# SpectacularAI/3dgs-deblur

Hardware: AMD Instinct MI355X
Metric: fwd+bwd rasterize MPix/s at 1M Gaussians, 1080p, 5 sub-poses (higher is better)
Workload: dtype f32

## Files before the change

3dgs-deblur_amd/_lib.py:

```python
from __future__ import annotations

import ctypes
from pathlib import Path

from ._build import LIB_PATH, build_library

_P, _I, _F, _L = ctypes.c_void_p, ctypes.c_int, ctypes.c_float, ctypes.c_longlong

_SIGS = {
    "gs_subpose_viewmats_fwd": [_I, _P, _P, _P, _P, _P, _P],
    "gs_subpose_viewmats_bwd": [_I, _P, _P, _P, _P, _P, _P, _P, _P, _P],
    "gs_project_fwd": [_I, _P, _P, _F, _P, _P, _F, _F, _F, _F, _I, _I, _F, _P, _P, _P, _P, _P, _P, _P, _P, _P],
    "gs_project_bwd": [_I, _P, _P, _F, _P, _P, _F, _F, _F, _F, _I, _I, _F, _P, _P, _P, _P, _P, _P, _P, _P, _I, _P, _L, _P],
    "gs_sh_fwd": [_I, _I, _I, _P, _P, _P, _P],
    "gs_sh_bwd": [_I, _I, _I, _P, _P, _P, _P],
    "gs_project_fused_fwd": [_I, _I, _P, _P, _F, _P, _P, _P, _I, _I, _P, _F, _F, _F, _F, _I, _I, _F, _I, _I,
                             _P, _P, _P, _P, _P, _I, _P],
    "gs_slice_colors": [_I, _P, _P, _I, _P, _P, _P, _I, _I, _P, _P, _P],
    "gs_project_fused_bwd": [_I, _I, _P, _P, _F, _P, _P, _P, _I, _I, _P, _F, _F, _F, _F, _I, _I, _F, _I,
                             _P, _P, _P, _P, _P, _P, _P, _P, _P, _P, _I, _P, _I, _P, _P, _L, _P],
    "gs_project_pixvel_fwd": [_I, _I, _P, _P, _F, _P, _P, _P, _I, _I, _P, _P, _P, _F, _F, _F, _F, _I, _I, _F, _I, _I,
                              _P, _P, _P, _P, _F, _P, _P, _I, _P],
    "gs_rasterize_fwd_rs_slice": [_P, _P, _P, _P, _I, _I, _I, _P, _P, _P, _P, _P, _I, _I, _P, _I, _P, _P, _P, _I, _F, _P,
                                  _P],
    "gs_rasterize_bwd_rs_slice": [_P, _P, _P, _P, _P, _I, _I, _I, _P, _P, _P, _P, _P, _P, _P, _P, _P, _I, _I, _P, _F, _F,
                                  _P, _I, _F, _P, _P],
    "gs_project_pixvel_bwd": [_I, _I, _P, _P, _F, _P, _P, _P, _I, _I, _P, _P, _P, _F, _F, _F, _F, _I, _I, _F, _I,
                              _P, _P, _P, _P, _P, _P, _P, _P, _P, _P, _P, _I, _P, _I, _P, _P, _L, _P],
    "gs_pack_records": [_I, _P, _P, _P, _P, _P, _P, _I, _I, _P, _P, _P, _P],
    "gs_unpack_record_grads": [_I, _P, _P, _P, _P, _P, _P],
    "gs_exclusive_scan_u32": [_L, _P, _P, _P, _P, _L, _P],
    "gs_radix_sort_pairs_u32": [_L, _P, _P, _P, _P, _I, _I, _I, _P, _L, ctypes.POINTER(_I), _P],
    "gs_radix_sort_pairs_u64": [_L, _P, _P, _P, _P, _I, _I, _I, _P, _L, ctypes.POINTER(_I), _P],
    "gs_radix_sort_pairs_gather_u32": [_L, _P, _P, _P, _P, _I, _I, _I, _P, _L, ctypes.POINTER(_I), _P, _P, _P, _P],
    "gs_radix_sort_pairs_carry_u32": [_L, _P, _P, _P, _P, _I, _I, _I, _P, _L, ctypes.POINTER(_I), _P, _P, _P,
                                      ctypes.POINTER(_I), _P, _P],
    "gs_segmented_sort_pairs_u32": [_L, _L, _P, _P, _P, _P, _I, _I, _I, _P, _L, ctypes.POINTER(_I), _P],
    "gs_segmented_sort_compact_u32": [_L, _L, _P, _P, _P, _P, _I, _I, _I, ctypes.c_uint, _P, _P, _P, _P, _L,
                                      ctypes.POINTER(_I), _P],
    "gs_segmented_sort_select_u32": [_L, _L, _P, _P, _P, _P, _P, _I, _I, _I, ctypes.c_uint, _P, _P, _P, _P, _P, _P, _L,
                                     ctypes.POINTER(_I), _L, _P],
    "gs_depth_select": [_L, _L, _P, _P, _L, _P, _P, _P, _L, _P],
    "gs_exclusive_scan_segments_u32": [_L, _L, _P, _P, _P, _P, _P, _L, _P],
    "gs_make_depth_keys64": [_L, _I, _P, _P, _P],
    "gs_gather_counts": [_L, _P, _P, _P, _P],
    "gs_emit_intersects": [_L, _I, _I, _I, _P, _P, _P, _L, _P, _P, ctypes.c_uint, _P],
    "gs_tile_bin_edges_u32": [_L, _P, _I, _P, _P, _P],
    "gs_tile_bin_edges_u64": [_L, _P, _I, _P, _P],
    "gs_tile_bin_edges_ids_u32": [_L, _P, _I, _P, _P, _P, _P, _P],
    "gs_map_gaussian_to_intersects": [_I, _P, _P, _P, _P, _I, _I, _P, _P, _P],
    "gs_rasterize_fwd": [_P, _P, _P, _P, _P, _I, _I, _I, _I, _P, _P, _P, _I, _I, _P],
    "gs_rasterize_bwd": [_P, _P, _P, _P, _P, _I, _I, _I, _I, _P, _P, _P, _P, _P, _I, _I, _P],
    "gs_slice_plan": [_I, _I, _I, _P, _P, _L, _P, _P, _P, _P, _P, _P],
    "gs_slice_plan_select": [_I, _I, _I, _P, _P, _P, _P, _P, _P, _P, _P, _P],
    "gs_tile_open_sat": [_I, _I, _I, _P, _P, _P, _P, _P],
    "gs_slice_counts": [_I, _I, _I, _P, _P, _P, _P, _P, _I, _I, _P, _P, _P],
    "gs_emit_open_intersects": [_I, _I, _I, _I, _P, _P, _P, _P, _P, _P, _P, ctypes.c_uint, _I, _I, _P, _P, _P, _P],
    "gs_slice_counts_exact": [_I, _I, _I, _P, _P, _P, _P, _P, _P, _I, _I, _P, _P, _I, _P, _P, _P, _P, _P, _P],
    "gs_slice_counts_exact_swept": [_I, _I, _I, _P, _P, _P, _P, _P, _P, _I, _I, _P, _P, _I, _P, _P, _P, _P, _P, _F, _F, _F,
                                    _P],
    "gs_rasterize_fwd_slice": [_P, _P, _P, _P, _P, _I, _I, _I, _I, _P, _P, _P, _P, _P, _I, _I, _P, _P, _I, _P, _P, _P,
                               _I, _P],
    "gs_rasterize_bwd_slice": [_P, _P, _P, _P, _P, _I, _I, _I, _I, _P, _P, _P, _P, _P, _P, _P, _P, _P, _P, _P, _I, _P,
                               _I, _P, _F, _F, _P],
    "gs_rasterize_fwd_slice_stats": [_P, _P, _P, _P, _P, _I, _I, _I, _I, _P, _P, _P, _P, _P, _I, _I, _P, _P, _P, _P],
    "gs_reduce_grad_tuples": [_I, _P, _P, _P, _P, _P, _P, _P, _L, _P, _I, _P],
    "gs_combine_fwd": [_I, _L, _P, _F, _F, _P, _P],
    "gs_combine_bwd": [_I, _L, _P, _F, _F, _P, _P, _P, _P],
    "gs_combine_bwd_scale": [_I, _L, _F, _P, _P, _P, _P],
    "gs_combine_fwd_batched": [_I, _I, _L, _P, _F, _F, _P, _P],
    "gs_combine_bwd_batched": [_I, _I, _L, _P, _F, _F, _P, _P, _P, _P],
    "gs_combine_bwd_scale_batched": [_I, _I, _L, _F, _P, _P, _P, _P],
    "gs_dp_row_mask": [_I, _I, _P, _P, _P, _P],
    "gs_dp_pack_rows": [_L, _P, _I, _P, _P, _P, _P],
    "gs_dp_scatter_add_rows": [_L, _P, _I, _P, _P, _F, _P],
    "gs_dp_pack_masked_rows": [_I, _P, _P, _I, _P, _I, _P, _P, _P, _P],
    "gs_dp_scatter_add_payload": [_I, _P, _I, _P, _P, _F, _P],
    "gs_slice_project_records": [_I, _I, _I, _P, _P, _P, _P, _I, _I, _P, _P],
    "gs_project_records": [_I, _I, _P, _I, _I, _P, _P],
    "gs_frame_forward": [_P, _P, _P, _P, _P, _P, _P, _P, _P, _P, _I, _I, _P, _P, _P, _P, _P, _P, _P, _P, _L, _P, _L, _P, _P],
    "gs_frame_backward": [_P, _P, _P, _P, _P, _P, _P, _P, _F, _F, _I, _P, _P, _P, _P, _P, _L, _P],
    "gs_frame_backward_depth": [_P, _P, _P, _P, _P, _P, _P, _P, _F, _F, _I, _P, _P, _P, _P, _P, _L, _P, _P],
    "gs_xy_absgrad_sum": [_I, _I, _I, _P, _P, _P, _P],
    "gs_frame_profile_enable": [ctypes.c_uint],
    "gs_frame_profile_read": [_I, _P, _P],
    "gs_image_loss_fwd_bwd": [_I, _I, _P, _P, _F, _P, _P, _P, _L, _P],
    "gs_adam_step": [_I, _P, _P, _P, _P, _P, _P, ctypes.c_double, ctypes.c_double, ctypes.c_double, _I, _P],
    "gs_adam_step_rows": [_I, _I, _P, _P, _P, _P, _P, _P, _P, ctypes.c_double, ctypes.c_double, ctypes.c_double, _I,
                          _P, _L, _P],
    "gs_visible_rows": [_I, _I, _P, _P, _P],
    "gs_mcmc_inject_noise": [_I, _P, _P, _P, _P, _F, _L, _L, _P, _P, _P],
    "gs_mcmc_relocation": [_I, _P, _P, _P, _P, _P, _P],
    "gs_bilagrid_slice_fwd": [_I, _I, _I, _I, _I, _I, _I, _P, _P, _P, _P, _P],
    "gs_bilagrid_slice_bwd": [_I, _I, _I, _I, _I, _I, _I, _P, _P, _P, _P, _P, _P, _P, _L, _P],
    "gs_bilagrid_tv_fwd_bwd": [_I, _I, _I, _I, _P, _F, _P, _P, _P, _L, _P],
}
_SIGS_LL = {
    "gs_scan_workspace_bytes": [_L],
    "gs_radix_sort_workspace_bytes": [_L, _I, _I],
    "gs_segmented_sort_workspace_bytes": [_L, _L, _I, _I],
    "gs_segmented_sort_compact_workspace_bytes": [_L, _L, _I, _I, _I],
    "gs_depth_select_workspace_bytes": [_I],
    "gs_project_pose_scratch_bytes": [_I, _I, _I],
    "gs_image_loss_workspace_bytes": [_I, _I],
    "gs_adam_step_rows_workspace_bytes": [_I],
    "gs_frame_backward_bytes": [_P],
    "gs_bilagrid_slice_bwd_workspace_bytes": [_I, _I, _I, _I, _I, _I, _I],
    "gs_bilagrid_tv_workspace_bytes": [_I, _I, _I, _I],
}

_lib = None


class HipLibraryError(RuntimeError):
    pass


def load(build_if_missing: bool = True) -> ctypes.CDLL:
    global _lib
    if _lib is not None:
        return _lib
    import os
    import shutil
    override = os.environ.get("GSD_LIB_PATH")
    path = Path(override) if override else LIB_PATH
    if not override and build_if_missing and shutil.which(os.environ.get("HIPCC", "/opt/rocm/bin/hipcc")):
        from ._build import is_current, HASH_PATH, CSRC
        stale = not is_current()
        if stale and path.exists() and not HASH_PATH.exists():
            t = path.stat().st_mtime
            stale = any(f.stat().st_mtime > t for f in list(CSRC.glob("*.hip")) + list(CSRC.glob("*.h")))
        if stale:
            import fcntl
            try:
                lock = open(str(path) + ".lock", "w")
            except OSError as e:
                if not path.exists():
                    raise HipLibraryError(f"{path} is missing and {path.parent} is not writable: {e}") from e
                import warnings
                warnings.warn(f"{path} may be older than its sources and {path.parent} is not writable; loading it as is")
            else:
                with lock:
                    fcntl.flock(lock, fcntl.LOCK_EX)
                    try:
                        build_library()
                    finally:
                        fcntl.flock(lock, fcntl.LOCK_UN)
    if not path.exists():
        raise HipLibraryError(f"{path} is missing; run __graft_entry__.build()")
    try:
        lib = ctypes.CDLL(str(path))
    except OSError as e:
        raise HipLibraryError(f"cannot load HIP library {path}: {e}") from e
    for name, args in _SIGS.items():
        fn = getattr(lib, name)
        fn.argtypes = args
        fn.restype = _I
    for name, args in _SIGS_LL.items():
        fn = getattr(lib, name)
        fn.argtypes = args
        fn.restype = _L
    lib.gs_version.restype = ctypes.c_char_p
    lib.gs_version.argtypes = []
    _lib = lib
    return lib


def exported_names():
    return sorted(list(_SIGS) + list(_SIGS_LL) + ["gs_version"])


def check(status: int, what: str) -> None:
    if status != 0:
        kind = {1: "invalid argument", 3: "workspace too small"}.get(status, None)
        if kind is None and status >= 1000:
            kind = f"hipError_t {status - 1000}"
        raise HipLibraryError(f"{what} failed: {kind or status}")
```

3dgs-deblur_amd/csrc/binning.hip:

```cpp
#include <algorithm>
#include <atomic>
#include "gs_common.h"

namespace gs {

constexpr int kScanItems = 8;
constexpr int kScanBlock = 256 * kScanItems;

__device__ __forceinline__ unsigned block_excl_scan(unsigned v, unsigned& total, unsigned* lds ) {
  const int lane = lane_id(), wave = threadIdx.x >> 6;
  unsigned inc = v;
#pragma unroll
  for (int o = 1; o < 64; o <<= 1) {
    unsigned t = __shfl_up(inc, o);
    if (lane >= o) inc += t;
  }
  if (lane == 63) lds[wave] = inc;
  __syncthreads();
  unsigned w0 = lds[0], w1 = lds[1], w2 = lds[2], w3 = lds[3];
  unsigned woff = wave == 0 ? 0u : (wave == 1 ? w0 : (wave == 2 ? w0 + w1 : w0 + w1 + w2));
  total = w0 + w1 + w2 + w3;
  __syncthreads();
  return woff + inc - v;
}
// ... 175 lines not shown
  if (n <= kScanSmallMax && !dl.keys && !sm.cnt) {
    hipLaunchKernelGGL(scan_small_kernel, dim3(1), dim3(256), 0, st, n, in, out, total_out);
    return gs_launch_status();
  }
  unsigned* bsum = reinterpret_cast<unsigned*>(ws);
  hipLaunchKernelGGL(scan_reduce_kernel, dim3((unsigned)nb), dim3(256), 0, st, n, in, bsum, dl, sm);
  if (nb <= kScanFusedMaxBlocks || dl.keys || sm.cnt) {
    hipLaunchKernelGGL(scan_apply_fused_kernel, dim3((unsigned)nb), dim3(256), 0, st, n, in, bsum, out, total_out, dl,
                       sm);
  } else {
    hipLaunchKernelGGL(scan_bsums_kernel, dim3(1), dim3(256), 0, st, (unsigned)nb, bsum, total_out);
    hipLaunchKernelGGL(scan_apply_kernel, dim3((unsigned)nb), dim3(256), 0, st, n, in, bsum, out);
  }
  return gs_launch_status();
}

#ifndef GS_SORT_ROUNDS_U32
#define GS_SORT_ROUNDS_U32 16
#endif
template <typename KeyT> struct SortCfg;
template <> struct SortCfg<unsigned> { static constexpr int kRounds = GS_SORT_ROUNDS_U32; };
template <> struct SortCfg<unsigned long long> { static constexpr int kRounds = 16; };

template <typename KeyT> constexpr int sort_block_keys() { return 256 * SortCfg<KeyT>::kRounds; }

struct SegInfo { size_t seg_len; unsigned nblk_seg; };

struct SegDev {
  const unsigned* cnt_in;
  unsigned* cnt_out;
  const unsigned* total;
  unsigned long long skip;
  const unsigned* key_lo;
  const unsigned* key_hi;
};

template <typename KeyT>
struct KeepTest {
  KeyT skip, lo, hi;
  bool on, has_hi;
  __device__ __forceinline__ KeepTest(const SegDev& sd, unsigned seg)
      : skip((KeyT)sd.skip), lo(sd.key_lo ? (KeyT)sd.key_lo[seg] : (KeyT)0), hi(sd.key_hi ? (KeyT)sd.key_hi[seg] : (KeyT)0),
        on(sd.cnt_out != nullptr), has_hi(sd.key_hi != nullptr) {}
  __device__ __forceinline__ bool drop(KeyT k) const { return on && (k == skip || k < lo || (has_hi && k >= hi)); }
};

template <typename KeyT, int BITS>
__global__ __launch_bounds__(256) void radix_hist_kernel(size_t n, const KeyT* __restrict__ keys, int shift,
                                                         unsigned mask, SegInfo sg,
                                                         unsigned* __restrict__ ghist,
                                                         const unsigned* __restrict__ n_dev, SegDev sd) {
  constexpr int NB = 1 << BITS;
  constexpr int R = SortCfg<KeyT>::kRounds;
  if (n_dev) {
    n = min(n, (size_t)*n_dev);
    sg.nblk_seg = (unsigned)((n + 256 * R - 1) / (256 * R));
    if (blockIdx.x >= sg.nblk_seg) return;
  }
  __shared__ unsigned hist[NB];
  const unsigned seg = blockIdx.x / sg.nblk_seg, b = blockIdx.x % sg.nblk_seg;
  const size_t base = (size_t)seg * sg.seg_len + (size_t)b * (256 * R);
  size_t limit = min(n, (size_t)(seg + 1) * sg.seg_len);
  if (sd.cnt_in) limit = min(limit, (size_t)seg * sg.seg_len + sd.cnt_in[seg]);
  if (base >= limit) {
    for (int d = threadIdx.x; d < NB; d += 256) ghist[((size_t)seg * NB + d) * sg.nblk_seg + b] = 0u;
    return;
  }
  for (int d = threadIdx.x; d < NB; d += 256) hist[d] = 0;
  __syncthreads();
  KeyT k[R];
#pragma unroll
  for (int r = 0; r < R; ++r) {
    size_t i = base + (size_t)r * 256 + threadIdx.x;
    k[r] = i < limit ? keys[i] : (KeyT)0;
  }
  const int lane = lane_id();
  const KeepTest<KeyT> keep(sd, seg);
  bool skewed;
  {
    const size_t i0 = base + threadIdx.x;
    const bool ok0 = i0 < limit && !keep.drop(k[0]);
    const unsigned d = (unsigned)(k[0] >> shift) & mask;
    const unsigned long long m = __ballot(ok0);
    const unsigned d0 = (unsigned)readlane_i((int)d, m ? __ffsll((long long)m) - 1 : 0);
    skewed = __popcll(__ballot(ok0 && d == d0)) >= 16;
  }
  if (skewed) {
#pragma unroll
    for (int r = 0; r < R; ++r) {
      size_t i = base + (size_t)r * 256 + threadIdx.x;
      const bool ok = i < limit && !keep.drop(k[r]);
      const unsigned d = (unsigned)(k[r] >> shift) & mask;
      unsigned long long todo = __ballot(ok);
#pragma unroll 1
      for (int it = 0; it < 4 && todo; ++it) {
        const int src = __ffsll((long long)todo) - 1;
        const unsigned d0 = (unsigned)readlane_i((int)d, src);
        const unsigned long long same = __ballot(ok && d == d0) & todo;
        if (lane == src) atomicAdd(&hist[d0], (unsigned)__popcll(same));
        todo &= ~same;
      }
      if ((todo >> lane) & 1ull) atomicAdd(&hist[d], 1u);
    }
  } else {
#pragma unroll
    for (int r = 0; r < R; ++r) {
      size_t i = base + (size_t)r * 256 + threadIdx.x;
      if (i < limit && !keep.drop(k[r])) atomicAdd(&hist[(unsigned)(k[r] >> shift) & mask], 1u);
    }
  }
  __syncthreads();
  for (int d = threadIdx.x; d < NB; d += 256) ghist[((size_t)seg * NB + d) * sg.nblk_seg + b] = hist[d];
}

template <typename KeyT, int BITS, int PACK = 0>
__global__ __launch_bounds__(256) void radix_scatter_kernel(size_t n, const KeyT* __restrict__ keys_in,
                                                            const unsigned* __restrict__ vals_in,
                                                            KeyT* __restrict__ keys_out,
                                                            unsigned* __restrict__ vals_out, int shift, unsigned mask,
                                                            SegInfo sg,
                                                            const unsigned* __restrict__ ghist_scanned,
                                                            const unsigned* __restrict__ gather_src,
                                                            unsigned* __restrict__ gather_out,
                                                            const unsigned* __restrict__ n_dev, SegDev sd,
                                                            const unsigned* __restrict__ p2_in,
                                                            unsigned* __restrict__ p2_out,
                                                            int pack_bits) {
  constexpr int NB = 1 << BITS;
  constexpr int R = SortCfg<KeyT>::kRounds;
  constexpr int BK = 256 * R;
  if (n_dev) {
    n = min(n, (size_t)*n_dev);
    sg.nblk_seg = (unsigned)((n + BK - 1) / BK);
    if (blockIdx.x >= sg.nblk_seg) return;
  }
  {
    const unsigned seg0 = blockIdx.x / sg.nblk_seg, blk0 = blockIdx.x % sg.nblk_seg;
    if (sd.cnt_in && (size_t)blk0 * BK >= (size_t)sd.cnt_in[seg0]) return;
  }
  constexpr int DPT = NB / 256;
  __shared__ KeyT s_keys[BK];
  __shared__ unsigned s_vals[BK];
  __shared__ unsigned cnt[4][NB];
  __shared__ unsigned s_dbase[NB];
  __shared__ unsigned s_gbase[NB];
  __shared__ unsigned s_scan[8];
  const int lane = lane_id(), wave = threadIdx.x >> 6;
  for (int d = threadIdx.x; d < 4 * NB; d += 256) (&cnt[0][0])[d] = 0;
  __syncthreads();
  const unsigned seg = blockIdx.x / sg.nblk_seg, blk = blockIdx.x % sg.nblk_seg;
  const size_t bbase = (size_t)seg * sg.seg_len + (size_t)blk * BK;
  size_t limit = min(n, (size_t)(seg + 1) * sg.seg_len);
  if (sd.cnt_in) limit = min(limit, (size_t)seg * sg.seg_len + sd.cnt_in[seg]);
  const bool compacting = sd.cnt_out != nullptr;
  const KeepTest<KeyT> keep(sd, seg);
  const size_t wbase = bbase + (size_t)wave * (R * 64);
  const unsigned long long lt_mask = (1ull << lane) - 1ull;
  KeyT key[R];
  unsigned short pos[R];
#pragma unroll
  for (int r = 0; r < R; ++r) {
    size_t i = wbase + (size_t)r * 64 + lane;
    key[r] = i < limit ? keys_in[i] : (KeyT)0;
  }
#pragma unroll
  for (int r = 0; r < R; ++r) {
    size_t i = wbase + (size_t)r * 64 + lane;
    bool valid = i < limit && !keep.drop(key[r]);
    unsigned digit = (unsigned)(key[r] >> shift) & mask;
    unsigned long long peers = __ballot(valid);
#pragma unroll
    for (int b = 0; b < BITS; ++b) {
      bool bit = (digit >> b) & 1u;
      unsigned long long m = __ballot(bit);
      peers &= bit ? m : ~m;
    }
    unsigned prefix = __popcll(peers & lt_mask);
    unsigned total = __popcll(peers);
    unsigned base = 0;
    if (valid) base = cnt[wave][digit];
    __builtin_amdgcn_wave_barrier();
    if (valid && prefix == 0) cnt[wave][digit] = base + total;
    __builtin_amdgcn_wave_barrier();
    pos[r] = (unsigned short)(base + prefix);
  }
  __syncthreads();
  {
    unsigned c[DPT], sum = 0;
#pragma unroll
    for (int j = 0; j < DPT; ++j) {
      int d = threadIdx.x * DPT + j;
      c[j] = cnt[0][d] + cnt[1][d] + cnt[2][d] + cnt[3][d];
      sum += c[j];
    }
    unsigned tot;
    unsigned ex = block_excl_scan(sum, tot, s_scan);
    if (threadIdx.x == 0) s_scan[4] = tot;
    const unsigned seg_org = (unsigned)((size_t)seg * sg.seg_len);
    unsigned gb[DPT];
    const size_t seg_first = (size_t)seg * NB * sg.nblk_seg;
    const unsigned seg_base = ghist_scanned[seg_first];
    if (compacting && blk == 0 && threadIdx.x == 0) {
      const unsigned nseg = gridDim.x / sg.nblk_seg;
      const unsigned next = seg + 1 < nseg ? ghist_scanned[seg_first + (size_t)NB * sg.nblk_seg] : *sd.total;
      sd.cnt_out[seg] = next - seg_base;
    }
#pragma unroll
    for (int j = 0; j < DPT; ++j)
      gb[j] = ghist_scanned[seg_first + (size_t)(threadIdx.x * DPT + j) * sg.nblk_seg + blk] - seg_base + seg_org;
#pragma unroll
    for (int j = 0; j < DPT; ++j) {
      int d = threadIdx.x * DPT + j;
      s_dbase[d] = ex;
      s_gbase[d] = gb[j];
      unsigned run = ex;
#pragma unroll
      for (int w = 0; w < 4; ++w) {
        unsigned cw = cnt[w][d];
        cnt[w][d] = run;
        run += cw;
      }
      ex += c[j];
    }
  }
  __syncthreads();
  constexpr int RB = R >= 4 ? 4 : R;
  unsigned pv[RB];
#pragma unroll
  for (int r0 = 0; r0 < R; r0 += RB) {
    if (PACK == 1 || vals_in) {
      const unsigned* __restrict__ src = PACK == 1 ? gather_src : vals_in;
      const size_t last = limit ? limit - 1 : 0;
#pragma unroll
      for (int q = 0; q < RB; ++q) pv[q] = src[min(wbase + (size_t)(r0 + q) * 64 + lane, last)];
    }
#pragma unroll
    for (int q = 0; q < RB; ++q) {
      const int r = r0 + q;
      size_t i = wbase + (size_t)r * 64 + lane;
      if (i < limit && !keep.drop(key[r])) {
        unsigned digit = (unsigned)(key[r] >> shift) & mask;
        unsigned slot = cnt[wave][digit] + pos[r];
        s_keys[slot] = key[r];
        if (PACK == 1) s_vals[slot] = (unsigned)i | (min(pv[q], (1u << (32 - pack_bits)) - 1u) << pack_bits);
        else s_vals[slot] = vals_in ? pv[q] : (unsigned)i;
      }
    }
  }
  __syncthreads();
  const unsigned nvalid = s_scan[4];
#pragma unroll 4
  for (int r = 0; r < R; ++r) {
    unsigned slot = (unsigned)r * 256 + threadIdx.x;
    if (slot < nvalid) {
      KeyT k = s_keys[slot];
      unsigned digit = (unsigned)(k >> shift) & mask;
      size_t dst = (size_t)s_gbase[digit] + (slot - s_dbase[digit]);
      keys_out[dst] = k;
      const unsigned v = s_vals[slot];
      if (PACK == 2) {
        const unsigned idx = v & ((1u << pack_bits) - 1u), c = v >> pack_bits;
        vals_out[dst] = idx;
        gather_out[dst] = c == (1u << (32 - pack_bits)) - 1u ? gather_src[idx] : c;
      } else {
        vals_out[dst] = v;
        if (gather_out) gather_out[dst] = gather_src[v];
      }
    }
  }
  if (p2_out) {
    __syncthreads();
#pragma unroll
    for (int r0 = 0; r0 < R; r0 += RB) {
      const size_t last = limit ? limit - 1 : 0;
#pragma unroll
      for (int q = 0; q < RB; ++q) pv[q] = p2_in[min(wbase + (size_t)(r0 + q) * 64 + lane, last)];
#pragma unroll
      for (int q = 0; q < RB; ++q) {
        const int r = r0 + q;
        size_t i = wbase + (size_t)r * 64 + lane;
        if (i < limit && !keep.drop(key[r])) {
          unsigned digit = (unsigned)(key[r] >> shift) & mask;
          s_vals[cnt[wave][digit] + pos[r]] = pv[q];
        }
      }
    }
    __syncthreads();
#pragma unroll 4
    for (int r = 0; r < R; ++r) {
      unsigned slot = (unsigned)r * 256 + threadIdx.x;
      if (slot < nvalid) {
        unsigned digit = (unsigned)(s_keys[slot] >> shift) & mask;
        p2_out[(size_t)s_gbase[digit] + (slot - s_dbase[digit])] = s_vals[slot];
      }
    }
  }
}

constexpr int kTailR = 24;
constexpr int kTailLocalCap = kTailR * 1024;
constexpr int kTailMaxBits = 9;
constexpr size_t kTailLds = ((size_t)kTailLocalCap + 16 * (1 << kTailMaxBits) + 64) * sizeof(unsigned);

__global__ __launch_bounds__(1024) void seg_tail_sort_kernel(size_t seg_len, const unsigned* __restrict__ keys_in,
                                                             const unsigned* __restrict__ vals_in,
                                                             unsigned* __restrict__ keys_out,
                                                             unsigned* __restrict__ vals_out,
                                                             const unsigned* __restrict__ cnt_in, int begin_bit, int end_bit,
                                                             const unsigned* __restrict__ gather_src,
                                                             unsigned* __restrict__ gather_out, int pack_bits) {
  extern __shared__ unsigned tail_lds[];
  unsigned* const stage = tail_lds;
  unsigned* const cnt = stage + kTailLocalCap;
  unsigned* const red = cnt + 16 * (1 << kTailMaxBits);
  const unsigned seg = blockIdx.x;
  const unsigned n = cnt_in[seg];
  if (n == 0 || n > (unsigned)kTailLocalCap) return;
  const size_t org = (size_t)seg * seg_len;
  const int lane = lane_id(), wave = threadIdx.x >> 6;
  const unsigned Re = (n + 1023u) >> 10;
  const unsigned wbase = (unsigned)wave * Re * 64u;
  const unsigned long long lt_mask = (1ull << lane) - 1ull;
  unsigned key[kTailR];
  unsigned pos2[kTailR / 2];
  unsigned kmin = 0xffffffffu, kmax = 0u;
  const unsigned emask = end_bit >= 32 ? 0xffffffffu : (1u << end_bit) - 1u;
#pragma unroll
  for (int r = 0; r < kTailR; ++r) {
    const unsigned e = wbase + (unsigned)r * 64u + lane;
    const bool ok = (unsigned)r < Re && e < n;
    key[r] = ok ? keys_in[org + e] : 0u;
    if (ok) {
      stage[e] = vals_in[org + e];
      kmin = min(kmin, key[r] & emask);
      kmax = max(kmax, key[r] & emask);
    }
  }
#pragma unroll
  for (int o = 32; o > 0; o >>= 1) {
    kmin = min(kmin, (unsigned)__shfl_xor((int)kmin, o));
    kmax = max(kmax, (unsigned)__shfl_xor((int)kmax, o));
  }
  if (lane == 0) { red[wave] = kmin; red[16 + wave] = kmax; }
  __syncthreads();
#pragma unroll
  for (int w = 0; w < 16; ++w) { kmin = min(kmin, red[w]); kmax = max(kmax, red[16 + w]); }
  const unsigned base = kmin & ~((1u << begin_bit) - 1u);
  const unsigned span = (kmax - base) >> begin_bit;
  const int rem = span ? 32 - __clz((int)span) : 0;
  const int passes = (rem + kTailMaxBits - 1) / kTailMaxBits;
  const int wbits = passes ? (rem + passes - 1) / passes : 0;
  const unsigned nb = 1u << wbits, mask = nb - 1u;
  int shift = begin_bit;
  for (int p = 0; p < passes; ++p, shift += wbits) {
    for (unsigned d = threadIdx.x; d < 16u * nb; d += 1024u) cnt[d] = 0u;
    __syncthreads();
    unsigned* const wcnt = cnt + (unsigned)wave * nb;
#pragma unroll
    for (int r = 0; r < kTailR; ++r) {
      if ((unsigned)r < Re) {
        const unsigned e = wbase + (unsigned)r * 64u + lane;
        const bool valid = e < n;
        const unsigned digit = (((key[r] & emask) - base) >> shift) & mask;
        unsigned long long peers = __ballot(valid);
#pragma unroll
        for (int b = 0; b < kTailMaxBits; ++b) {
          if (b < wbits) {
            const bool bit = (digit >> b) & 1u;
            const unsigned long long m = __ballot(bit);
            peers &= bit ? m : ~m;
          }
        }
        const unsigned prefix = __popcll(peers & lt_mask), total = __popcll(peers);
        unsigned c0 = 0;
        if (valid) c0 = wcnt[digit];
        __builtin_amdgcn_wave_barrier();
        if (valid && prefix == 0) wcnt[digit] = c0 + total;
        __builtin_amdgcn_wave_barrier();
        pos2[r >> 1] = (r & 1) ? (pos2[r >> 1] | ((c0 + prefix) << 16)) : (c0 + prefix);
      }
    }
    __syncthreads();
    {
      const unsigned d = threadIdx.x;
      unsigned c = 0;
      if (d < nb) {
#pragma unroll
        for (int w = 0; w < 16; ++w) c += cnt[(unsigned)w * nb + d];
      }
      unsigned inc = c;
#pragma unroll
      for (int o = 1; o < 64; o <<= 1) {
        const unsigned t = __shfl_up(inc, o);
        if (lane >= o) inc += t;
      }
      if (lane == 63) red[32 + wave] = inc;
      __syncthreads();
      unsigned run = inc - c;
      for (int w = 0; w < wave; ++w) run += red[32 + w];
      if (d < nb) {
#pragma unroll
        for (int w = 0; w < 16; ++w) {
          const unsigned cw = cnt[(unsigned)w * nb + d];
          cnt[(unsigned)w * nb + d] = run;
          run += cw;
        }
      }
    }
    __syncthreads();
    unsigned val[kTailR];
#pragma unroll
    for (int r = 0; r < kTailR; ++r) {
      const unsigned e = wbase + (unsigned)r * 64u + lane;
      if ((unsigned)r < Re && e < n) {
        val[r] = stage[e];
        const unsigned rank = (r & 1) ? pos2[r >> 1] >> 16 : pos2[r >> 1] & 0xffffu;
        const unsigned slot = wcnt[(((key[r] & emask) - base) >> shift) & mask] + rank;
        pos2[r >> 1] = (r & 1) ? ((pos2[r >> 1] & 0xffffu) | (slot << 16)) : ((pos2[r >> 1] & 0xffff0000u) | slot);
      }
    }
    __syncthreads();
#pragma unroll
    for (int r = 0; r < kTailR; ++r) {
      const unsigned e = wbase + (unsigned)r * 64u + lane;
      if ((unsigned)r < Re && e < n) stage[(r & 1) ? pos2[r >> 1] >> 16 : pos2[r >> 1] & 0xffffu] = key[r];
    }
    __syncthreads();
#pragma unroll
    for (int r = 0; r < kTailR; ++r) {
      const unsigned e = wbase + (unsigned)r * 64u + lane;
      if ((unsigned)r < Re && e < n) key[r] = stage[e];
    }
    __syncthreads();
#pragma unroll
    for (int r = 0; r < kTailR; ++r) {
      const unsigned e = wbase + (unsigned)r * 64u + lane;
      if ((unsigned)r < Re && e < n) stage[(r & 1) ? pos2[r >> 1] >> 16 : pos2[r >> 1] & 0xffffu] = val[r];
    }
    __syncthreads();
  }
#pragma unroll
  for (int r = 0; r < kTailR; ++r) {
    const unsigned e = wbase + (unsigned)r * 64u + lane;
    if ((unsigned)r < Re && e < n) {
      keys_out[org + e] = key[r];
      const unsigned v = stage[e];
      if (pack_bits) {
        const unsigned idx = v & ((1u << pack_bits) - 1u), c = v >> pack_bits;
        vals_out[org + e] = idx;
        gather_out[org + e] = c == (1u << (32 - pack_bits)) - 1u ? gather_src[idx] : c;
      } else {
        vals_out[org + e] = v;
        if (gather_out) gather_out[org + e] = gather_src[v];
      }
    }
  }
}

template <typename KeyT>
static inline unsigned sort_nblk(size_t n) {
  return (unsigned)((n + sort_block_keys<KeyT>() - 1) / sort_block_keys<KeyT>());
}
template <typename KeyT>
static inline unsigned sort_nblk_seg(size_t n, size_t seg_len, unsigned* nblk_seg) {
  if (seg_len == 0 || seg_len >= n) { *nblk_seg = sort_nblk<KeyT>(n); return *nblk_seg; }
  *nblk_seg = sort_nblk<KeyT>(seg_len);
  return (unsigned)((n + seg_len - 1) / seg_len) * *nblk_seg;
}

static inline void radix_plan(int bits, int* passes, int* per, int* tmpl_bits, int max_digit = 11) {
  if (max_digit < 8) max_digit = 8;
  if (max_digit > 11) max_digit = 11;
  int ps = (bits + max_digit - 1) / max_digit;
  if (ps < 1) ps = 1;
  int w = (bits + ps - 1) / ps;
  *passes = ps; *per = w; *tmpl_bits = w < 8 ? 8 : w;
}

template <typename KeyT>
static inline size_t radix_hist_bytes(size_t n, size_t seg_len, int bits, int max_digit = 11) {
  int ps, per, tb;
  radix_plan(bits, &ps, &per, &tb, max_digit);
  unsigned nbs;
  size_t b = ((size_t)1 << tb) * sort_nblk_seg<KeyT>(n, seg_len, &nbs) * sizeof(unsigned);
  return (b + 255) & ~(size_t)255;
}

template <typename KeyT>
static inline size_t radix_ws_bytes(size_t n, size_t seg_len, int bits, int max_digit = 11) {
  int ps, per, tb;
  radix_plan(bits, &ps, &per, &tb, max_digit);
  unsigned nbs;
  return radix_hist_bytes<KeyT>(n, seg_len, bits, max_digit) +
         scan_ws_bytes(((size_t)1 << tb) * sort_nblk_seg<KeyT>(n, seg_len, &nbs)) + 256;
}

template <typename KeyT, int BITS>
static void radix_pass(size_t n, size_t seg_len, const KeyT* kin, const unsigned* vin, KeyT* kout, unsigned* vout,
                       int shift, unsigned mask, void* ws, size_t hist_bytes, hipStream_t st,
                       const unsigned* gather_src = nullptr, unsigned* gather_out = nullptr,
                       const unsigned* n_dev = nullptr, SegDev sd = SegDev{nullptr, nullptr, nullptr, 0ull, nullptr, nullptr},
                       const unsigned* p2_in = nullptr, unsigned* p2_out = nullptr, int pack = 0, int pack_bits = 0,
                       unsigned tail_blocks = 0) {
  SegInfo sg;
  unsigned nblk = sort_nblk_seg<KeyT>(n, seg_len, &sg.nblk_seg);
  sg.seg_len = (seg_len == 0 || seg_len >= n) ? n : seg_len;
  if (tail_blocks && tail_blocks < sg.nblk_seg) {
    nblk = nblk / sg.nblk_seg * tail_blocks;
    sg.nblk_seg = tail_blocks;
  }
  unsigned* ghist = reinterpret_cast<unsigned*>(ws);
  {
    size_t hn = ((size_t)1 << BITS) * nblk;
    void* scan_ws = reinterpret_cast<char*>(ws) + hist_bytes;
    hipLaunchKernelGGL((radix_hist_kernel<KeyT, BITS>), dim3(nblk), dim3(256), 0, st, n, kin, shift, mask, sg, ghist,
                       n_dev, sd);
    run_scan(hn, ghist, ghist, sd.cnt_out ? const_cast<unsigned*>(sd.total) : nullptr, scan_ws, st,
             DevLen{n_dev, (unsigned)sort_block_keys<KeyT>(), (unsigned)(1u << BITS)});
  }
  if constexpr (BITS == 8 && sizeof(KeyT) == 4) {
    if (pack == 1) {
      hipLaunchKernelGGL((radix_scatter_kernel<KeyT, BITS, 1>), dim3(nblk), dim3(256), 0, st, n, kin, vin, kout, vout,
                         shift, mask, sg, ghist, gather_src, gather_out, n_dev, sd, p2_in, p2_out, pack_bits);
      return;
    }
    if (pack == 2) {
      hipLaunchKernelGGL((radix_scatter_kernel<KeyT, BITS, 2>), dim3(nblk), dim3(256), 0, st, n, kin, vin, kout, vout,
                         shift, mask, sg, ghist, gather_src, gather_out, n_dev, sd, p2_in, p2_out, pack_bits);
      return;
    }
  }
  hipLaunchKernelGGL((radix_scatter_kernel<KeyT, BITS>), dim3(nblk), dim3(256), 0, st, n, kin, vin, kout, vout, shift,
                     mask, sg, ghist, gather_src, gather_out, n_dev, sd, p2_in, p2_out, 0);
}

template <typename KeyT>
static int radix_sort(size_t n, size_t seg_len, KeyT* k0, unsigned* v0, KeyT* k1, unsigned* v1, int v0_is_iota,
                      int begin_bit, int end_bit, void* ws, size_t ws_bytes, int* result_buf, hipStream_t st,
                      int max_digit = 11, const unsigned* gather_src = nullptr, unsigned* gather_out = nullptr,
                      const unsigned* n_dev = nullptr, unsigned* seg_counts = nullptr,
                      unsigned long long skip_key = 0ull, const unsigned* p2_src = nullptr, unsigned* p2_a = nullptr,
                      unsigned* p2_b = nullptr, int* result_p2 = nullptr, const KeyT* k_src = nullptr,
                      const unsigned* key_lo = nullptr, const unsigned* key_hi = nullptr, unsigned tail_blocks = 0) {
  int bits = end_bit - begin_bit;
  if (bits <= 0) return GS_ERR_INVALID;
  if (ws_bytes < radix_ws_bytes<KeyT>(n, seg_len, bits, max_digit)) return GS_ERR_WORKSPACE;
  int passes, per, tb;
  radix_plan(bits, &passes, &per, &tb, max_digit);
  const size_t hist_bytes = radix_hist_bytes<KeyT>(n, seg_len, bits, max_digit);
  KeyT* kk[2] = {k0, k1};
  unsigned* vv[2] = {v0, v1};
  int cur = 0, shift = begin_bit;
  int pack_bits = 0;
  if (sizeof(KeyT) == 4 && gather_src && gather_out && seg_counts && v0_is_iota && !p2_src &&
      tb == 8 && passes >= 2) {
    while (((size_t)1 << pack_bits) < n) ++pack_bits;
    if (pack_bits > 28) pack_bits = 0;
  }
  for (int p = 0; p < passes; ++p) {
    int w = per;
    if (shift + w > end_bit) w = end_bit - shift;
    const unsigned mask = (1u << w) - 1u;
    const unsigned* vin = (p == 0 && v0_is_iota) ? nullptr : vv[cur];
    const int pack = pack_bits ? (p == 0 ? 1 : (p == passes - 1 ? 2 : 0)) : 0;
    const unsigned* gs_ = (p == passes - 1 || pack == 1) ? gather_src : nullptr;
    unsigned* go_ = (p == passes - 1) ? gather_out : nullptr;
    SegDev sd{nullptr, nullptr, nullptr, 0ull};
    if (seg_counts) {
      unsigned* total_dev = reinterpret_cast<unsigned*>(reinterpret_cast<char*>(ws) +
                                                        radix_ws_bytes<KeyT>(n, seg_len, bits, max_digit) - 128);
      if (p == 0) sd = SegDev{nullptr, seg_counts, total_dev, skip_key, key_lo, key_hi};
      else sd = SegDev{seg_counts, nullptr, nullptr, 0ull, nullptr, nullptr};
    }
    const unsigned* p2i = nullptr;
    unsigned* p2o = nullptr;
    if (p2_src) {
      p2o = (p & 1) ? p2_b : p2_a;
      p2i = p == 0 ? p2_src : ((p & 1) ? p2_a : p2_b);
    }
    const KeyT* kin = (p == 0 && k_src) ? k_src : kk[cur];
    switch (tb) {
      case 8:  radix_pass<KeyT, 8>(n, seg_len, kin, vin, kk[cur ^ 1], vv[cur ^ 1], shift, mask, ws, hist_bytes, st, gs_, go_, n_dev, sd, p2i, p2o, pack, pack_bits, p > 0 ? tail_blocks : 0u); break;
      case 9:  radix_pass<KeyT, 9>(n, seg_len, kin, vin, kk[cur ^ 1], vv[cur ^ 1], shift, mask, ws, hist_bytes, st, gs_, go_, n_dev, sd, p2i, p2o, 0, 0, p > 0 ? tail_blocks : 0u); break;
      case 10: radix_pass<KeyT, 10>(n, seg_len, kin, vin, kk[cur ^ 1], vv[cur ^ 1], shift, mask, ws, hist_bytes, st, gs_, go_, n_dev, sd, p2i, p2o, 0, 0, p > 0 ? tail_blocks : 0u); break;
      default: radix_pass<KeyT, 11>(n, seg_len, kin, vin, kk[cur ^ 1], vv[cur ^ 1], shift, mask, ws, hist_bytes, st, gs_, go_, n_dev, sd, p2i, p2o, 0, 0, p > 0 ? tail_blocks : 0u); break;
    }
    shift += w;
    cur ^= 1;
    if constexpr (sizeof(KeyT) == 4) {
      if (p == 0 && passes >= 2 && seg_counts && !p2_src && tail_blocks &&
          (size_t)tail_blocks * sort_block_keys<KeyT>() <= (size_t)kTailLocalCap && (pack_bits || !gather_out || gather_src)) {
        static std::atomic<unsigned long long> lds_set{0ull};
        int dev = 0;
        (void)hipGetDevice(&dev);
        const unsigned long long bit = 1ull << (dev & 63);
        bool lds_ok = (lds_set.load(std::memory_order_relaxed) & bit) != 0;
        if (!lds_ok && hipFuncSetAttribute(reinterpret_cast<const void*>(seg_tail_sort_kernel),
                                           hipFuncAttributeMaxDynamicSharedMemorySize, (int)kTailLds) == hipSuccess) {
          lds_set.fetch_or(bit, std::memory_order_relaxed);
          lds_ok = true;
        }
        if (lds_ok) {
          const size_t sl = (seg_len == 0 || seg_len >= n) ? n : seg_len;
          hipLaunchKernelGGL(seg_tail_sort_kernel, dim3((unsigned)((n + sl - 1) / sl)), dim3(1024), kTailLds, st, sl,
                             reinterpret_cast<const unsigned*>(kk[cur]), vv[cur], reinterpret_cast<unsigned*>(kk[cur ^ 1]),
                             vv[cur ^ 1], seg_counts, shift, end_bit, gather_src, gather_out, pack_bits);
          *result_buf = cur ^ 1;
          return gs_launch_status();
        }
      }
    }
  }
  *result_buf = cur;
  if (result_p2) *result_p2 = (passes - 1) & 1;
  return gs_launch_status();
}

__global__ __launch_bounds__(256) void gather_counts_kernel(size_t n, const unsigned* __restrict__ sorted_gi,
                                                            const int* __restrict__ ntiles,
                                                            unsigned* __restrict__ out) {
  size_t i = (size_t)blockIdx.x * 256 + threadIdx.x;
  if (i < n) out[i] = (unsigned)ntiles[sorted_gi[i]];
}

struct Ellipse { float gx, gy, a, b, c, tau, ra, rc, ustar, vstar, vext;
                 float pvx, pvy, st0, st1, srs; };

__device__ __forceinline__ void ellipse_derive(Ellipse& e) {
#pragma clang fp contract(off)
  e.ra = 1.0f / e.a; e.rc = 1.0f / e.c;
  const float det = e.a * e.c - e.b * e.b;
  if (e.tau >= 0.f && det > 0.f && e.a > 0.f && e.c > 0.f) {
    const float k = 2.0f * e.tau / det;
    e.ustar = sqrtf(k * e.c) * 1.0001f;
    e.vext = sqrtf(k * e.a) * 1.0001f;
    e.vstar = e.b * e.ustar * e.rc;
  } else {
    e.ustar = e.vext = 3.0e38f;
    e.vstar = 0.f;
  }
}

__device__ __forceinline__ Ellipse make_ellipse(const float* __restrict__ rec) {
#pragma clang fp contract(off)
  Ellipse e;
  e.gx = rec[0]; e.gy = rec[1]; e.a = rec[2]; e.b = rec[3]; e.c = rec[4];
  const float op = rec[5];
  e.tau = op > 0.f ? __logf(255.0f * op) : -1.f;
  e.tau = e.tau < 0.f ? -1.f : e.tau * 1.001f + 1e-3f;
  ellipse_derive(e);
  return e;
}

struct RowSpan { float ul, ur; };

template <bool SWEEP = false>
__device__ __forceinline__ RowSpan row_span(const Ellipse& e, int ty, int H) {
#pragma clang fp contract(off)
  RowSpan r;
  r.ul = 1.f; r.ur = -1.f;
  if (e.tau < 0.f) return r;
  if (e.ustar > 1.0e37f) { r.ul = -3.0e38f; r.ur = 3.0e38f; return r; }
  float v0 = (float)(ty * K::kTile) + 0.5f - e.gy;
  float v1 = fminf((float)(ty * K::kTile + K::kTile) - 0.5f, (float)H - 0.5f) - e.gy;
  float ox0 = 0.f, ox1 = 0.f;
  if (SWEEP) {
    const float invH = 1.0f / (float)H;
    const float ya = (float)(ty * K::kTile) + 0.5f, yb = fminf((float)(ty * K::kTile + K::kTile) - 0.5f, (float)H - 0.5f);
    const float ta = (ya * invH - 0.5f) * e.srs, tb = (yb * invH - 0.5f) * e.srs;
    const float t_lo = e.st0 + fminf(ta, tb), t_hi = e.st1 + fmaxf(ta, tb);
    const float slack = 1e-3f + 1e-5f * (fabsf(t_lo) + fabsf(t_hi)) * (fabsf(e.pvx) + fabsf(e.pvy));
    ox0 = fminf(t_lo * e.pvx, t_hi * e.pvx) - slack; ox1 = fmaxf(t_lo * e.pvx, t_hi * e.pvx) + slack;
    const float oy0 = fminf(t_lo * e.pvy, t_hi * e.pvy) - slack, oy1 = fmaxf(t_lo * e.pvy, t_hi * e.pvy) + slack;
    v0 -= oy1; v1 -= oy0;
  }
  if (v1 < -e.vext || v0 > e.vext) return r;
  const float w0 = fmaxf(v0, -e.vext), w1 = fminf(v1, e.vext);
  const float det = e.a * e.c - e.b * e.b;
  const float k2 = 2.0f * e.a * e.tau;
  const float d0 = sqrtf(fmaxf(k2 - det * w0 * w0, 0.f)), d1 = sqrtf(fmaxf(k2 - det * w1 * w1, 0.f));
  const float c0 = -e.b * w0, c1 = -e.b * w1;
  float ur = fmaxf((c0 + d0) * e.ra, (c1 + d1) * e.ra);
  float ul = fminf((c0 - d0) * e.ra, (c1 - d1) * e.ra);
  if (-e.vstar >= w0 && -e.vstar <= w1) ur = e.ustar;
  if (e.vstar >= w0 && e.vstar <= w1) ul = -e.ustar;
  const float eps = 2e-3f + 2e-6f * (fabsf(e.gx) + e.ustar);
  r.ur = fmaxf(ur, ul) + eps + ox1;
  r.ul = fminf(ul, ur) - eps + ox0;
  return r;
}

__device__ __forceinline__ void span_tiles(const Ellipse& e, const RowSpan& sp, int x0, int x1, int& t0, int& t1) {
#pragma clang fp contract(off)
  if (sp.ur < sp.ul) { t0 = t1 = x0; return; }
  const float lo = (sp.ul + e.gx - 15.5f) * (1.0f / (float)K::kTile);
  const float hi = (sp.ur + e.gx - 0.5f) * (1.0f / (float)K::kTile);
  const float flo = fminf(fmaxf(ceilf(lo), (float)x0), (float)x1);
  const float fhi = fminf(fmaxf(floorf(hi) + 1.0f, (float)x0), (float)x1);
  t0 = (int)flo; t1 = (int)fhi;
  if (t1 < t0) t1 = t0;
}

template <bool SWEEP = false>
__device__ __forceinline__ bool tile_hit(const Ellipse& e, int tx, int ty, int W, int H) {
  (void)W;
  const RowSpan sp = row_span<SWEEP>(e, ty, H);
  int t0, t1;
  span_tiles(e, sp, tx, tx + 1, t0, t1);
  return t1 > t0;
}

constexpr int kEmitItems = 16;
constexpr int kEmitChunk = 256 * kEmitItems;

__device__ __forceinline__ unsigned rank_of_entry(const unsigned* __restrict__ cum, unsigned n, unsigned e) {
  unsigned lo = 0, hi = n - 1;
  while (lo < hi) {
    unsigned mid = (lo + hi + 1) >> 1;
    if (cum[mid] <= e) lo = mid; else hi = mid - 1;
  }
  return lo;
}

__global__ __launch_bounds__(256) void emit_kernel(size_t n_ranked, int N, int T, int tiles_x,
                                                   const unsigned* __restrict__ sorted_gi,
                                                   const unsigned* __restrict__ cum,
                                                   const float* __restrict__ records, size_t n_isect,
                                                   unsigned* __restrict__ keys, unsigned* __restrict__ vals,
                                                   int W, int H, unsigned invalid_key ) {
  __shared__ unsigned s_cum[257];
  __shared__ unsigned s_gi[256];
  __shared__ unsigned s_kbase[256];
  __shared__ unsigned s_w[256];
  __shared__ unsigned s_xy0[256];
  __shared__ float s_rw[256];
  __shared__ float s_gx[256], s_gy[256], s_a[256], s_b[256], s_c[256], s_tau[256];
  __shared__ unsigned s_rng[2];
  const unsigned e_begin = blockIdx.x * (unsigned)kEmitChunk;
  const unsigned e_end = (unsigned)min((size_t)e_begin + kEmitChunk, n_isect);
  if (threadIdx.x < 2)
    s_rng[threadIdx.x] = rank_of_entry(cum, (unsigned)n_ranked, threadIdx.x == 0 ? e_begin : e_end - 1);
  __syncthreads();
  const unsigned g_lo = s_rng[0], g_hi = s_rng[1];
  for (unsigned wbase = g_lo; wbase <= g_hi; wbase += 256) {
    const unsigned r = wbase + threadIdx.x;
    unsigned gi = 0, c = 0xFFFFFFFFu, kbase = 0, w = 1, xy0 = 0;
    Ellipse el = {0.f, 0.f, 1.f, 0.f, 1.f, -1.f, 1.f, 1.f, 0.f, 0.f, 0.f};
    if (r <= g_hi) {
      gi = sorted_gi[r];
      c = cum[r];
      const float* rec = records + (size_t)gi * kRecFloats;
      unsigned lo = (unsigned)__float_as_int(rec[10]);
      unsigned hi = (unsigned)__float_as_int(rec[11]);
      unsigned x0 = lo & 0xFFFFu, x1 = hi & 0xFFFFu;
      w = x1 > x0 ? x1 - x0 : 1u;
      xy0 = lo;
      kbase = (gi / (unsigned)N) * (unsigned)T;
      if (invalid_key) el = make_ellipse(rec);
// ... 579 lines not shown
    for (int r = 0; r < kSelRounds; ++r) {
      const size_t i = base + (size_t)r * 256 + threadIdx.x;
      const bool ok = (k[r] >> 31) == 0u && (LEVEL == 0 || (k[r] >> 20) == b1);
      w[r] = ok ? weights[min(i, limit - 1)] : 0u;
    }
#pragma unroll
    for (int r = 0; r < kSelRounds; ++r)
      if (w[r]) atomicAdd(&h[LEVEL == 0 ? (k[r] >> 20) : ((k[r] >> 9) & (unsigned)(kSelBins - 1))], (unsigned long long)w[r]);
  }
  __syncthreads();
  for (int d = threadIdx.x; d < kSelBins; d += 256)
    if (h[d]) atomicAdd(&S.hist[LEVEL][d], h[d]);
}

__global__ __launch_bounds__(256) void depth_find_kernel(unsigned long long budget, const SelSeg* __restrict__ ws,
                                                         unsigned* __restrict__ thr_out,
                                                         unsigned* __restrict__ grand_out) {
  __shared__ unsigned long long s_scan[8], s_res[2];
  const unsigned seg = blockIdx.x;
  const SelSeg& S = ws[seg];
  unsigned long long before0, total0, before1, total1;
  const unsigned b1 = sel_crossing(S.hist[0], budget, s_scan, s_res, before0, total0);
  unsigned thr = 0x80000000u;
  if (b1 < (unsigned)kSelBins) {
    unsigned b2 = sel_crossing(S.hist[1], budget - before0, s_scan, s_res, before1, total1);
    if (b2 >= (unsigned)kSelBins) b2 = (unsigned)(kSelBins - 1);
    thr = (((b1 << kSelBits) | b2) + 1u) << 9;
  }
  if (threadIdx.x == 0) {
    thr_out[seg] = thr;
    if (grand_out) atomicAdd(grand_out, (unsigned)total0);
  }
}

__global__ __launch_bounds__(256) void map_isect_kernel(int N, const float* __restrict__ xys,
                                                        const float* __restrict__ depths,
                                                        const int* __restrict__ radii,
                                                        const int* __restrict__ cum_tiles_hit,
                                                        int tiles_x, int tiles_y, long long* __restrict__ isect_ids,
                                                        int* __restrict__ gaussian_ids) {
  int i = blockIdx.x * 256 + threadIdx.x;
  if (i >= N) return;
  int rad = radii[i];
  if (rad <= 0) return;
  const float inv_tile = 1.0f / (float)K::kTile;
  float radf = (float)rad;
  float tcx = xys[2 * i] * inv_tile, tcy = xys[2 * i + 1] * inv_tile, tr = radf * inv_tile;
  int x0 = (int)(tcx - tr), x1 = (int)(tcx + tr + 1.0f);
  int y0 = (int)(tcy - tr), y1 = (int)(tcy + tr + 1.0f);
  x0 = x0 < 0 ? 0 : (x0 > tiles_x ? tiles_x : x0);
  x1 = x1 < 0 ? 0 : (x1 > tiles_x ? tiles_x : x1);
  y0 = y0 < 0 ? 0 : (y0 > tiles_y ? tiles_y : y0);
  y1 = y1 < 0 ? 0 : (y1 > tiles_y ? tiles_y : y1);
  long long depth_bits = (long long)(unsigned)__float_as_int(depths[i]);
  int cur = i == 0 ? 0 : cum_tiles_hit[i - 1];
  for (int y = y0; y < y1; ++y)
    for (int x = x0; x < x1; ++x) {
      long long tile = (long long)(y * tiles_x + x);
      isect_ids[cur] = (tile << 32) | depth_bits;
      gaussian_ids[cur] = i;
      ++cur;
    }
}

__global__ __launch_bounds__(256) void depth_keys64_kernel(size_t n, int N, const unsigned* __restrict__ dk,
                                                           unsigned long long* __restrict__ out) {
  size_t i = (size_t)blockIdx.x * 256 + threadIdx.x;
  if (i < n) out[i] = ((unsigned long long)(i / (size_t)N) << 32) | (unsigned long long)dk[i];
}

}

using namespace gs;

GS_EXPORT long long gs_scan_workspace_bytes(long long n) { return (long long)scan_ws_bytes((size_t)n) + 256; }
GS_EXPORT long long gs_radix_sort_workspace_bytes(long long n, int begin_bit, int end_bit) {
  if (n <= 0 || end_bit <= begin_bit) return 0;
  size_t a = radix_ws_bytes<unsigned>((size_t)n, 0, end_bit - begin_bit);
  size_t b = radix_ws_bytes<unsigned long long>((size_t)n, 0, end_bit - begin_bit);
  return (long long)(a > b ? a : b);
}

GS_EXPORT int gs_exclusive_scan_u32(long long n, const unsigned* in, unsigned* out, unsigned* total_out, void* ws,
                                    long long ws_bytes, void* stream) {
  if (n <= 0) return GS_ERR_INVALID;
  if ((size_t)ws_bytes < scan_ws_bytes((size_t)n)) return GS_ERR_WORKSPACE;
  return run_scan((size_t)n, in, out, total_out, ws, (hipStream_t)stream);
}

GS_EXPORT int gs_radix_sort_pairs_u32(long long n, unsigned* keys0, unsigned* vals0, unsigned* keys1,
                                      unsigned* vals1, int vals0_is_iota, int begin_bit, int end_bit, void* ws,
                                      long long ws_bytes, int* result_buf, void* stream) {
  if (n <= 0 || begin_bit < 0 || end_bit > 32) return GS_ERR_INVALID;
  return radix_sort<unsigned>((size_t)n, 0, keys0, vals0, keys1, vals1, vals0_is_iota, begin_bit, end_bit, ws,
                              (size_t)ws_bytes, result_buf, (hipStream_t)stream);
}

GS_EXPORT int gs_radix_sort_pairs_gather_u32(long long n, unsigned* keys0, unsigned* vals0, unsigned* keys1,
                                             unsigned* vals1, int vals0_is_iota, int begin_bit, int end_bit,
                                             void* ws, long long ws_bytes, int* result_buf,
                                             const unsigned* gather_src, unsigned* gather_out,
                                             const unsigned* n_dev, void* stream) {
  if (n <= 0 || begin_bit < 0 || end_bit > 32 || !gather_src || !gather_out) return GS_ERR_INVALID;
  return radix_sort<unsigned>((size_t)n, 0, keys0, vals0, keys1, vals1, vals0_is_iota, begin_bit, end_bit, ws,
                              (size_t)ws_bytes, result_buf, (hipStream_t)stream, 11, gather_src, gather_out, n_dev);
}

GS_EXPORT int gs_radix_sort_pairs_carry_u32(long long n, unsigned* keys0, unsigned* vals0, unsigned* keys1,
                                            unsigned* vals1, int vals0_is_iota, int begin_bit, int end_bit, void* ws,
                                            long long ws_bytes, int* result_buf, const unsigned* payload2_in,
                                            unsigned* payload2_a, unsigned* payload2_b, int* result_p2,
                                            const unsigned* n_dev, void* stream) {
  if (n <= 0 || begin_bit < 0 || end_bit > 32 || !payload2_in || !payload2_a || !payload2_b || !result_p2)
    return GS_ERR_INVALID;
  return radix_sort<unsigned>((size_t)n, 0, keys0, vals0, keys1, vals1, vals0_is_iota, begin_bit, end_bit, ws,
                              (size_t)ws_bytes, result_buf, (hipStream_t)stream, 11, nullptr, nullptr, n_dev, nullptr,
                              0ull, payload2_in, payload2_a, payload2_b, result_p2);
}

GS_EXPORT int gs_radix_sort_pairs_u64(long long n, unsigned long long* keys0, unsigned* vals0,
                                      unsigned long long* keys1, unsigned* vals1, int vals0_is_iota, int begin_bit,
                                      int end_bit, void* ws, long long ws_bytes, int* result_buf, void* stream) {
  if (n <= 0 || begin_bit < 0 || end_bit > 64) return GS_ERR_INVALID;
  return radix_sort<unsigned long long>((size_t)n, 0, keys0, vals0, keys1, vals1, vals0_is_iota, begin_bit, end_bit,
                                        ws, (size_t)ws_bytes, result_buf, (hipStream_t)stream);
}

GS_EXPORT long long gs_segmented_sort_workspace_bytes(long long n, long long seg_len, int begin_bit, int end_bit) {
  if (n <= 0 || seg_len <= 0 || end_bit <= begin_bit) return 0;
  return (long long)radix_ws_bytes<unsigned>((size_t)n, (size_t)seg_len, end_bit - begin_bit, 8);
}

GS_EXPORT int gs_segmented_sort_pairs_u32(long long n, long long seg_len, unsigned* keys0, unsigned* vals0,
                                          unsigned* keys1, unsigned* vals1, int vals0_is_iota, int begin_bit,
                                          int end_bit, void* ws, long long ws_bytes, int* result_buf, void* stream) {
  if (n <= 0 || seg_len <= 0 || n % seg_len != 0 || begin_bit < 0 || end_bit > 32) return GS_ERR_INVALID;
  return radix_sort<unsigned>((size_t)n, (size_t)seg_len, keys0, vals0, keys1, vals1, vals0_is_iota, begin_bit,
                              end_bit, ws, (size_t)ws_bytes, result_buf, (hipStream_t)stream, 8);
}

GS_EXPORT long long gs_segmented_sort_compact_workspace_bytes(long long n, long long seg_len, int begin_bit,
                                                              int end_bit, int max_digit_bits) {
  if (n <= 0 || seg_len <= 0 || end_bit <= begin_bit) return 0;
  return (long long)radix_ws_bytes<unsigned>((size_t)n, (size_t)seg_len, end_bit - begin_bit, max_digit_bits);
}

GS_EXPORT int gs_segmented_sort_compact_u32(long long n, long long seg_len, unsigned* keys0, unsigned* vals0,
                                            unsigned* keys1, unsigned* vals1, int begin_bit, int end_bit,
                                            int max_digit_bits, unsigned skip_key, unsigned* seg_counts,
                                            const unsigned* gather_src, unsigned* gather_out, void* ws,
                                            long long ws_bytes, int* result_buf, void* stream) {
  if (n <= 0 || seg_len <= 0 || n % seg_len != 0 || begin_bit < 0 || end_bit > 32 || !seg_counts)
    return GS_ERR_INVALID;
  if ((gather_src != nullptr) != (gather_out != nullptr)) return GS_ERR_INVALID;
  return radix_sort<unsigned>((size_t)n, (size_t)seg_len, keys0, vals0, keys1, vals1, 1, begin_bit, end_bit, ws,
                              (size_t)ws_bytes, result_buf, (hipStream_t)stream, max_digit_bits, gather_src,
                              gather_out, nullptr, seg_counts, (unsigned long long)skip_key);
}

GS_EXPORT int gs_exclusive_scan_segments_u32(long long n, long long seg_len, const unsigned* seg_counts,
                                             const unsigned* in, unsigned* out, unsigned* total_out, void* ws,
                                             long long ws_bytes, void* stream) {
  if (n <= 0 || seg_len <= 0 || n % seg_len != 0 || !seg_counts) return GS_ERR_INVALID;
  if ((size_t)ws_bytes < scan_ws_bytes((size_t)n)) return GS_ERR_WORKSPACE;
  return run_scan((size_t)n, in, out, total_out, ws, (hipStream_t)stream, DevLen{nullptr, 1u, 1u},
                  SegMask{seg_counts, (size_t)seg_len});
}

GS_EXPORT int gs_make_depth_keys64(long long n, int N, const unsigned* depth_keys, unsigned long long* out,
                                   void* stream) {
  if (n <= 0 || N <= 0) return GS_ERR_INVALID;
  hipLaunchKernelGGL(depth_keys64_kernel, dim3((unsigned)((n + 255) / 256)), dim3(256), 0, (hipStream_t)stream,
                     (size_t)n, N, depth_keys, out);
  return gs_launch_status();
}

GS_EXPORT int gs_gather_counts(long long n, const unsigned* sorted_gi, const int* num_tiles_hit, unsigned* counts_out,
                               void* stream) {
  if (n <= 0) return GS_ERR_INVALID;
  hipLaunchKernelGGL(gather_counts_kernel, dim3((unsigned)((n + 255) / 256)), dim3(256), 0, (hipStream_t)stream,
                     (size_t)n, sorted_gi, num_tiles_hit, counts_out);
  return gs_launch_status();
}

GS_EXPORT int gs_emit_intersects(long long n_ranked, int N, int H, int W, const unsigned* sorted_gi,
                                 const unsigned* cum_excl, const float* records, long long n_isect, unsigned* keys,
                                 unsigned* vals, unsigned invalid_key, void* stream) {
  if (n_ranked <= 0 || N <= 0) return GS_ERR_INVALID;
  if (n_isect <= 0) return GS_OK;
  int tiles_x = (W + K::kTile - 1) / K::kTile, tiles_y = (H + K::kTile - 1) / K::kTile;
  hipLaunchKernelGGL(emit_kernel, dim3((unsigned)((n_isect + kEmitChunk - 1) / kEmitChunk)), dim3(256), 0,
                     (hipStream_t)stream, (size_t)n_ranked, N, tiles_x * tiles_y, tiles_x, sorted_gi, cum_excl, records,
                     (size_t)n_isect, keys, vals, W, H, invalid_key);
  return gs_launch_status();
}

GS_EXPORT int gs_tile_bin_edges_u32(long long n, const unsigned* sorted_keys, int num_bins, int* bins,
                                    const unsigned* n_dev, void* stream) {
  if (num_bins <= 0) return GS_ERR_INVALID;
  if (n <= 0) {
    hipError_t e = hipMemsetAsync(bins, 0, (size_t)num_bins * 2 * sizeof(int), (hipStream_t)stream);
    return e == hipSuccess ? GS_OK : 1000 + (int)e;
  }
  unsigned blocks = (unsigned)((n + 255) / 256);
  if (n_dev && blocks > 8192u) blocks = 8192u;
  hipLaunchKernelGGL((bin_edges_kernel<unsigned, 0>), dim3(blocks), dim3(256), 0,
                     (hipStream_t)stream, (size_t)n, sorted_keys, reinterpret_cast<int2*>(bins), (unsigned)num_bins, n_dev);
  return gs_launch_status();
}

GS_EXPORT int gs_tile_bin_edges_ids_u32(long long n, const unsigned* sorted_keys, int num_bins, int* bins,
                                        const unsigned* sorted_vals, const unsigned* gi_of_e, unsigned* ids_out,
                                        void* stream) {
  if (num_bins <= 0 || !sorted_vals || !gi_of_e || !ids_out) return GS_ERR_INVALID;
  hipError_t e = hipMemsetAsync(bins, 0, (size_t)num_bins * 2 * sizeof(int), (hipStream_t)stream);
  if (e != hipSuccess) return 1000 + (int)e;
  if (n < 0) return GS_ERR_INVALID;
  hipLaunchKernelGGL(bin_edges_ids_kernel, dim3((unsigned)((n + 8 + 255) / 256)), dim3(256), 0, (hipStream_t)stream,
                     (size_t)n, sorted_keys, reinterpret_cast<int2*>(bins), sorted_vals, gi_of_e, ids_out);
  return gs_launch_status();
}

GS_EXPORT int gs_tile_bin_edges_u64(long long n, const unsigned long long* sorted_ids, int num_bins, int* bins,
                                    void* stream) {
  if (num_bins <= 0) return GS_ERR_INVALID;
  if (n <= 0) {
    hipError_t e = hipMemsetAsync(bins, 0, (size_t)num_bins * 2 * sizeof(int), (hipStream_t)stream);
    return e == hipSuccess ? GS_OK : 1000 + (int)e;
  }
  hipLaunchKernelGGL((bin_edges_kernel<unsigned long long, 32>), dim3((unsigned)((n + 255) / 256)), dim3(256), 0,
                     (hipStream_t)stream, (size_t)n, sorted_ids, reinterpret_cast<int2*>(bins), (unsigned)num_bins);
  return gs_launch_status();
}

GS_EXPORT int gs_map_gaussian_to_intersects(int N, const float* xys, const float* depths, const int* radii,
                                            const int* cum_tiles_hit, int H, int W, long long* isect_ids,
                                            int* gaussian_ids, void* stream) {
  if (N <= 0) return GS_ERR_INVALID;
  int tiles_x = (W + K::kTile - 1) / K::kTile, tiles_y = (H + K::kTile - 1) / K::kTile;
  hipLaunchKernelGGL(map_isect_kernel, dim3((N + 255) / 256), dim3(256), 0, (hipStream_t)stream, N, xys, depths,
                     radii, cum_tiles_hit, tiles_x, tiles_y, isect_ids, gaussian_ids);
  return gs_launch_status();
}

GS_EXPORT int gs_slice_plan(int P, int N, int K, const unsigned* cum_excl, const unsigned* total, long long base,
                            int* bounds, unsigned* rels, unsigned* seg_totals, const unsigned* n_live,
                            unsigned* tail, void* stream) {
  if (P <= 0 || N <= 0 || K <= 0 || K > 32 || base <= 0) return GS_ERR_INVALID;
  hipLaunchKernelGGL(slice_plan_kernel, dim3((P * K + 63) / 64), dim3(64), 0, (hipStream_t)stream, P, N, K, cum_excl,
                     total, (unsigned long long)base, bounds, rels, seg_totals, n_live, tail, (const unsigned*)nullptr);
  return gs_launch_status();
}

GS_EXPORT int gs_slice_plan_select(int P, int N, int K, const unsigned* cum_excl, const unsigned* total, int* bounds,
                                   unsigned* rels, unsigned* seg_totals, const unsigned* n_live, unsigned* tail,
                                   const unsigned* grand, void* stream) {
  if (P <= 0 || N <= 0 || K <= 0 || K > 32 || !n_live || !grand) return GS_ERR_INVALID;
  hipLaunchKernelGGL(slice_plan_kernel, dim3((P * K + 63) / 64), dim3(64), 0, (hipStream_t)stream, P, N, K, cum_excl,
                     total, 1ull << 40, bounds, rels, seg_totals, n_live, tail, grand);
  return gs_launch_status();
}

GS_EXPORT long long gs_depth_select_workspace_bytes(int segments) {
  return segments > 0 ? (long long)segments * (long long)sizeof(SelSeg) + 256 : 0;
}

GS_EXPORT int gs_depth_select(long long n, long long seg_len, const unsigned* keys, const unsigned* weights,
                              long long budget, unsigned* thr_out, unsigned* grand_out, void* ws, long long ws_bytes,
                              void* stream) {
  if (n <= 0 || seg_len <= 0 || n % seg_len != 0 || budget <= 0 || !keys || !weights || !thr_out || !ws)
    return GS_ERR_INVALID;
  const long long segs = n / seg_len;
  if (segs > 65535) return GS_ERR_INVALID;
  if (ws_bytes < gs_depth_select_workspace_bytes((int)segs)) return GS_ERR_WORKSPACE;
  const long long chunks = (seg_len + 256 * kSelRounds - 1) / (256 * kSelRounds);
  const unsigned gx = (unsigned)std::max(1ll, std::min((chunks + 1) / 2, std::max(1ll, 1024 / segs)));
  SelSeg* S = reinterpret_cast<SelSeg*>(ws);
  hipLaunchKernelGGL(depth_hist_kernel<0>, dim3(gx, (unsigned)segs), dim3(256), 0, (hipStream_t)stream, (size_t)seg_len,
                     keys, weights, (unsigned long long)budget, S);
  hipLaunchKernelGGL(depth_hist_kernel<1>, dim3(gx, (unsigned)segs), dim3(256), 0, (hipStream_t)stream, (size_t)seg_len,
                     keys, weights, (unsigned long long)budget, S);
  hipLaunchKernelGGL(depth_find_kernel, dim3((unsigned)segs), dim3(256), 0, (hipStream_t)stream,
                     (unsigned long long)budget, S, thr_out, grand_out);
  return gs_launch_status();
}

GS_EXPORT int gs_segmented_sort_select_u32(long long n, long long seg_len, const unsigned* keys_src, unsigned* keys0,
                                           unsigned* vals0, unsigned* keys1, unsigned* vals1, int begin_bit, int end_bit,
                                           int max_digit_bits, unsigned skip_key, const unsigned* key_lo,
                                           const unsigned* key_hi, unsigned* seg_counts, const unsigned* gather_src,
                                           unsigned* gather_out, void* ws, long long ws_bytes, int* result_buf,
                                           long long tail_cap, void* stream) {
  if (n <= 0 || seg_len <= 0 || n % seg_len != 0 || begin_bit < 0 || end_bit > 32 || !seg_counts || !keys_src ||
      tail_cap < 0)
    return GS_ERR_INVALID;
  if ((gather_src != nullptr) != (gather_out != nullptr)) return GS_ERR_INVALID;
  return radix_sort<unsigned>((size_t)n, (size_t)seg_len, keys0, vals0, keys1, vals1, 1, begin_bit, end_bit, ws,
                              (size_t)ws_bytes, result_buf, (hipStream_t)stream, max_digit_bits, gather_src,
                              gather_out, nullptr, seg_counts, (unsigned long long)skip_key, nullptr, nullptr, nullptr,
                              nullptr, keys_src, key_lo, key_hi,
                              tail_cap > 0 ? (unsigned)((tail_cap + sort_block_keys<unsigned>() - 1) / sort_block_keys<unsigned>()) : 0u);
}

GS_EXPORT int gs_tile_open_sat(int P, int H, int W, const unsigned char* tile_done, int* sat,
                               unsigned long long* open_bits, const int* gate, void* stream) {
  if (P <= 0) return GS_ERR_INVALID;
  int tiles_x = (W + K::kTile - 1) / K::kTile, tiles_y = (H + K::kTile - 1) / K::kTile;
  size_t lds = (size_t)(tiles_x + 1) * (tiles_y + 1) * sizeof(int);
  if (lds > 160 * 1024) return GS_ERR_INVALID;
  if (lds > 48 * 1024)
    (void)hipFuncSetAttribute(reinterpret_cast<const void*>(tile_sat_kernel), hipFuncAttributeMaxDynamicSharedMemorySize,
                              (int)lds);
  hipLaunchKernelGGL(tile_sat_kernel, dim3(P), dim3(256), lds, (hipStream_t)stream, tiles_x, tiles_y, tile_done, sat,
                     open_bits, gate);
  return gs_launch_status();
}

GS_EXPORT int gs_slice_counts(int n_slice, int P, int N, const int* slice_begin, const int* slice_prefix,
                              const unsigned* sorted_gi, const float* records, const int* sat, int H, int W,
                              unsigned* slice_gi, unsigned* counts, void* stream) {
  SliceDesc sd;
  if (n_slice <= 0 || !make_slice_desc(P, slice_begin, slice_prefix, sd)) return GS_ERR_INVALID;
  int tiles_x = (W + K::kTile - 1) / K::kTile, tiles_y = (H + K::kTile - 1) / K::kTile;
  hipLaunchKernelGGL(slice_counts_kernel, dim3((n_slice + 255) / 256), dim3(256), 0, (hipStream_t)stream, n_slice, sd,
                     N, tiles_x, tiles_y, sorted_gi, records, sat, slice_gi, counts);
  return gs_launch_status();
}

GS_EXPORT int gs_slice_counts_exact(int n_slice, int P, int N, const int* slice_begin, const int* slice_prefix,
                                    const unsigned* sorted_gi, const float* records, const int* sat,
                                    const unsigned char* tile_done, int H, int W, unsigned* slice_gi,
                                    unsigned* counts, int wave_per_gaussian, const unsigned* cum_rank,
                                    unsigned long long* hit_masks, unsigned* mask_off,
                                    const unsigned long long* open_bits, const int* gate, void* stream) {
  SliceDesc sd;
  if (n_slice <= 0 || !make_slice_desc(P, slice_begin, slice_prefix, sd)) return GS_ERR_INVALID;
  if (hit_masks && (!cum_rank || !mask_off)) return GS_ERR_INVALID;
  if ((tile_done != nullptr) != (open_bits != nullptr)) return GS_ERR_INVALID;
  int tiles_x = (W + K::kTile - 1) / K::kTile, tiles_y = (H + K::kTile - 1) / K::kTile;
  const SweepP none{nullptr, 0.f, 0.f, 0.f};
  if (wave_per_gaussian)
    hipLaunchKernelGGL(slice_counts_exact_kernel<true>, dim3((n_slice + 3) / 4), dim3(256), 0, (hipStream_t)stream,
                       n_slice, sd, N, tiles_x, tiles_y, sorted_gi, records, sat, tile_done, W, H, slice_gi, counts,
                       cum_rank, hit_masks, mask_off, open_bits, gate, none);
  else
    hipLaunchKernelGGL(slice_counts_exact_kernel<false>, dim3((n_slice + 255) / 256), dim3(256), 0,
                       (hipStream_t)stream, n_slice, sd, N, tiles_x, tiles_y, sorted_gi, records, sat, tile_done, W,
                       H, slice_gi, counts, cum_rank, hit_masks, mask_off, open_bits, gate, none);
  return gs_launch_status();
}

GS_EXPORT int gs_slice_counts_exact_swept(int n_slice, int P, int N, const int* slice_begin, const int* slice_prefix,
                                          const unsigned* sorted_gi, const float* records, const int* sat,
                                          const unsigned char* tile_done, int H, int W, unsigned* slice_gi,
                                          unsigned* counts, int wave_per_gaussian, const unsigned* cum_rank,
                                          unsigned long long* hit_masks, unsigned* mask_off,
                                          const unsigned long long* open_bits, const float* pix_vel, float t_min,
                                          float t_max, float rolling_shutter_time, void* stream) {
  SliceDesc sd;
  if (n_slice <= 0 || N <= 0 || !pix_vel || !hit_masks || !cum_rank || !mask_off ||
      !make_slice_desc(P, slice_begin, slice_prefix, sd))
    return GS_ERR_INVALID;
  if ((tile_done != nullptr) != (open_bits != nullptr)) return GS_ERR_INVALID;
  int tiles_x = (W + K::kTile - 1) / K::kTile, tiles_y = (H + K::kTile - 1) / K::kTile;
  const SweepP sw{pix_vel, fminf(t_min, t_max), fmaxf(t_min, t_max), rolling_shutter_time};
  if (wave_per_gaussian)
    hipLaunchKernelGGL((slice_counts_exact_kernel<true, true>), dim3((n_slice + 3) / 4), dim3(256), 0, (hipStream_t)stream,
                       n_slice, sd, N, tiles_x, tiles_y, sorted_gi, records, sat, tile_done, W, H, slice_gi, counts,
                       cum_rank, hit_masks, mask_off, open_bits, (const int*)nullptr, sw);
  else
    hipLaunchKernelGGL((slice_counts_exact_kernel<false, true>), dim3((n_slice + 255) / 256), dim3(256), 0,
                       (hipStream_t)stream, n_slice, sd, N, tiles_x, tiles_y, sorted_gi, records, sat, tile_done, W,
                       H, slice_gi, counts, cum_rank, hit_masks, mask_off, open_bits, (const int*)nullptr, sw);
  return gs_launch_status();
}

GS_EXPORT int gs_emit_open_intersects(int n_slice, int N, int H, int W, const unsigned* slice_gi,
                                      const unsigned* counts, const unsigned* cum_excl, const float* records,
                                      const unsigned char* tile_done, unsigned* keys, unsigned* vals,
                                      unsigned invalid_key, int compact, int wave_per_gaussian,
                                      const unsigned long long* hit_masks, const unsigned* mask_off,
                                      unsigned char* tile_hot, void* stream) {
  if (n_slice <= 0) return GS_ERR_INVALID;
  if (hit_masks && (!mask_off || !compact)) return GS_ERR_INVALID;
  int tiles_x = (W + K::kTile - 1) / K::kTile, tiles_y = (H + K::kTile - 1) / K::kTile;
  if (wave_per_gaussian)
    hipLaunchKernelGGL(emit_open_kernel<true>, dim3((n_slice + 3) / 4), dim3(256), 0, (hipStream_t)stream, n_slice, N,
                       tiles_x * tiles_y, tiles_x, slice_gi, counts, cum_excl, records, tile_done, keys, vals, W, H,
                       invalid_key, compact, hit_masks, mask_off, tile_hot);
  else
    hipLaunchKernelGGL(emit_open_kernel<false>, dim3((n_slice + 255) / 256), dim3(256), 0, (hipStream_t)stream, n_slice,
                       N, tiles_x * tiles_y, tiles_x, slice_gi, counts, cum_excl, records, tile_done, keys, vals, W, H,
                       invalid_key, compact, hit_masks, mask_off, tile_hot);
  return gs_launch_status();
}

GS_EXPORT const char* gs_version(void) { return "gsdeblur-hip 0.1 (gfx950, wave64)"; }
```

3dgs-deblur_amd/csrc/frame.hip:

```cpp
#include <hip/hip_runtime.h>
#include <stdint.h>
#include <string.h>
#include <time.h>
#include <algorithm>
#include <atomic>
#include <mutex>
#include <vector>
#include "../../include/gsdeblur.h"

#define GS_OK 0
#define GS_ERR_INVALID 1
#define GS_ERR_WORKSPACE 3
#define GS_EXPORT extern "C" __attribute__((visibility("default")))

extern "C" int gs_rasterize_bwd_slice_depth(const float* records, const int* sorted_vals, const int* tile_bins,
                                            const int* band_edges, const float* background, int S, int R, int H, int W,
                                            const float* out_T, const int* final_idx, const float* v_img,
                                            const float* v_alpha, float* bwd_T, float* bwd_B, float* v_records,
                                            const int* gi_of_e, float* tuples, unsigned char* flags,
                                            const int* sorted_ids, int n_records, const unsigned char* tile_hot,
                                            int variant, const float* cmb_scale, float cmb_gamma, float cmb_min_level,
                                            const float* v_depth, int cameras, void* stream);
extern "C" int gs_rasterize_bwd_rs_slice_depth(const float* records, const int* sorted_vals, const int* tile_bins,
                                               const int* band_edges, const float* background, int S, int H, int W,
                                               const float* out_T, const int* final_idx, const float* v_img,
                                               const float* v_alpha, float* bwd_T, float* bwd_B, float* tuples,
                                               unsigned char* flags, const int* sorted_ids, int n_records, int variant,
                                               const float* cmb_scale, float cmb_gamma, float cmb_min_level,
                                               const float* pix_vel, int N, float rolling_shutter_time,
                                               const float* shared_list_times, const float* v_depth, void* stream);
extern "C" int gs_reduce_grad_tuples_depth(int n_slice, const unsigned* slice_gi, const unsigned* counts,
                                           const unsigned* cum_excl, const float* tuples, const unsigned char* flags,
                                           float* v_records, unsigned char* touched, long long n_isect,
                                           const float* records, int tuples_per_entry, int depth, void* stream);

namespace {

constexpr int kTile = 16;
constexpr int kKMax = GS_FRAME_MAX_SLICES;
constexpr int kIdsPad = 8;

struct Arena {
  char* base;
  long long cap, off;
  bool ok;
  Arena(void* b, long long c, long long start = 0) : base((char*)b), cap(c), off(start), ok(true) {}
  static long long up(long long x) { return (x + 255) & ~255ll; }
  template <typename T> T* take(long long count) {
    const long long a = up(off), bytes = count * (long long)sizeof(T);
    if (!ok || a + bytes > cap) { ok = false; off = a + bytes; return nullptr; }
    off = a + bytes;
    return reinterpret_cast<T*>(base + a);
  }
  long long offset_of(const void* p) const { return p ? (long long)((const char*)p - base) : -1; }
};

inline int bits_for(long long n) {
  int b = 1;
  while ((1ll << b) < std::max(2ll, n)) ++b;
  return b;
}

inline int hip_status(hipError_t e) { return e == hipSuccess ? GS_OK : 1000 + (int)e; }

struct StageEvents { int stage; hipEvent_t a, b; };
std::atomic<unsigned> g_profile_mask{0};
std::mutex g_profile_mu;
std::vector<StageEvents> g_events;
std::vector<StageEvents> g_pool;

struct StageScope {
  hipStream_t st;
  bool on;
  StageEvents ev;
  StageScope(int stage, hipStream_t s) : st(s), on((g_profile_mask.load(std::memory_order_relaxed) >> stage) & 1u) {
    if (!on) return;
    bool have = false;
    {
      std::lock_guard<std::mutex> lk(g_profile_mu);
      if (!g_pool.empty()) { ev = g_pool.back(); g_pool.pop_back(); have = true; }
    }
    if (!have) { (void)hipEventCreate(&ev.a); (void)hipEventCreate(&ev.b); }
    ev.stage = stage;
    (void)hipEventRecord(ev.a, st);
  }
  ~StageScope() {
    if (!on) return;
    (void)hipEventRecord(ev.b, st);
    std::lock_guard<std::mutex> lk(g_profile_mu);
    g_events.push_back(ev);
  }
};

constexpr long long kPollTimeoutUs = 50000;

__global__ __launch_bounds__(256) void publish_words_kernel(const unsigned* __restrict__ src, unsigned* dst, int n,
                                                            unsigned seq) {
  for (int i = threadIdx.x; i < n; i += 256)
    __hip_atomic_store(dst + 1 + i, src[i], __ATOMIC_RELAXED, __HIP_MEMORY_SCOPE_SYSTEM);
  __threadfence_system();
  __syncthreads();
  if (threadIdx.x == 0) __hip_atomic_store(dst, seq, __ATOMIC_RELEASE, __HIP_MEMORY_SCOPE_SYSTEM);
}

inline long long now_us() {
  timespec ts;
  clock_gettime(CLOCK_MONOTONIC, &ts);
  return (long long)ts.tv_sec * 1000000ll + ts.tv_nsec / 1000;
}

__global__ void and_tile_done_kernel(int S, int T, const unsigned char* __restrict__ done_s, unsigned char* __restrict__ done) {
  const int t = blockIdx.x * blockDim.x + threadIdx.x;
  if (t >= T) return;
  unsigned char a = 1;
  for (int s = 0; s < S; ++s) a &= done_s[(size_t)s * T + t] != 0;
  done[t] = a;
}

inline void cpu_relax() {
#if defined(__x86_64__) || defined(__i386__)
  __builtin_ia32_pause();
#elif defined(__aarch64__)
  asm volatile("yield" ::: "memory");
#else
  asm volatile("" ::: "memory");
#endif
}

template <class Between>
inline int read_back(const unsigned* src_dev, unsigned* host_pinned, int n, bool poll, hipStream_t st, Between between) {
  if (!poll) {
    hipError_t e = hipMemcpyAsync(host_pinned + 1, src_dev, 4ll * n, hipMemcpyDeviceToHost, st);
    if (e != hipSuccess) return 1000 + (int)e;
    int rb = between();
    if (rb != GS_OK) return rb;
    return hip_status(hipStreamSynchronize(st));
  }
  volatile unsigned* seqw = host_pinned;
  *seqw = 0u;
  __atomic_thread_fence(__ATOMIC_SEQ_CST);
  hipLaunchKernelGGL(publish_words_kernel, dim3(1), dim3(256), 0, st, src_dev, host_pinned, n, 1u);
  hipError_t e = hipGetLastError();
  if (e != hipSuccess) return 1000 + (int)e;
  int rb = between();
  if (rb != GS_OK) return rb;
  const long long t0 = now_us();
  unsigned spins = 0;
  while (__atomic_load_n(host_pinned, __ATOMIC_ACQUIRE) != 1u) {
    cpu_relax();
    if ((++spins & 1023u) == 0 && now_us() - t0 > kPollTimeoutUs) {
      int r = hip_status(hipStreamSynchronize(st));
      if (r != GS_OK) return r;
      return __atomic_load_n(host_pinned, __ATOMIC_ACQUIRE) == 1u ? GS_OK : GS_ERR_INVALID;
    }
  }
  return GS_OK;
}

inline int read_back(const unsigned* src_dev, unsigned* host_pinned, int n, bool poll, hipStream_t st) {
  return read_back(src_dev, host_pinned, n, poll, st, [] { return GS_OK; });
}

#define CHECK(call)            \
  do {                         \
    int _st = (call);          \
    if (_st != GS_OK) return _st; \
  } while (0)

}

enum { ST_DEPTH_SORT = 0, ST_COUNT_SCAN, ST_PLAN, ST_COUNT, ST_EMIT, ST_TILE_SORT, ST_BIN_EDGES, ST_RASTER_FWD, ST_SAT,
       ST_RASTER_BWD, ST_REDUCE, ST_N };

GS_EXPORT int gs_frame_profile_enable(unsigned stage_mask) {
  g_profile_mask.store(stage_mask, std::memory_order_relaxed);
  return GS_OK;
}

GS_EXPORT int gs_frame_profile_read(int max_events, int* stage_ids, float* ms) {
  int n = 0;
  std::lock_guard<std::mutex> lk(g_profile_mu);
  for (StageEvents& e : g_events) {
    if (n < max_events && stage_ids && ms) {
      (void)hipEventSynchronize(e.b);
      float t = 0.f;
      (void)hipEventElapsedTime(&t, e.a, e.b);
      stage_ids[n] = e.stage;
      ms[n] = t;
      ++n;
    }
    g_pool.push_back(e);
  }
  g_events.clear();
  return n;
}

static long long slice_bytes(const gs_frame_desc& d, long long n_k, long long I_k, bool masks, long long true_total) {
  const long long P = d.P, T = (long long)((d.W + kTile - 1) / kTile) * ((d.H + kTile - 1) / kTile);
  long long b = 0;
  auto add = [&](long long bytes) { b = Arena::up(b) + bytes; };
  if (n_k > 0) {
    add(4 * n_k); add(4 * n_k);
    if (masks) { add(8 * (true_total / 64 + n_k + 2)); add(4 * n_k); }
    add(4 * n_k); add(4); add(gs_scan_workspace_bytes(n_k));
  }
  if (I_k > 0) {
    add(4 * I_k); add(4 * (I_k + kIdsPad));
    add(4 * (I_k + kIdsPad)); add(4 * I_k); add(4 * (I_k + kIdsPad));
    add(4 * (I_k + kIdsPad)); add(4 * (I_k + kIdsPad));
    add(gs_radix_sort_workspace_bytes(I_k, 0, bits_for(P * T + 1)));
    add(8 * (P * T + 1));
  } else {
    add(4); add(8 * (d.shared_list ? (long long)d.S : P) * T);
  }
  add(4ll * d.S * d.H * d.W);
  return Arena::up(b) + 256;
}

GS_EXPORT long long gs_frame_backward_bytes(const gs_frame_state* state) {
  if (!state) return 0;
  long long maxI = 0;
  for (int k = 0; k < state->n_slices; ++k) maxI = std::max(maxI, state->slice[k].I);
  const long long tpe = state->shared_list ? state->S : 1;
  long long b = Arena::up(48 * maxI * tpe) + Arena::up(maxI * tpe) + 512;
  if (state->n_slices > 1) b += 2 * Arena::up(4ll * state->S * state->H * state->W);
  return b;
}

GS_EXPORT int gs_frame_forward(const gs_frame_desc* dp, float* records, unsigned* depth_keys, const int* num_tiles_hit,
                               const float* background, const int* band_edges, const unsigned char* band_tile_done,
                               const float* color_means, const float* color_sh, const float* color_sh_rest, int color_K,
                               int color_degree,
                               const float* color_viewmats, const float* pix_vel, const float* sample_times,
                               float* out_img, float* out_T,
                               float* out_depth, float* out_combined, void* arena_ptr, long long arena_bytes, void* host_pinned, long long host_pinned_bytes,
                               gs_frame_state* state, void* stream_) {
  if (!dp || !records || !depth_keys || !num_tiles_hit || !background || !band_edges || !out_img || !out_T ||
      !arena_ptr || !host_pinned || !state)
    return GS_ERR_INVALID;
  const gs_frame_desc d = *dp;
  const bool shared = d.shared_list != 0;
  if (d.N <= 0 || d.P <= 0 || d.S <= 0 || d.R <= 0 || d.H <= 0 || d.W <= 0 || d.P > 256 || d.S > 256) return GS_ERR_INVALID;
  if (shared ? (d.P != 1 || d.R != 1 || !pix_vel || !sample_times) : (d.P != d.S * d.R)) return GS_ERR_INVALID;
  if (d.R > 1 && !band_tile_done) return GS_ERR_INVALID;
  if ((long long)d.S * d.H * d.W >= (1ll << 30)) return GS_ERR_INVALID;
  const int cams = d.cameras > 1 ? d.cameras : 1;
  if (cams > 1 && (d.S % cams != 0 || shared || pix_vel)) return GS_ERR_INVALID;
  const bool rs = pix_vel != nullptr && (d.rolling_shutter_time != 0.f || shared);
  if (rs && d.R != 1) return GS_ERR_INVALID;
  const gs_project_inputs* lazy = d.lazy_records;
  if (lazy && (pix_vel || shared)) return GS_ERR_INVALID;
  hipStream_t st = (hipStream_t)stream_;
  const int P = d.P, N = d.N, S = d.S, R = d.R, H = d.H, W = d.W;
  const long long n = (long long)P * N;
  const int tx = (W + kTile - 1) / kTile, ty = (H + kTile - 1) / kTile;
  const long long T = (long long)tx * ty;
  const long long plan_ints = 2ll * P * kKMax + 2 * P + 1;
  if (host_pinned_bytes < 4 * (plan_ints + 1) + 64) return GS_ERR_INVALID;
  memset(state, 0, sizeof(*state));
  state->P = P; state->N = N; state->S = S; state->R = R; state->H = H; state->W = W;
  state->cameras = cams;
  state->rolling_shutter_time = rs ? d.rolling_shutter_time : 0.f;
  state->shared_list = shared ? 1 : 0;
  Arena A(arena_ptr, arena_bytes);

  const bool planned = d.slice_base > 0;
  const bool select = planned && d.depth_select != 0;
  unsigned* k0s = select ? A.take<unsigned>(n) : nullptr;
  unsigned* v0 = A.take<unsigned>(n);
  unsigned* k1 = A.take<unsigned>(n);
  unsigned* v1 = A.take<unsigned>(n);
  unsigned* counts_r = A.take<unsigned>(n);
  unsigned* n_live = A.take<unsigned>(P);
  const int digit = d.depth_sort_digit >= 8 && d.depth_sort_digit <= 11 ? d.depth_sort_digit : 8;
  const long long sort_ws_b = gs_segmented_sort_compact_workspace_bytes(n, N, 0, 31, digit);
  char* sort_ws = A.take<char>(sort_ws_b);
  unsigned* cum = A.take<unsigned>(n);
  unsigned* total = A.take<unsigned>(1);
  const long long scan_ws_b = gs_scan_workspace_bytes(n);
  char* scan_ws = A.take<char>(scan_ws_b);
  float* live_T = A.take<float>((long long)S * H * W);
  int* sat = A.take<int>((long long)P * (ty + 1) * (tx + 1));
  const long long w64 = (tx + 63) / 64;
  unsigned long long* open_bits = A.take<unsigned long long>((long long)P * ty * w64);
  const long long sel_b = select ? Arena::up(gs_depth_select_workspace_bytes(P)) + 256 : 0;
  const long long flag_off = ((1 + kKMax) * P * T + 3) & ~3ll;
  char* zero_blk = A.take<char>(sel_b + flag_off + 4 * kKMax);
  unsigned char* zeros_u8 = reinterpret_cast<unsigned char*>(zero_blk) + sel_b;
  unsigned* sel_grand = reinterpret_cast<unsigned*>(zero_blk + sel_b - 256);
  unsigned* thr_dev = select ? A.take<unsigned>(P) : nullptr;
  int* plan_dev = A.take<int>(plan_ints);
  unsigned char* tile_done_rs = R > 1 ? A.take<unsigned char>(P * T) : nullptr;
  unsigned char* tile_done_samples = shared ? A.take<unsigned char>((long long)S * T) : nullptr;
  if (!A.ok) { state->arena_required = 2 * A.off; return GS_ERR_WORKSPACE; }
  if (shared) CHECK(hip_status(hipMemsetAsync(tile_done_samples, 0, (long long)S * T, st)));
  CHECK(hip_status(hipMemsetAsync(zero_blk, 0, sel_b + flag_off + 4 * kKMax, st)));
  int* open_flags = reinterpret_cast<int*>(zeros_u8 + flag_off);
  const long long plan_tiles = (d.band_clipped && R > 1) ? (T + R - 1) / R : T;
  const long long base0 = plan_tiles * (long long)std::max(1, d.slice_base);

  const unsigned* sorted_gi = nullptr;
  bool bound_known = false;
  auto presort = [&](int phase, long long tail_cap) -> int {
    int res = 0;
    {
      StageScope sc(ST_DEPTH_SORT, st);
      if (!select) {
        CHECK(gs_segmented_sort_compact_u32(n, N, depth_keys, v0, k1, v1, 0, 31, digit, 0xFFFFFFFFu, n_live,
                                            reinterpret_cast<const unsigned*>(num_tiles_hit), counts_r, sort_ws, sort_ws_b,
                                            &res, st));
      } else {
        if (phase == 0 && !bound_known) {
          CHECK(gs_depth_select(n, N, depth_keys, reinterpret_cast<const unsigned*>(num_tiles_hit), base0, thr_dev,
                                sel_grand, zero_blk, sel_b - 256, st));
          bound_known = true;
        }
        CHECK(gs_segmented_sort_select_u32(n, N, depth_keys, k0s, v0, k1, v1, 0, 31, digit, 0xFFFFFFFFu,
                                           phase == 0 ? nullptr : thr_dev, phase == 0 ? thr_dev : nullptr, n_live,
                                           reinterpret_cast<const unsigned*>(num_tiles_hit), counts_r, sort_ws, sort_ws_b,
                                           &res, phase == 0 ? tail_cap : 0, st));
      }
    }
    sorted_gi = res == 1 ? v1 : v0;
    StageScope sc(ST_COUNT_SCAN, st);
    CHECK(gs_exclusive_scan_segments_u32(n, N, n_live, counts_r, cum, total, scan_ws, scan_ws_b, st));
    return GS_OK;
  };
  long long tail_cap = (select && d.select_cap > 0) ? (long long)d.select_cap : 0;
  CHECK(presort(0, tail_cap));

  unsigned* hp = reinterpret_cast<unsigned*>(host_pinned) + 1;
  unsigned* hp_seq = reinterpret_cast<unsigned*>(host_pinned);
  const bool poll = d.poll_readback != 0;
  const long long PK = (long long)P * kKMax;
  std::vector<long long> NV(P), seg_totals(P);
  std::vector<std::vector<long long>> bnd(P), rel(P);
  long long n_total = 0, true_total = 0;
  int K = 1;
  bool use_masks = false, rs_exact = false;
  std::vector<std::vector<int>> begins, prefixes;
  std::vector<long long> n_of, I_of;
  auto make_plan = [&](int phase) -> int {
    if (planned) {
      StageScope sc(ST_PLAN, st);
      if (select && phase == 0)
        CHECK(gs_slice_plan_select(P, N, kKMax, cum, total, plan_dev, reinterpret_cast<unsigned*>(plan_dev + PK),
                                   reinterpret_cast<unsigned*>(plan_dev + 2 * PK), n_live,
                                   reinterpret_cast<unsigned*>(plan_dev + 2 * PK + P), sel_grand, st));
      else
        CHECK(gs_slice_plan(P, N, kKMax, cum, total, phase == 0 ? base0 : 2 * base0, plan_dev,
                            reinterpret_cast<unsigned*>(plan_dev + PK), reinterpret_cast<unsigned*>(plan_dev + 2 * PK),
                            n_live, reinterpret_cast<unsigned*>(plan_dev + 2 * PK + P), st));
      CHECK(read_back(reinterpret_cast<const unsigned*>(plan_dev), hp_seq, (int)plan_ints, poll, st));
      for (int p = 0; p < P; ++p) {
        bnd[p].resize(kKMax); rel[p].resize(kKMax);
        for (int k = 0; k < kKMax; ++k) { bnd[p][k] = hp[p * kKMax + k]; rel[p][k] = hp[PK + p * kKMax + k]; }
        seg_totals[p] = hp[2 * PK + p];
        NV[p] = std::min<long long>(N, hp[2 * PK + P + p]);
      }
      if (phase == 0) n_total = hp[plan_ints - 1];
      const int k_cap = phase == 0 ? kKMax : kKMax - 1;
      K = k_cap;
      for (int k = 0; k < k_cap; ++k) {
        bool all = true;
        for (int p = 0; p < P; ++p) all = all && bnd[p][k] >= NV[p];
        if (all) { K = k + 1; break; }
      }
    } else {
      CHECK(hip_status(hipMemcpyAsync(hp, total, 4, hipMemcpyDeviceToHost, st)));
      CHECK(hip_status(hipMemcpyAsync(hp + 1, n_live, 4 * P, hipMemcpyDeviceToHost, st)));
      CHECK(hip_status(hipStreamSynchronize(st)));
      n_total = hp[0];
      for (int p = 0; p < P; ++p) { NV[p] = std::min<long long>(N, hp[1 + p]); seg_totals[p] = 0; }
      K = 1;
    }
    true_total = 0;
    for (int p = 0; p < P; ++p) true_total += seg_totals[p];
    use_masks = planned && true_total < 4294967296ll - 64;
    rs_exact = rs && use_masks;
    if (rs && !rs_exact) use_masks = false;
    begins.assign(K, std::vector<int>(P));
    prefixes.assign(K, std::vector<int>(P + 1));
    n_of.assign(K, 0); I_of.assign(K, 0);
    for (int k = 0; k < K; ++k) {
      prefixes[k][0] = 0;
      long long I_k = 0;
      for (int p = 0; p < P; ++p) {
        const long long lo = k == 0 ? 0 : std::min(bnd[p].empty() ? NV[p] : bnd[p][k - 1], NV[p]);
        const long long hi = (k == K - 1) ? NV[p] : std::min(bnd[p][k], NV[p]);
        begins[k][p] = (int)((long long)p * N + lo);
        prefixes[k][p + 1] = prefixes[k][p] + (int)std::max(0ll, hi - lo);
        if (planned) {
          const long long hi_rel = (k == K - 1) ? seg_totals[p] : rel[p][k];
          const long long lo_rel = k == 0 ? 0 : rel[p][k - 1];
          I_k += (hi_rel - lo_rel) & 0xFFFFFFFFll;
        }
      }
      n_of[k] = prefixes[k][P];
      I_of[k] = planned ? I_k : n_total;
      if (n_of[k] == 0) I_of[k] = 0;
    }
    return GS_OK;
  };
  CHECK(make_plan(0));
  if (tail_cap > 0) {
    long long most = 0;
    for (int p = 0; p < P; ++p) most = std::max(most, NV[p]);
    if (most > tail_cap) {
      state->select_overflow = 1;
      CHECK(presort(0, 0));
      CHECK(make_plan(0));
    }
  }
  for (int p = 0; p < P; ++p) state->max_selected = std::max<long long>(state->max_selected, select ? NV[p] : 0);
  state->n_total = n_total;
  state->depth_select = select ? 1 : 0;
  state->open_after_first = -1.f;
  bool rest_behind = select && ((n_total - true_total) & 0xFFFFFFFFll) != 0;

  long long maxI_issued = 0;
  auto fits = [&](long long n_s, long long I_s, int k_next) -> bool {
    if (I_s >= 2147483647ll - kIdsPad) return false;
    const long long mI = std::max(maxI_issued, I_s);
    const long long tpe = shared ? S : 1;
    const long long bwd = d.reserve_backward ? Arena::up(48 * mI * tpe) + Arena::up(mI * tpe) + 2 * Arena::up(4ll * S * H * W) + 1024 : 0;
    const long long need = Arena::up(A.off) + slice_bytes(d, n_s, I_s, use_masks, true_total) + bwd;
    if (need <= arena_bytes) return true;
    state->arena_required = need + (k_next < K && I_of[k_next] < 2147483647ll
                                        ? slice_bytes(d, n_of[k_next], I_of[k_next], use_masks, true_total) + 49 * I_of[k_next]
                                        : 0);
    return false;
  };
  auto merged = [&](int k0, int k1, std::vector<int>& beg, std::vector<int>& pre, long long& n_s, long long& I_s) {
    beg = begins[k0];
    pre.assign(P + 1, 0);
    I_s = 0;
    for (int p = 0; p < P; ++p) {
      int cnt = 0;
      for (int k = k0; k < k1; ++k) cnt += prefixes[k][p + 1] - prefixes[k][p];
      pre[p + 1] = pre[p] + cnt;
    }
    for (int k = k0; k < k1; ++k) I_s += I_of[k];
    n_s = pre[P];
    if (n_s == 0) I_s = 0;
  };

  unsigned char* tile_done = zeros_u8;
  const bool holes0 = R > 1;
  if (R > 1) {
    tile_done = tile_done_rs;
    CHECK(hip_status(hipMemcpyAsync(tile_done, band_tile_done, P * T, hipMemcpyDeviceToDevice, st)));
    CHECK(gs_tile_open_sat(P, H, W, tile_done, sat, open_bits, nullptr, st));
  }
  const unsigned invalid_key = rs ? 0u : (unsigned)(P * T);
  const int key_bits = bits_for(P * T + 1);
  int n_out = 0;
  int span = 1;
  long long open_before = (long long)S * T;
  std::vector<int> beg_s, pre_s;
  int slice_no = 0;
  bool lazy_done = false;
  for (int phase = 0; phase < 2; ++phase) {
  long long open_left = 0;
  for (int k = 0, k1 = 0; k < K; k = k1, ++slice_no) {
    long long n_k = 0, I_k = 0;
    k1 = std::min(K, k + span);
    merged(k, k1, beg_s, pre_s, n_k, I_k);
    while (k1 > k + 1 && I_k >= 2147483647ll - kIdsPad) merged(k, --k1, beg_s, pre_s, n_k, I_k);
    const bool first = slice_no == 0, last = k1 == K && !(phase == 0 && rest_behind);
    if (I_k >= 2147483647ll - kIdsPad) return GS_ERR_INVALID;
    if (shared && I_k * (long long)S >= 4294967296ll) return GS_ERR_INVALID;
    if (!fits(n_k, I_k, k1)) return GS_ERR_WORKSPACE;
    maxI_issued = std::max(maxI_issued, I_k);
    unsigned *slice_gi = nullptr, *counts = nullptr, *cum_k = nullptr, *total_k = nullptr, *mask_off = nullptr;
    unsigned long long* masks = nullptr;
    unsigned *vals = nullptr, *svals = nullptr, *sorted_ids = nullptr;
    int* bins = nullptr;
    unsigned char* tile_hot = zeros_u8 + (1 + slice_no) * P * T;
    int wave_per_g = 0;
    if (n_k > 0) {
      StageScope sc(ST_COUNT, st);
      slice_gi = A.take<unsigned>(n_k);
      counts = A.take<unsigned>(n_k);
      const bool have_holes = !first || holes0;
      long long box_total = 0;
      if (first) {
        if (!planned) box_total = n_total;
        else if (K == 1) box_total = true_total;
        else for (int p = 0; p < P; ++p) box_total += rel[p][0];
      }
      wave_per_g = (first && box_total > 128 * n_k) ? 1 : 0;
      if (use_masks) {
        masks = A.take<unsigned long long>(true_total / 64 + n_k + 2);
        mask_off = A.take<unsigned>(n_k);
      }
      cum_k = A.take<unsigned>(n_k);
      total_k = A.take<unsigned>(1);
      const long long ws_b = gs_scan_workspace_bytes(n_k);
      char* ws = A.take<char>(ws_b);
      if (!A.ok) { state->arena_required = 2 * A.off; return GS_ERR_WORKSPACE; }
      if (lazy && !lazy_done) {
        if (slice_no == 0)
          CHECK(gs_slice_project_records((int)n_k, P, N, beg_s.data(), pre_s.data(), sorted_gi, lazy, H, W, records, st));
        else {
          CHECK(gs_project_records(P, N, lazy, H, W, records, st));
          lazy_done = true;
        }
      }
      if (rs_exact)
        CHECK(gs_slice_counts_exact_swept((int)n_k, P, N, beg_s.data(), pre_s.data(), sorted_gi, records,
                                          have_holes ? sat : nullptr, have_holes ? tile_done : nullptr, H, W, slice_gi,
                                          counts, wave_per_g, cum, masks, mask_off, have_holes ? open_bits : nullptr,
                                          pix_vel, shared ? d.sweep_t_min : 0.f, shared ? d.sweep_t_max : 0.f,
                                          d.rolling_shutter_time, st));
      else if (rs)
        CHECK(gs_slice_counts((int)n_k, P, N, beg_s.data(), pre_s.data(), sorted_gi, records,
                              have_holes ? sat : nullptr, H, W, slice_gi, counts, st));
      else
        CHECK(gs_slice_counts_exact((int)n_k, P, N, beg_s.data(), pre_s.data(), sorted_gi, records,
                                    have_holes ? sat : nullptr, have_holes ? tile_done : nullptr, H, W, slice_gi, counts,
                                    wave_per_g, masks ? cum : nullptr, masks, mask_off, have_holes ? open_bits : nullptr,
                                    nullptr, st));
      CHECK(gs_exclusive_scan_u32(n_k, counts, cum_k, total_k, ws, ws_b, st));
      if (color_means && color_sh && color_viewmats)
        CHECK(gs_slice_colors((int)n_k, slice_gi, counts, N, color_means, color_sh, color_sh_rest, color_K, color_degree,
                              color_viewmats, records, st));
    }
    if (I_k > 0) {
      unsigned* keys = A.take<unsigned>(I_k);
      vals = A.take<unsigned>(I_k + kIdsPad);
      unsigned* s_v0 = A.take<unsigned>(I_k + kIdsPad);
      unsigned* s_k1 = A.take<unsigned>(I_k);
      unsigned* s_v1 = A.take<unsigned>(I_k + kIdsPad);
      unsigned* pa = A.take<unsigned>(I_k + kIdsPad);
      unsigned* pb = A.take<unsigned>(I_k + kIdsPad);
      const long long ws_b = gs_radix_sort_workspace_bytes(I_k, 0, key_bits);
      char* ws = A.take<char>(ws_b);
      bins = A.take<int>(2 * (P * T + 1));
      if (!A.ok) { state->arena_required = 2 * A.off; return GS_ERR_WORKSPACE; }
      {
        StageScope sc(ST_EMIT, st);
        if (rs && !rs_exact && first && !holes0)
          CHECK(gs_emit_intersects(n_k, N, H, W, slice_gi, cum_k, records, I_k, keys, vals, invalid_key, st));
        else
          CHECK(gs_emit_open_intersects((int)n_k, N, H, W, slice_gi, counts, cum_k, records,
                                        (!first || holes0) ? tile_done : nullptr, keys, vals, invalid_key,
                                        (rs && !rs_exact) ? 0 : 1, wave_per_g, masks, mask_off, rs ? nullptr : tile_hot, st));
      }
      int r1 = 0, r2 = 0;
      {
        StageScope sc(ST_TILE_SORT, st);
        CHECK(gs_radix_sort_pairs_carry_u32(I_k, keys, s_v0, s_k1, s_v1, 1, 0, key_bits, ws, ws_b, &r1, vals, pa, pb, &r2,
                                            total_k, st));
      }
      const unsigned* skeys = r1 == 1 ? s_k1 : keys;
      svals = r1 == 1 ? s_v1 : s_v0;
      sorted_ids = r2 == 1 ? pb : pa;
      {
        StageScope sc(ST_BIN_EDGES, st);
        CHECK(gs_tile_bin_edges_u32(I_k, skeys, (int)(P * T + 1), bins, total_k, st));
      }
    }
    if (I_k == 0 && !(first || last)) continue;
    if (I_k == 0) {
      const long long nb = (shared ? (long long)S : (long long)P) * T;
      svals = A.take<unsigned>(1 + kIdsPad);
      bins = A.take<int>(2 * nb);
      if (!A.ok) { state->arena_required = 2 * A.off; return GS_ERR_WORKSPACE; }
      CHECK(hip_status(hipMemsetAsync(svals, 0, 4 * (1 + kIdsPad), st)));
      CHECK(hip_status(hipMemsetAsync(bins, 0, 8 * nb, st)));
    }
    int* fidx = A.take<int>((long long)S * H * W);
    if (!A.ok) { state->arena_required = 2 * A.off; return GS_ERR_WORKSPACE; }
    const int fwd_variant = (I_k == 0 && d.fwd_variant == 3) ? 0 : d.fwd_variant;
    {
      StageScope sc(ST_RASTER_FWD, st);
      if (rs && I_k > 0)
        CHECK(gs_rasterize_fwd_rs_slice(records, bins, band_edges, background, S, H, W, out_img, out_T, live_T, fidx,
                                        shared ? tile_done_samples : tile_done, first ? 1 : 0, last ? 1 : 0,
                                        reinterpret_cast<const int*>(sorted_ids), (int)std::min(n, 2147483647ll), out_depth,
                                        last ? nullptr : open_flags + slice_no, pix_vel, N, d.rolling_shutter_time,
                                        shared ? sample_times : nullptr, st));
      else
      CHECK(gs_rasterize_fwd_slice(records, reinterpret_cast<const int*>(svals), bins, band_edges, background, S, R, H, W,
                                   out_img, out_T, live_T, fidx, shared ? tile_done_samples : tile_done, first ? 1 : 0,
                                   last ? 1 : 0, I_k > 0 ? reinterpret_cast<const int*>(vals) : nullptr,
                                   reinterpret_cast<const int*>(sorted_ids), I_k > 0 ? (int)std::min(n, 2147483647ll) : 0,
                                   I_k > 0 ? out_depth : nullptr, I_k > 0 ? tile_hot : nullptr,
                                   last ? nullptr : open_flags + slice_no, fwd_variant, st));
    }
    if (I_k > 0) {
      if (n_out >= GS_FRAME_MAX_SLICES) return GS_ERR_INVALID;
      gs_frame_slice& sl = state->slice[n_out++];
      sl.I = I_k; sl.n = (int)n_k; sl.wave_per_gaussian = wave_per_g; sl.first = first; sl.last = last;
      sl.svals = A.offset_of(svals); sl.bins = A.offset_of(bins); sl.fidx = A.offset_of(fidx);
      sl.gi_of_e = A.offset_of(vals); sl.sorted_ids = A.offset_of(sorted_ids); sl.slice_gi = A.offset_of(slice_gi);
      sl.counts = A.offset_of(counts); sl.cum = A.offset_of(cum_k); sl.tile_hot = A.offset_of(tile_hot);
      sl.n_emitted_dev = A.offset_of(total_k);
    }
    auto average = [&]() -> int {
      if (!out_combined) return GS_OK;
      if (cams > 1)
        return gs_combine_fwd_batched(cams, S / cams, 3ll * H * W, out_img, d.combine_gamma, d.combine_min_level,
                                      out_combined, st);
      return gs_combine_fwd(S, 3ll * H * W, out_img, d.combine_gamma, d.combine_min_level, out_combined, st);
    };
    if (last) CHECK(average());
    if (!last) {
      CHECK(read_back(reinterpret_cast<const unsigned*>(open_flags + slice_no), hp_seq, 1, poll, st, average));
      const long long open_now = hp[0];
      open_left = open_now;
      if (slice_no == 0) state->open_after_first = (float)((double)open_now / (double)((long long)S * T));
      if (open_now == 0) { ++slice_no; break; }
      span = (d.merge_open_fraction > 0.f && (double)open_now >= (double)d.merge_open_fraction * (double)open_before)
                 ? 2 * (k1 - k) : 1;
      open_before = open_now;
      StageScope sc(ST_SAT, st);
      if (shared)
        hipLaunchKernelGGL(and_tile_done_kernel, dim3((unsigned)((T + 255) / 256)), dim3(256), 0, st, S, (int)T,
                           tile_done_samples, tile_done);
      CHECK(gs_tile_open_sat(P, H, W, tile_done, sat, open_bits, nullptr, st));
    }
  }
  if (!(phase == 0 && rest_behind && open_left > 0)) break;
  state->depth_select = 2;
  rest_behind = false;
  span = 1;
  CHECK(presort(1, 0));
  CHECK(make_plan(1));
  }
  state->n_slices = n_out;
  state->arena_used = Arena::up(A.off);
  return GS_OK;
}

GS_EXPORT int gs_frame_backward_depth(const gs_frame_state* state, const float* records, const float* background,
                                      const int* band_edges, const float* out_T, const float* v_img, const float* v_alpha,
                                      const float* cmb_scale, float cmb_gamma, float cmb_min_level, int bwd_variant,
                                      float* v_records, unsigned char* touched, const float* pix_vel,
                                      const float* sample_times, void* arena_ptr, long long arena_bytes,
                                      const float* v_depth, void* stream_) {
  if (!state || !records || !background || !band_edges || !out_T || !v_img || !v_records || !arena_ptr)
    return GS_ERR_INVALID;
  hipStream_t st = (hipStream_t)stream_;
  const int S = state->S, R = state->R, H = state->H, W = state->W;
  const long long n_rec = (long long)state->P * state->N;
  Arena A(arena_ptr, arena_bytes, state->arena_used);
  char* base = (char*)arena_ptr;
  long long maxI = 0;
  for (int k = 0; k < state->n_slices; ++k) maxI = std::max(maxI, state->slice[k].I);
  float *bwd_T = nullptr, *bwd_B = nullptr;
  if (state->n_slices > 1) {
    bwd_T = A.take<float>((long long)S * H * W);
    bwd_B = A.take<float>((long long)S * H * W);
  }
  const bool shared = state->shared_list != 0;
  if (shared && (!pix_vel || !sample_times)) return GS_ERR_INVALID;
  if ((bwd_variant & GS_BWD_ABSGRAD) && (state->rolling_shutter_time != 0.f || shared)) return GS_ERR_INVALID;
  const long long tpe = shared ? S : 1;
  float* tuples = A.take<float>(12 * maxI * tpe);
  unsigned char* flags = A.take<unsigned char>((maxI * tpe + 15) & ~15ll);
  if (!A.ok) return GS_ERR_WORKSPACE;
  if (bwd_T) {
    CHECK(hip_status(hipMemcpyAsync(bwd_T, out_T, 4ll * S * H * W, hipMemcpyDeviceToDevice, st)));
    CHECK(hip_status(hipMemsetAsync(bwd_B, 0, 4ll * S * H * W, st)));
  }
  for (int k = state->n_slices - 1; k >= 0; --k) {
    const gs_frame_slice& sl = state->slice[k];
    CHECK(hip_status(hipMemsetAsync(flags, 0, (sl.I * tpe + 15) & ~15ll, st)));
    {
      StageScope sc(ST_RASTER_BWD, st);
      if (state->rolling_shutter_time != 0.f || shared) {
        if (!pix_vel) return GS_ERR_INVALID;
        CHECK(gs_rasterize_bwd_rs_slice_depth(records, reinterpret_cast<const int*>(base + sl.svals),
                                        reinterpret_cast<const int*>(base + sl.bins), band_edges, background, S, H, W, out_T,
                                        reinterpret_cast<const int*>(base + sl.fidx), v_img, v_alpha, bwd_T, bwd_B, tuples,
                                        flags, reinterpret_cast<const int*>(base + sl.sorted_ids),
                                        (int)std::min(n_rec, 2147483647ll), bwd_variant & 256, cmb_scale, cmb_gamma,
                                        cmb_min_level, pix_vel, state->N, state->rolling_shutter_time,
                                        shared ? sample_times : nullptr, v_depth, st));
      } else
      CHECK(gs_rasterize_bwd_slice_depth(records, reinterpret_cast<const int*>(base + sl.svals),
                                   reinterpret_cast<const int*>(base + sl.bins), band_edges, background, S, R, H, W, out_T,
                                   reinterpret_cast<const int*>(base + sl.fidx), v_img, v_alpha, bwd_T, bwd_B, v_records,
                                   reinterpret_cast<const int*>(base + sl.gi_of_e), tuples, flags,
                                   reinterpret_cast<const int*>(base + sl.sorted_ids), (int)std::min(n_rec, 2147483647ll),
                                   reinterpret_cast<const unsigned char*>(base + sl.tile_hot), bwd_variant, cmb_scale,
                                   cmb_gamma, cmb_min_level, v_depth, state->cameras, st));
    }
    {
      StageScope sc(ST_REDUCE, st);
      CHECK(gs_reduce_grad_tuples_depth(sl.n, reinterpret_cast<const unsigned*>(base + sl.slice_gi),
                                  reinterpret_cast<const unsigned*>(base + sl.counts),
                                  reinterpret_cast<const unsigned*>(base + sl.cum), tuples, flags, v_records, touched,
                                  (sl.wave_per_gaussian || (R > 1 && sl.n < (1 << 19))) ? sl.I : 0, records, (int)tpe,
                                  v_depth != nullptr, st));
    }
  }
  return GS_OK;
}

GS_EXPORT int gs_frame_backward(const gs_frame_state* state, const float* records, const float* background,
                                const int* band_edges, const float* out_T, const float* v_img, const float* v_alpha,
                                const float* cmb_scale, float cmb_gamma, float cmb_min_level, int bwd_variant,
                                float* v_records, unsigned char* touched, const float* pix_vel,
                                const float* sample_times, void* arena_ptr, long long arena_bytes, void* stream_) {
  return gs_frame_backward_depth(state, records, background, band_edges, out_T, v_img, v_alpha, cmb_scale, cmb_gamma,
                                 cmb_min_level, bwd_variant, v_records, touched, pix_vel, sample_times, arena_ptr,
                                 arena_bytes, nullptr, stream_);
}
```

3dgs-deblur_amd/ops.py:

```python
from __future__ import annotations

import ctypes
import math
from typing import Optional, Tuple

import torch
from torch import Tensor
from torch.autograd import Function

from . import _lib

import os
import threading

TILE = 16
REC = 16
GRAD = 12
MAX_SUBPOSES = 256
SLICE_BASE = int(os.environ.get("GSD_SLICE_BASE", "512"))
SLICE_ADAPT = int(os.environ.get("GSD_SLICE_ADAPT", "1"))
SLICE_GROW_OPEN = float(os.environ.get("GSD_SLICE_GROW_OPEN", "0.5"))
_state_lock = threading.RLock()


class FrameHints:

    __slots__ = ("mult", "age", "arena_bytes", "arena_retries", "frames", "box_share", "last_slices", "select_misses",
                 "select_cap", "select_overflows", "_recent", "_lock", "_views")

    def __init__(self):
        self.mult, self.age, self.arena_bytes, self.arena_retries, self.frames = 1, 0, 0, 0, 0
        self.box_share = None
        self.last_slices = None
        self.select_misses = 0
        self.select_cap = 0
        self.select_overflows = 0
        self._recent = []
        self._lock = threading.Lock()
        self._views = {}

    def slice_base(self) -> int:
        return SLICE_BASE * (self.mult if SLICE_ADAPT and SLICE_BASE > 0 else 1)

    def feedback(self, n_issued: int, retries: int = 0, box_share: Optional[float] = None, select_state: int = 0,
                 open_after_first: Optional[float] = None, max_selected: int = 0, select_overflow: int = 0) -> None:
        with self._lock:
            self.frames += 1
            self.last_slices = int(n_issued)
            if select_state == 2:
                self.select_misses += 1
            if max_selected > 0:
                want = int(1.5 * max_selected) + 4096
                self.select_cap = want if (select_overflow or want > self.select_cap) else max(want, int(0.9 * self.select_cap))
            self.select_overflows += int(bool(select_overflow))
            if box_share is not None:
                self.box_share = float(box_share)
            self.arena_retries += retries
            self._recent = (self._recent + [(int(n_issued), self.mult, int(retries))])[-4:]
            if SLICE_ADAPT and SLICE_BASE > 0:
                grow = n_issued >= 2 and self.mult < 8 and (open_after_first is None or open_after_first < 0
                                                            or open_after_first >= SLICE_GROW_OPEN)
                if self.age >= 255:
                    self.mult, self.age = 1, 0
                else:
                    self.mult, self.age = (self.mult * 2 if grow else self.mult), self.age + 1

    @property
    def settled(self) -> bool:
        with self._lock:
            r = self._recent
            return (len(r) >= 2 and r[-1][0] == r[-2][0] and r[-1][1] == r[-2][1] == self.mult
                    and r[-1][2] == 0 and r[-2][2] == 0)

    def lazy_records(self) -> bool:
        return self.mult == 1 and (self.box_share is None or self.box_share < 0.25)

    def depth_select(self) -> bool:
        return self.last_slices == 1 and self.box_share is not None and self.box_share < 0.5

    def view(self, key) -> "ViewHints":
        with self._lock:
            v = self._views.get(key)
            if v is None:
                if len(self._views) >= 16384:
                    self._views.clear()
                v = self._views[key] = ViewHints(self)
                v.box_share, v.last_slices, v.select_cap = self.box_share, self.last_slices, self.select_cap
            return v

    def reset(self) -> None:
        with self._lock:
            self.mult, self.age, self.arena_bytes, self._recent, self.box_share = 1, 0, 0, [], None
            self.last_slices, self.select_cap = None, 0
            self._views.clear()


class ViewHints:

    __slots__ = ("scene", "box_share", "last_slices", "select_cap")

    def __init__(self, scene: "FrameHints"):
        self.scene = scene
        self.box_share, self.last_slices, self.select_cap = None, None, 0

    arena_bytes = property(lambda self: self.scene.arena_bytes,
                           lambda self, v: setattr(self.scene, "arena_bytes", v))
    mult = property(lambda self: self.scene.mult)
    frames = property(lambda self: self.scene.frames)
    arena_retries = property(lambda self: self.scene.arena_retries)
    select_misses = property(lambda self: self.scene.select_misses)
    select_overflows = property(lambda self: self.scene.select_overflows)
    settled = property(lambda self: self.scene.settled)

    def slice_base(self) -> int:
        return self.scene.slice_base()

    def lazy_records(self) -> bool:
        return self.scene.mult == 1 and (self.box_share is None or self.box_share < 0.25)

    def depth_select(self) -> bool:
        return self.last_slices == 1 and self.box_share is not None and self.box_share < 0.5

    def view(self, key) -> "ViewHints":
        return self.scene.view(key)

    def feedback(self, n_issued: int, retries: int = 0, box_share: Optional[float] = None, select_state: int = 0,
                 open_after_first: Optional[float] = None, max_selected: int = 0, select_overflow: int = 0) -> None:
        sc = self.scene
        with sc._lock:
            self.last_slices = int(n_issued)
            if box_share is not None:
                self.box_share = float(box_share)
            if max_selected > 0:
                want = int(1.5 * max_selected) + 4096
                self.select_cap = want if (select_overflow or want > self.select_cap) else max(want, int(0.9 * self.select_cap))
        sc.feedback(n_issued, retries, box_share, select_state, open_after_first, max_selected, select_overflow)


_hints = {}


def hints_for(key) -> FrameHints:
    with _state_lock:
        h = _hints.get(key)
        if h is None:
            if len(_hints) >= 64:
                _hints.clear()
            h = _hints[key] = FrameHints()
        return h


SLICE_MERGE = float(os.environ.get("GSD_SLICE_MERGE", "0.75"))
FRAME_POLL = int(os.environ.get("GSD_FRAME_POLL", "1"))


def _host_cores() -> int:
    try:
        return len(os.sched_getaffinity(0))
    except (AttributeError, OSError):
        return os.cpu_count() or 1


def frame_poll() -> int:
    if "GSD_FRAME_POLL" in os.environ or not FRAME_POLL:
        return int(FRAME_POLL)
    local_world = max(1, int(os.environ.get("LOCAL_WORLD_SIZE", "1") or 1))
    return 1 if _host_cores() >= 2 * local_world else 0


def readback_mode() -> dict:
    return {"poll": bool(frame_poll()), "host_cores": _host_cores(),
            "local_rank": int(os.environ.get("LOCAL_RANK", "0") or 0),
            "local_world": int(os.environ.get("LOCAL_WORLD_SIZE", "1") or 1),
            "forced": "GSD_FRAME_POLL" in os.environ}
DEPTH_SORT_DIGIT = 8
UPSTREAM_GRADS = int(os.environ.get("GSD_UPSTREAM_GRADS", "6"))


BAND_AWARE = int(os.environ.get("GSD_BAND_AWARE", "1"))
LAZY_RECORDS = int(os.environ.get("GSD_LAZY_RECORDS", "1"))
DEPTH_SELECT = int(os.environ.get("GSD_DEPTH_SELECT", "1"))
NEEDLE_HP = int(os.environ.get("GSD_NEEDLE_HP", "1"))


def _proj_grad_flags() -> int:
    return (UPSTREAM_GRADS & 1) | (0 if NEEDLE_HP else 8)


BWD_SPLAT = int(os.environ.get("GSD_BWD_SPLAT", "0"))


BWD_ABSGRAD = 2048


def _bwd_variant(absgrad: bool = False) -> int:
    if absgrad:
        return (256 if (UPSTREAM_GRADS & 4) else 0) | BWD_ABSGRAD
    return (256 if (UPSTREAM_GRADS & 4) else 0) | (1024 if BWD_SPLAT else 0)
_slice_totals = []


def __getattr__(name):
    if name == "last_slice_intersects":
        for i, v in enumerate(_slice_totals):
            if isinstance(v, torch.Tensor):
                _slice_totals[i] = int(v.item()) & 0xFFFFFFFF
        return list(_slice_totals)
    raise AttributeError(name)


from ._profile import FRAME_STAGES, StageProfiler, _NULL

profiler: Optional[StageProfiler] = None
last_num_intersects: int = 0
last_depth_select: int = 0


def _stage(name: str):
    return _NULL if profiler is None else profiler.stage(name)


def _L():
    return _lib.load()


def _ptr(t: Optional[Tensor]):
    return None if t is None else ctypes.c_void_p(t.data_ptr())


def _stream():
    return ctypes.c_void_p(torch.cuda.current_stream().cuda_stream)


def _f32(t: Tensor, name: str) -> Tensor:
    if not t.is_cuda:
        raise ValueError(f"{name} must be a CUDA(HIP) tensor: the HIP path has no CPU fallback")
    if t.dtype != torch.float32:
        raise ValueError(f"{name} must be float32, got {t.dtype}")
    return t.contiguous()


def _tiles(h: int, w: int) -> Tuple[int, int]:
    return (w + TILE - 1) // TILE, (h + TILE - 1) // TILE


IDS_PAD = 8


def _padded_i32(n: int, dev) -> Tensor:
    return torch.empty(n + IDS_PAD, dtype=torch.int32, device=dev)[:n]


def _bits(n: int) -> int:
    return max(1, int(math.ceil(math.log2(max(2, n)))))


SYNC_CHECK = int(os.environ.get("GSD_SYNC_CHECK", "0"))


def _check(st: int, what: str):
    _lib.check(st, what)
    if SYNC_CHECK:
        try:
            torch.cuda.synchronize()
        except RuntimeError as e:
            raise _lib.HipLibraryError(f"asynchronous HIP fault surfaced right after stage '{what}': {e}") from e


def _pose_scratch(N: int, P: int, with_touched: bool, dev) -> Tensor:
    return torch.empty(int(_L().gs_project_pose_scratch_bytes(int(N), int(P), int(bool(with_touched)))), dtype=torch.uint8,
                       device=dev)


def _viewmat16(viewmat: Tensor) -> Tensor:
    v = _f32(viewmat, "viewmat")
    if v.shape[-2:] == (3, 4):
        pad = torch.tensor([[0.0, 0.0, 0.0, 1.0]], device=v.device, dtype=v.dtype)
        v = torch.cat([v, pad.expand(v.shape[:-2] + (1, 4))], dim=-2).contiguous()
    if v.shape[-2:] != (4, 4):
        raise ValueError("viewmat must be [4,4] (or [3,4])")
    return v


def exclusive_scan_u32(x: Tensor) -> Tuple[Tensor, Tensor]:
    assert x.dtype == torch.int32 and x.is_cuda and x.is_contiguous()
    n = x.numel()
    out = torch.empty_like(x)
    if n == 0:
        return out, torch.zeros(1, dtype=torch.int32, device=x.device)
    total = torch.empty(1, dtype=torch.int32, device=x.device)
    ws_bytes = _L().gs_scan_workspace_bytes(n)
    ws = torch.empty(ws_bytes, dtype=torch.uint8, device=x.device)
    _check(_L().gs_exclusive_scan_u32(n, _ptr(x), _ptr(out), _ptr(total), _ptr(ws), ws_bytes, _stream()), "scan")
    return out, total


def radix_sort_pairs(keys: Tensor, vals: Optional[Tensor], begin_bit: int, end_bit: int,
                     gather_src: Optional[Tensor] = None, n_dev: Optional[Tensor] = None,
                     carry: Optional[Tensor] = None):
    assert keys.is_cuda and keys.is_contiguous() and keys.dtype in (torch.int32, torch.int64)
    n = keys.numel()
    dev = keys.device
    if vals is None:
        v0 = _padded_i32(n, dev)
        iota = 1
    else:
        assert vals.dtype == torch.int32 and vals.is_contiguous() and vals.numel() == n
        v0, iota = vals, 0
    if n == 0:
        return keys, v0
    k1 = torch.empty_like(keys)
    v1 = _padded_i32(n, dev)
    L = _L()
    ws_bytes = L.gs_radix_sort_workspace_bytes(n, begin_bit, end_bit)
    ws = torch.empty(ws_bytes, dtype=torch.uint8, device=dev)
    res = ctypes.c_int(0)
    if carry is not None:
        assert keys.dtype == torch.int32 and carry.dtype == torch.int32 and carry.is_contiguous() and gather_src is None
        assert carry.numel() >= n
        pa, pb = _padded_i32(n, dev), _padded_i32(n, dev)
        res2 = ctypes.c_int(0)
        _check(L.gs_radix_sort_pairs_carry_u32(n, _ptr(keys), _ptr(v0), _ptr(k1), _ptr(v1), iota, begin_bit, end_bit,
                                               _ptr(ws), ws_bytes, ctypes.byref(res), _ptr(carry), _ptr(pa), _ptr(pb),
                                               ctypes.byref(res2), _ptr(n_dev), _stream()), "radix sort + carry")
        return ((k1, v1) if res.value == 1 else (keys, v0)) + (pb if res2.value == 1 else pa,)
    if gather_src is not None:
        assert keys.dtype == torch.int32 and gather_src.dtype == torch.int32 and gather_src.is_contiguous()
        gathered = _padded_i32(n, dev)
        _check(L.gs_radix_sort_pairs_gather_u32(n, _ptr(keys), _ptr(v0), _ptr(k1), _ptr(v1), iota, begin_bit, end_bit,
                                                _ptr(ws), ws_bytes, ctypes.byref(res), _ptr(gather_src), _ptr(gathered),
                                                _ptr(n_dev), _stream()), "radix sort + gather")
        return ((k1, v1) if res.value == 1 else (keys, v0)) + (gathered,)
    fn = L.gs_radix_sort_pairs_u32 if keys.dtype == torch.int32 else L.gs_radix_sort_pairs_u64
    _check(fn(n, _ptr(keys), _ptr(v0), _ptr(k1), _ptr(v1), iota, begin_bit, end_bit, _ptr(ws), ws_bytes,
              ctypes.byref(res), _stream()), "radix sort")
    return (k1, v1) if res.value == 1 else (keys, v0)


def bin_and_sort_records(records: Tensor, depth_keys: Tensor, num_tiles_hit: Tensor, P: int, N: int,
                         img_height: int, img_width: int, with_emission: bool = False):
    L = _L()
    dev = records.device
    n = P * N
    tx, ty = _tiles(img_height, img_width)
    T = tx * ty
    global last_num_intersects
    with _stage("depth_sort"):
        keys64 = torch.empty(n, dtype=torch.int64, device=dev)
        _check(L.gs_make_depth_keys64(n, N, _ptr(depth_keys), _ptr(keys64), _stream()), "depth keys")
        end_bit = 32 + (_bits(P) if P > 1 else 0)
        _, sorted_gi = radix_sort_pairs(keys64, None, 0, end_bit)
    with _stage("count_scan"):
        counts = torch.empty(n, dtype=torch.int32, device=dev)
        _check(L.gs_gather_counts(n, _ptr(sorted_gi), _ptr(num_tiles_hit), _ptr(counts), _stream()), "gather counts")
        cum, total = exclusive_scan_u32(counts)
    n_isect = int(total.item())
    last_num_intersects = n_isect
    bins = torch.empty(P * T, 2, dtype=torch.int32, device=dev)
    if n_isect == 0:
        bins.zero_()
        z = torch.zeros(1, dtype=torch.int32, device=dev)
        return (z, bins, 0, z.clone()) + ((None,) if with_emission else ())
    if n_isect < 0:
        raise OverflowError("more than 2^31-1 tile intersections; chunk the sub-poses")
    with _stage("emit"):
        keys = torch.empty(n_isect, dtype=torch.int32, device=dev)
        vals = _padded_i32(n_isect, dev)
        _check(L.gs_emit_intersects(n, N, img_height, img_width, _ptr(sorted_gi), _ptr(cum), _ptr(records), n_isect,
                                    _ptr(keys), _ptr(vals), 0, _stream()), "emit intersects")
    extra = None
    with _stage("tile_sort"):
        if with_emission:
            skeys, eids, svals = radix_sort_pairs(keys, None, 0, _bits(P * T), carry=vals)
            extra = dict(eids=eids, sorted_gi=sorted_gi, counts=counts, cum=cum)
        else:
            skeys, svals = radix_sort_pairs(keys, vals, 0, _bits(P * T))
    with _stage("bin_edges"):
        _check(L.gs_tile_bin_edges_u32(n_isect, _ptr(skeys), P * T, _ptr(bins), None, _stream()), "bin edges")
    return (svals, bins, n_isect, skeys) + ((extra,) if with_emission else ())


_band_edge_cache = {}


def _band_edges(img_height: int, rs_bands: int, device) -> Tensor:
    key = (int(img_height), max(1, int(rs_bands)), str(device))
    t = _band_edge_cache.get(key)
    if t is None:
        _, ty = _tiles(img_height, 1)
        R = key[1]
        t = torch.tensor([(r * ty) // R for r in range(R + 1)], dtype=torch.int32, device=device)
        if len(_band_edge_cache) > 64:
            _band_edge_cache.clear()
        _band_edge_cache[key] = t
    return t


_placeholder_cache = {}


def _placeholder_i32(dev) -> Tensor:
    t = _placeholder_cache.get(str(dev))
    if t is None:
        t = _placeholder_cache[str(dev)] = torch.zeros(1, dtype=torch.int32, device=dev)
    return t


_band_done_cache = {}


def _band_tile_done(S: int, R: int, ty: int, tx: int, dev) -> Tensor:
    key = (S, R, ty, tx, str(dev))
    t = _band_done_cache.get(key)
    if t is None:
        e = [(r * ty) // R for r in range(R + 1)]
        rows = torch.arange(ty, device=dev)
        band_open = torch.stack([(rows >= e[r]) & (rows < e[r + 1]) for r in range(R)])
        t = (~band_open).to(torch.uint8)[None, :, :, None].expand(S, R, ty, tx).reshape(-1).contiguous()
        if len(_band_done_cache) > 16:
            _band_done_cache.clear()
        _band_done_cache[key] = t
    return t


def _background(background: Optional[Tensor], device) -> Tensor:
    if background is None:
        return torch.zeros(3, dtype=torch.float32, device=device)
    bg = background.detach().to(device=device, dtype=torch.float32).contiguous()
    if bg.numel() != 3:
        raise ValueError("background must have 3 channels")
    return bg


frame_backend = None


class _FrameDesc(ctypes.Structure):
    _fields_ = [(k, ctypes.c_int) for k in ("N", "P", "S", "R", "H", "W", "slice_base", "depth_sort_digit",
                                             "fwd_variant", "reserve_backward")] + [("merge_open_fraction", ctypes.c_float),
                                                                                     ("rolling_shutter_time", ctypes.c_float),
                                                                                     ("poll_readback", ctypes.c_int),
                                                                                     ("shared_list", ctypes.c_int),
                                                                                     ("combine_gamma", ctypes.c_float),
                                                                                     ("combine_min_level", ctypes.c_float),
                                                                                     ("band_clipped", ctypes.c_int),
                                                                                     ("depth_select", ctypes.c_int),
                                                                                     ("select_cap", ctypes.c_int),
                                                                                     ("sweep_t_min", ctypes.c_float),
                                                                                     ("sweep_t_max", ctypes.c_float),
                                                                                     ("lazy_records", ctypes.c_void_p),
                                                                                     ("cameras", ctypes.c_int)]


class _ProjectInputs(ctypes.Structure):
    _fields_ = ([(k, ctypes.c_void_p) for k in ("means", "scales", "quats", "opacities", "viewmats")] +
                [(k, ctypes.c_float) for k in ("glob_scale", "fx", "fy", "cx", "cy", "clip_thresh")] +
                [(k, ctypes.c_int) for k in ("antialiased", "defer_color", "param_flags")])


class _FrameSlice(ctypes.Structure):
    _fields_ = ([("I", ctypes.c_longlong)] + [(k, ctypes.c_int) for k in ("n", "wave_per_gaussian", "first", "last")] +
                [(k, ctypes.c_longlong) for k in ("svals", "bins", "fidx", "gi_of_e", "sorted_ids", "slice_gi", "counts",
                                                  "cum", "tile_hot", "n_emitted_dev")])


class _FrameState(ctypes.Structure):
    _fields_ = ([(k, ctypes.c_int) for k in ("n_slices", "P", "N", "S", "R", "H", "W")] +
                [("rolling_shutter_time", ctypes.c_float), ("shared_list", ctypes.c_int), ("depth_select", ctypes.c_int),
                 ("select_overflow", ctypes.c_int), ("open_after_first", ctypes.c_float)] +
                [(k, ctypes.c_longlong) for k in ("n_total", "max_selected", "arena_used", "arena_required")] +
                [("slice", _FrameSlice * 16), ("cameras", ctypes.c_int)])


def _box_share(state) -> Optional[float]:
    n_total = int(state.n_total)
    if n_total <= 0:
        return None
    held = sum(int(state.slice[i].I) for i in range(int(state.n_slices)))
    return min(1.0, held / n_total)


class _ArenaTooSmall(Exception):
    pass


_ARENA_ATTEMPTS = 16
_arena_pool = {}


class _Arena:
    __slots__ = ("tensor", "gen")

    def __init__(self, tensor):
        self.tensor, self.gen = tensor, 0

    def numel(self):
        return self.tensor.numel()

    def data_ptr(self):
        return self.tensor.data_ptr()


_lease_counter = 0


class _ArenaLease:
    __slots__ = ("arena", "key", "gen")

    def __init__(self, arena: _Arena, key):
        global _lease_counter
        self.arena, self.key = arena, key
        with _state_lock:
            _lease_counter += 1
            self.gen = arena.gen = _lease_counter

    @property
    def tensor(self):
        a = self.arena
        return None if a is None else a.tensor

    def release(self):
        try:
            with _state_lock:
                a, self.arena = self.arena, None
                if a is None:
                    return
                free = _arena_pool.setdefault(self.key, [])
                free.append(a)
                if len(free) > 2:
                    free.remove(min(free, key=lambda x: x.numel()))
        except Exception:
            pass

    __del__ = release


def _arena_acquire(dev, want_bytes: int) -> _ArenaLease:
    key = (str(dev), torch.cuda.current_stream(dev).cuda_stream)
    with _state_lock:
        free = _arena_pool.setdefault(key, [])
        free[:] = [x if isinstance(x, _Arena) else _Arena(x) for x in free]
        a = max(free, key=lambda x: x.numel()) if free else None
        if a is not None:
            free.remove(a)
    if a is None or a.numel() < want_bytes:
        a = None
        a = _Arena(torch.empty(int(want_bytes), dtype=torch.uint8, device=dev))
    return _ArenaLease(a, key)


def _arena_relend(frame) -> bool:
    a = frame["arena_obj"]
    with _state_lock:
        free = _arena_pool.get(frame["lease"].key, [])
        if a.gen != frame["gen"] or a not in free:
            raise RuntimeError("this frame's arena was handed back after its first backward and a later frame has "
                               "used it since: a second backward of one frame (retain_graph=True) must run before "
                               "the next frame's forward")
        free.remove(a)
    return True


def _arena_return(frame) -> None:
    with _state_lock:
        free = _arena_pool.setdefault(frame["lease"].key, [])
        free.append(frame["arena_obj"])
        if len(free) > 2:
            free.remove(min(free, key=lambda x: x.numel()))


def release_arenas() -> None:
    with _state_lock:
        _arena_pool.clear()


_pinned_cache = {}


def _profile_mask() -> int:
    if profiler is None:
        return 0
    names = FRAME_STAGES if profiler.only is None else [n for n in FRAME_STAGES if n in profiler.only]
    return sum(1 << FRAME_STAGES.index(n) for n in names)


def native_frame_forward(records: Tensor, depth_keys: Tensor, num_tiles_hit: Tensor, P: int, N: int, S: int, R: int,
                         H: int, W: int, bg: Tensor, edges: Tensor, slice_base: int, color=None,
                         out_depth: Optional[Tensor] = None, reserve_backward: bool = True, rs=None, combine=None,
                         hints: Optional[FrameHints] = None, band_clipped: bool = False, lazy=None,
                         depth_select: Optional[bool] = None, cameras: int = 1):
    global last_num_intersects, _slice_totals, last_depth_select
    L = _L()
    dev = records.device
    tx, ty = _tiles(H, W)
    shared = rs is not None and len(rs) > 2 and rs[2] is not None
    if hints is None:
        hints = hints_for((str(dev), N, P, S, H, W, shared))
    if depth_select is None:
        depth_select = bool(DEPTH_SELECT == 2 or (DEPTH_SELECT and hints.depth_select()))
    n = P * N
    nbytes = hints.arena_bytes
    if not nbytes:
        I0 = max(1, slice_base) * tx * ty * P
        nbytes = 44 * n + 16 * S * H * W + (80 + (56 * S if shared else 0)) * I0 + (64 << 20)
    lease = _arena_acquire(dev, nbytes)
    arena = lease.tensor
    nbytes = arena.numel()
    pin_key = (str(dev), threading.get_ident(), torch.cuda.current_stream().cuda_stream)
    pin = _pinned_cache.get(pin_key)
    need_pin = 4 * (2 * P * 16 + 2 * P + 2) + 64
    if pin is None or pin.numel() < need_pin:
        pin = _pinned_cache[pin_key] = torch.empty(max(8192, need_pin), dtype=torch.uint8, pin_memory=True)
    desc = _FrameDesc(N, P, S, R, H, W, int(slice_base), DEPTH_SORT_DIGIT, 0, int(reserve_backward),
                      float(SLICE_MERGE), float(rs[1]) if rs is not None else 0.0, frame_poll(), int(shared),
                      float(combine[0]) if combine is not None else 1.0, float(combine[1]) if combine is not None else 0.0,
                      int(bool(band_clipped)), int(bool(depth_select and slice_base > 0)),
                      int(min(hints.select_cap, 2 ** 31 - 1)) if depth_select else 0,
                      float(rs[3][0]) if shared and len(rs) > 3 else 0.0, float(rs[3][1]) if shared and len(rs) > 3 else 0.0,
                      ctypes.addressof(lazy) if lazy is not None else None, int(cameras))
    state = _FrameState()
    out_img = torch.empty(S, H, W, 3, device=dev)
    out_T = torch.empty(S, H, W, device=dev)
    band_done = _band_tile_done(S, R, ty, tx, dev) if R > 1 else None
    c_means = c_sh = c_rest = c_V = None
    c_K = c_deg = 0
    if color is not None:
        c_means, c_sh, c_rest, c_K, c_deg, c_V = color
    L.gs_frame_profile_enable(_profile_mask())
    st = L.gs_frame_forward(ctypes.byref(desc), _ptr(records), _ptr(depth_keys), _ptr(num_tiles_hit), _ptr(bg), _ptr(edges),
                            _ptr(band_done), _ptr(c_means), _ptr(c_sh), _ptr(c_rest), int(c_K), int(c_deg), _ptr(c_V),
                            _ptr(rs[0]) if rs is not None else None, _ptr(rs[2]) if shared else None, _ptr(out_img),
                            _ptr(out_T), _ptr(out_depth), _ptr(combine[2]) if combine is not None else None,
                            _ptr(arena), arena.numel(), ctypes.c_void_p(pin.data_ptr()), pin.numel(), ctypes.byref(state),
                            _stream())
    if st == 3:
        hints.arena_bytes = max(int(state.arena_required * 1.15) + (32 << 20), int(nbytes * 1.5))
        raise _ArenaTooSmall()
    _check(st, "frame_forward")
    hints.arena_bytes = max(int(hints.arena_bytes),
                            int((state.arena_used + L.gs_frame_backward_bytes(ctypes.byref(state))) * 1.15))
    last_num_intersects = int(state.n_total)
    last_depth_select = int(state.depth_select)
    _slice_totals = [arena[sl.n_emitted_dev:sl.n_emitted_dev + 4].view(torch.int32)
                     for sl in (state.slice[i] for i in range(state.n_slices))]
    return out_img, out_T, dict(arena=arena, arena_obj=lease.arena, lease=lease, gen=lease.gen, state=state,
                                pix_vel=rs[0] if rs is not None else None,
                                sample_times=rs[2] if shared else None)


def native_frame_backward(frame, records: Tensor, bg: Tensor, edges: Tensor, out_T: Tensor, v_img: Tensor,
                          v_alpha: Optional[Tensor], v_records: Tensor, touched: Tensor, combine=None,
                          v_depth: Optional[Tensor] = None, absgrad: bool = False):
    L = _L()
    cmb = combine if combine is not None else (None, 1.0, 0.0)
    arena, state = frame["arena"], frame["state"]
    lease = frame["lease"]
    relent = lease.arena is None and _arena_relend(frame)
    try:
        _native_frame_backward(L, frame, arena, state, records, bg, edges, out_T, v_img, v_alpha, v_records, touched, cmb,
                               v_depth, absgrad)
    finally:
        if relent:
            _arena_return(frame)
        else:
            lease.release()


def _native_frame_backward(L, frame, arena, state, records, bg, edges, out_T, v_img, v_alpha, v_records, touched, cmb,
                           v_depth=None, absgrad=False):
    L.gs_frame_profile_enable(_profile_mask())
    if v_depth is None:
        st = L.gs_frame_backward(ctypes.byref(state), _ptr(records), _ptr(bg), _ptr(edges), _ptr(out_T), _ptr(v_img),
                                 _ptr(v_alpha), _ptr(cmb[0]), float(cmb[1]), float(cmb[2]), _bwd_variant(absgrad),
                                 _ptr(v_records), _ptr(touched), _ptr(frame.get("pix_vel")), _ptr(frame.get("sample_times")), _ptr(arena),
                                 arena.numel(), _stream())
    else:
        st = L.gs_frame_backward_depth(ctypes.byref(state), _ptr(records), _ptr(bg), _ptr(edges), _ptr(out_T),
                                       _ptr(v_img), _ptr(v_alpha), _ptr(cmb[0]), float(cmb[1]), float(cmb[2]),
                                       _bwd_variant(absgrad), _ptr(v_records), _ptr(touched),
                                       _ptr(frame.get("pix_vel")),
                                       _ptr(frame.get("sample_times")), _ptr(arena), arena.numel(), _ptr(v_depth),
                                       _stream())
    if st == 3:
        raise _lib.HipLibraryError("frame_backward: the forward's arena cannot hold the backward's buffers "
                                   "(call native_frame_forward with reserve_backward=True)")
    _check(st, "frame_backward")


class _ProjectGaussians(Function):
    @staticmethod
    def forward(ctx, means3d, scales, glob_scale, quats, viewmat, fx, fy, cx, cy, img_height, img_width,
                block_width, clip_thresh):
        if block_width != TILE:
            raise ValueError("only block_width=16 is supported")
        means3d, scales, quats = _f32(means3d, "means3d"), _f32(scales, "scales"), _f32(quats, "quats")
        V = _viewmat16(viewmat)
        N = means3d.shape[0]
        dev = means3d.device
        xys = torch.empty(N, 2, device=dev)
        depths = torch.empty(N, device=dev)
        radii = torch.empty(N, dtype=torch.int32, device=dev)
        conics = torch.empty(N, 3, device=dev)
        comp = torch.empty(N, device=dev)
        ntiles = torch.empty(N, dtype=torch.int32, device=dev)
        cov3d = torch.empty(N, 6, device=dev)
        _check(_L().gs_project_fwd(N, _ptr(means3d), _ptr(scales), float(glob_scale), _ptr(quats), _ptr(V),
                                   float(fx), float(fy), float(cx), float(cy), int(img_height), int(img_width),
                                   float(clip_thresh), _ptr(xys), _ptr(depths), _ptr(radii), _ptr(conics),
                                   _ptr(comp), _ptr(ntiles), _ptr(cov3d), None, _stream()), "project_fwd")
        ctx.save_for_backward(means3d, scales, quats, V)
        ctx.args = (float(glob_scale), float(fx), float(fy), float(cx), float(cy), int(img_height),
                    int(img_width), float(clip_thresh))
        ctx.mark_non_differentiable(radii, ntiles)
        return xys, depths, radii, conics, comp, ntiles, cov3d

    @staticmethod
    def backward(ctx, v_xys, v_depths, v_radii, v_conics, v_comp, v_ntiles, v_cov3d):
        means3d, scales, quats, V = ctx.saved_tensors
        glob, fx, fy, cx, cy, H, W, clip = ctx.args
        N = means3d.shape[0]
        dev = means3d.device

        def z(g, shape):
            return torch.zeros(shape, device=dev) if g is None else g.contiguous().float()
        v_xys, v_depths, v_conics, v_comp = z(v_xys, (N, 2)), z(v_depths, (N,)), z(v_conics, (N, 3)), z(v_comp, (N,))
        v_means = torch.empty(N, 3, device=dev)
        v_scales = torch.empty(N, 3, device=dev)
        v_quats = torch.empty(N, 4, device=dev)
        need_v = ctx.needs_input_grad[4]
        v_V = torch.zeros(4, 4, device=dev) if need_v else None
        scratch = _pose_scratch(N, 1, False, dev) if need_v else None
        _check(_L().gs_project_bwd(N, _ptr(means3d), _ptr(scales), glob, _ptr(quats), _ptr(V), fx, fy, cx, cy, H, W,
                                   clip, _ptr(v_xys), _ptr(v_depths), _ptr(v_conics), _ptr(v_comp), _ptr(v_means),
                                   _ptr(v_scales), _ptr(v_quats), _ptr(v_V), UPSTREAM_GRADS & 3, _ptr(scratch),
                                   0 if scratch is None else scratch.numel(), _stream()),
               "project_bwd")
        return (v_means, v_scales, None, v_quats, v_V, None, None, None, None, None, None, None, None)


def project_gaussians(means3d: Tensor, scales: Tensor, glob_scale: float, quats: Tensor, viewmat: Tensor,
                      fx: float, fy: float, cx: float, cy: float, img_height: int, img_width: int,
                      block_width: int = TILE, clip_thresh: float = 0.01, *, lin_vel: Optional[Tensor] = None,
                      ang_vel: Optional[Tensor] = None, exposure_time: float = 0.0, rolling_shutter_time: float = 0.0,
                      blur_samples: int = 0):
    if lin_vel is None and ang_vel is None:
        return _ProjectGaussians.apply(means3d, scales, glob_scale, quats, viewmat, fx, fy, cx, cy, img_height,
                                       img_width, block_width, clip_thresh)
    if lin_vel is None or ang_vel is None:
        raise ValueError("lin_vel and ang_vel go together")
    if block_width != TILE:
        raise ValueError("only block_width=16 is supported")
    from . import velocity_ops as VO
    _, _, span = VO.sample_span(blur_samples, exposure_time, rolling_shutter_time)
    return VO.ProjectGaussiansPixvel.apply(means3d, scales, glob_scale, quats, viewmat, fx, fy, cx, cy, img_height,
                                           img_width, clip_thresh, lin_vel, ang_vel, span)


class _SphericalHarmonics(Function):
    @staticmethod
    def forward(ctx, degrees_to_use, viewdirs, coeffs):
        viewdirs, coeffs = _f32(viewdirs, "viewdirs"), _f32(coeffs, "coeffs")
        N, K = coeffs.shape[0], coeffs.shape[1]
        colors = torch.empty(N, 3, device=coeffs.device)
        _check(_L().gs_sh_fwd(N, K, int(degrees_to_use), _ptr(viewdirs), _ptr(coeffs), _ptr(colors), _stream()),
               "sh_fwd")
        ctx.save_for_backward(viewdirs)
        ctx.K, ctx.deg = K, int(degrees_to_use)
        return colors

    @staticmethod
    def backward(ctx, v_colors):
        (viewdirs,) = ctx.saved_tensors
        N = viewdirs.shape[0]
        v_coeffs = torch.empty(N, ctx.K, 3, device=viewdirs.device)
        _check(_L().gs_sh_bwd(N, ctx.K, ctx.deg, _ptr(viewdirs), _ptr(v_colors.contiguous().float()),
                              _ptr(v_coeffs), _stream()), "sh_bwd")
        return None, None, v_coeffs


def spherical_harmonics(degrees_to_use: int, viewdirs: Tensor, coeffs: Tensor) -> Tensor:
    return _SphericalHarmonics.apply(degrees_to_use, viewdirs, coeffs)


class _RasterizeGaussians(Function):
    @staticmethod
    def forward(ctx, xys, depths, radii, conics, num_tiles_hit, colors, opacity, img_height, img_width,
                block_width, background, return_alpha):
        if block_width != TILE:
            raise ValueError("only block_width=16 is supported")
        assert colors.shape[-1] == 3
        xys, depths, conics = _f32(xys, "xys"), _f32(depths, "depths"), _f32(conics, "conics")
        colors, opacity = _f32(colors, "colors"), _f32(opacity, "opacity").reshape(-1)
        radii = radii.to(torch.int32).contiguous()
        N = xys.shape[0]
        dev = xys.device
        H, W = int(img_height), int(img_width)
        L = _L()
        records = torch.empty(N, REC, device=dev)
        dkeys = torch.empty(N, dtype=torch.int32, device=dev)
        ntiles = torch.empty(N, dtype=torch.int32, device=dev)
        _check(L.gs_pack_records(N, _ptr(xys), _ptr(depths), _ptr(radii), _ptr(conics), _ptr(colors), _ptr(opacity),
                                 H, W, _ptr(records), _ptr(dkeys), _ptr(ntiles), _stream()), "pack_records")
        svals, bins, n_isect, _ = bin_and_sort_records(records, dkeys, ntiles, 1, N, H, W)
        bg = _background(background, dev)
        edges = _band_edges(H, 1, dev)
        out_img = torch.empty(1, H, W, 3, device=dev)
        out_T = torch.empty(1, H, W, device=dev)
        fidx = torch.empty(1, H, W, dtype=torch.int32, device=dev)
        _check(L.gs_rasterize_fwd(_ptr(records), _ptr(svals), _ptr(bins), _ptr(edges), _ptr(bg), 1, 1, H, W,
                                  _ptr(out_img), _ptr(out_T), _ptr(fidx), N if n_isect > 0 else 0, 0,
                                  _stream()), "rasterize_fwd")
        ctx.save_for_backward(records, svals, bins, edges, bg, out_T, fidx)
        ctx.dims = (N, H, W)
        ctx.bg_grad = background is not None and ctx.needs_input_grad[10]
        out = out_img[0]
        if return_alpha:
            return out, 1.0 - out_T[0]
        return out

    @staticmethod
    def backward(ctx, v_img, v_alpha=None):
        records, svals, bins, edges, bg, out_T, fidx = ctx.saved_tensors
        N, H, W = ctx.dims
        dev = records.device
        L = _L()
        v_img = v_img.contiguous().float()
        v_al = None if v_alpha is None else v_alpha.contiguous().float()
        v_records = torch.zeros(N, GRAD, device=dev)
        _check(L.gs_rasterize_bwd(_ptr(records), _ptr(svals), _ptr(bins), _ptr(edges), _ptr(bg), 1, 1, H, W,
                                  _ptr(out_T), _ptr(fidx), _ptr(v_img), _ptr(v_al), _ptr(v_records), N, _bwd_variant(),
                                  _stream()), "rasterize_bwd")
        v_xys = torch.empty(N, 2, device=dev)
        v_conics = torch.empty(N, 3, device=dev)
        v_colors = torch.empty(N, 3, device=dev)
        v_opacity = torch.empty(N, 1, device=dev)
        _check(L.gs_unpack_record_grads(N, _ptr(v_records), _ptr(v_xys), _ptr(v_conics), _ptr(v_colors),
                                        _ptr(v_opacity), _stream()), "unpack grads")
        v_bg = (out_T[0][..., None] * v_img).sum(dim=(0, 1)) if ctx.bg_grad else None
        return (v_xys, None, None, v_conics, None, v_colors, v_opacity, None, None, None, v_bg, None)


def rasterize_gaussians(xys: Tensor, depths: Tensor, radii: Tensor, conics: Tensor, num_tiles_hit: Tensor,
                        colors: Tensor, opacity: Tensor, img_height: int, img_width: int, block_width: int = TILE,
                        background: Optional[Tensor] = None, return_alpha: bool = False, *,
                        pix_vels: Optional[Tensor] = None, exposure_time: float = 0.0, rolling_shutter_time: float = 0.0,
                        blur_samples: int = 0, return_samples: bool = False):
    if pix_vels is not None:
        if block_width != TILE:
            raise ValueError("only block_width=16 is supported")
        if colors.shape[-1] != 3:
            raise ValueError("rasterize_gaussians with pix_vels composites 3 channels")
        from . import velocity_ops as VO
        _, times, span = VO.sample_span(blur_samples, exposure_time, rolling_shutter_time)
        img, alpha = VO.RasterizeGaussiansPixvel.apply(xys, depths, radii, conics, colors, opacity.reshape(-1, 1), pix_vels,
                                                       int(img_height), int(img_width), background, times,
                                                       float(rolling_shutter_time), span)
        if not return_samples:
            img, alpha = img.mean(dim=0), alpha.mean(dim=0)
        return (img, alpha) if return_alpha else img
    C = colors.shape[-1]
    if C == 3:
        return _RasterizeGaussians.apply(xys, depths, radii, conics, num_tiles_hit, colors, opacity.reshape(-1, 1),
                                         img_height, img_width, block_width, background, return_alpha)
    if background is not None and background.numel() != C:
        raise ValueError(f"background must have {C} channels")
    imgs, alpha = [], None
    for c0 in range(0, C, 3):
        n = min(3, C - c0)
        col = colors[:, c0:c0 + n]
        bg = None if background is None else background.reshape(-1)[c0:c0 + n]
        if n < 3:
            col = torch.cat([col, col.new_zeros(col.shape[0], 3 - n)], dim=1)
            bg = None if bg is None else torch.cat([bg, bg.new_zeros(3 - n)])
        res = _RasterizeGaussians.apply(xys, depths, radii, conics, num_tiles_hit, col, opacity.reshape(-1, 1),
                                        img_height, img_width, block_width, bg, return_alpha and alpha is None)
        if return_alpha and alpha is None:
            res, alpha = res
        imgs.append(res[..., :n])
    out = torch.cat(imgs, dim=-1)
    return (out, alpha) if return_alpha else out


def compute_cumulative_intersects(num_tiles_hit: Tensor) -> Tuple[int, Tensor]:
    nt = num_tiles_hit.to(torch.int32).contiguous()
    ex, total = exclusive_scan_u32(nt)
    return int(total.item()), ex + nt


def map_gaussian_to_intersects(num_points: int, num_intersects: int, xys: Tensor, depths: Tensor, radii: Tensor,
                               cum_tiles_hit: Tensor, tile_bounds, block_width: int = TILE):
    dev = xys.device
    isect = torch.zeros(max(1, num_intersects), dtype=torch.int64, device=dev)
    gids = torch.zeros(max(1, num_intersects), dtype=torch.int32, device=dev)
    W, H = int(tile_bounds[0]) * TILE, int(tile_bounds[1]) * TILE
    _check(_L().gs_map_gaussian_to_intersects(int(num_points), _ptr(_f32(xys, "xys")), _ptr(_f32(depths, "depths")),
                                              _ptr(radii.to(torch.int32).contiguous()),
                                              _ptr(cum_tiles_hit.to(torch.int32).contiguous()), H, W, _ptr(isect),
                                              _ptr(gids), _stream()), "map_gaussian_to_intersects")
    return isect[:num_intersects], gids[:num_intersects]


def get_tile_bin_edges(num_intersects: int, isect_ids_sorted: Tensor, tile_bounds) -> Tensor:
    T = int(tile_bounds[0]) * int(tile_bounds[1])
    bins = torch.empty(T, 2, dtype=torch.int32, device=isect_ids_sorted.device)
    _check(_L().gs_tile_bin_edges_u64(int(num_intersects), _ptr(isect_ids_sorted.contiguous()), T, _ptr(bins),
                                      _stream()), "tile_bin_edges")
    return bins


def bin_and_sort_gaussians(num_points: int, num_intersects: int, xys: Tensor, depths: Tensor, radii: Tensor,
                           cum_tiles_hit: Tensor, tile_bounds, block_width: int = TILE):
    isect, gids = map_gaussian_to_intersects(num_points, num_intersects, xys, depths, radii, cum_tiles_hit,
                                             tile_bounds, block_width)
    T = int(tile_bounds[0]) * int(tile_bounds[1])
    if num_intersects == 0:
        return isect, gids, isect, gids, torch.zeros(T, 2, dtype=torch.int32, device=xys.device)
    ks, vs = radix_sort_pairs(isect.clone(), gids.clone(), 0, 32 + _bits(T))
    bins = get_tile_bin_edges(num_intersects, ks, tile_bounds)
    return isect, gids, ks, vs, bins


class _SubposeViewmats(Function):
    @staticmethod
    def forward(ctx, viewmat, lin_vel, ang_vel, times):
        V = _viewmat16(viewmat)
        lin, ang, times = _f32(lin_vel, "lin_vel"), _f32(ang_vel, "ang_vel"), _f32(times, "times")
        P = times.numel()
        out = torch.empty(P, 4, 4, device=V.device)
        _check(_L().gs_subpose_viewmats_fwd(P, _ptr(V), _ptr(lin), _ptr(ang), _ptr(times), _ptr(out), _stream()),
               "subpose_viewmats_fwd")
        ctx.save_for_backward(V, lin, ang, times)
        return out

    @staticmethod
    def backward(ctx, v_out):
        V, lin, ang, times = ctx.saved_tensors
        P = times.numel()
        dev = V.device
        acc = torch.zeros(22, device=dev)
        v_V, v_lin, v_ang = acc[:16].view(4, 4), acc[16:19], acc[19:22]
        _check(_L().gs_subpose_viewmats_bwd(P, _ptr(V), _ptr(lin), _ptr(ang), _ptr(times),
                                            _ptr(v_out.contiguous().float()), _ptr(v_V), _ptr(v_lin), _ptr(v_ang),
                                            _stream()), "subpose_viewmats_bwd")
        return v_V, v_lin, v_ang, None

# ... 453 lines not shown
```

include/gsdeblur.h:

```cpp
#ifndef GSDEBLUR_H
#define GSDEBLUR_H

#ifdef __cplusplus
extern "C" {
#endif

#define GS_BWD_ABSGRAD 2048

const char* gs_version(void);

int gs_subpose_viewmats_fwd(int P, const float* viewmat , const float* lin_vel ,
                            const float* ang_vel , const float* times ,
                            float* out_viewmats , void* stream);
int gs_subpose_viewmats_bwd(int P, const float* viewmat, const float* lin_vel, const float* ang_vel,
                            const float* times, const float* v_out , float* v_viewmat,
                            float* v_lin, float* v_ang, void* stream);

int gs_project_fwd(int N, const float* means3d , const float* scales , float glob_scale,
                   const float* quats , const float* viewmat , float fx, float fy,
                   float cx, float cy, int img_height, int img_width, float clip_thresh,
                   float* xys , float* depths , int* radii , float* conics ,
                   float* compensation , int* num_tiles_hit , float* cov3d ,
                   int* tile_bounds , void* stream);
long long gs_project_pose_scratch_bytes(int N, int P, int with_touched);
int gs_project_bwd(int N, const float* means3d, const float* scales, float glob_scale, const float* quats,
                   const float* viewmat, float fx, float fy, float cx, float cy, int img_height,
                   int img_width, float clip_thresh, const float* v_xys, const float* v_depths,
                   const float* v_conics, const float* v_comp, float* v_means3d, float* v_scales,
                   float* v_quats, float* v_viewmat,
                   int grad_flags ,
                   void* pose_scratch ,
                         long long pose_scratch_bytes,
                         void* stream);

int gs_sh_fwd(int N, int K_stride, int degrees_to_use, const float* viewdirs ,
              const float* coeffs, float* colors , void* stream);
int gs_sh_bwd(int N, int K_stride, int degrees_to_use, const float* viewdirs, const float* v_colors,
              float* v_coeffs , void* stream);

int gs_project_fused_fwd(int N, int P, const float* means3d, const float* scales, float glob_scale,
                         const float* quats, const float* opacities ,
                         const float* sh , int K_stride, int sh_degree,
                         const float* viewmats , float fx, float fy, float cx, float cy,
                         int img_height, int img_width, float clip_thresh, int antialiased,
                         int defer_color ,
                         float* records , unsigned* depth_keys ,
                         int* num_tiles_hit , int* radii ,
                         const float* sh_rest ,
                         int param_flags ,
                         void* stream);
int gs_slice_colors(int n_slice, const unsigned* slice_gi, const unsigned* counts, int N, const float* means3d,
                    const float* sh, const float* sh_rest , int K_stride, int sh_degree,
                    const float* viewmats, float* records, void* stream);
int gs_project_fused_bwd(int N, int P, const float* means3d, const float* scales, float glob_scale,
                         const float* quats, const float* opacities, const float* sh, int K_stride,
                         int sh_degree, const float* viewmats, float fx, float fy, float cx, float cy,
                         int img_height, int img_width, float clip_thresh, int antialiased,
                         const float* records, const float* v_records, float* v_means3d, float* v_scales,
                         float* v_quats, float* v_opacities, float* v_sh, float* v_viewmats,
                         const unsigned char* touched ,
                         float* v_xy_sum ,
                         int grad_flags ,
                         const float* sh_rest, int param_flags ,
                         float* v_sh_rest ,
                         void* pose_scratch ,
                         long long pose_scratch_bytes,
                         void* stream);

int gs_project_pixvel_fwd(int N, int P, const float* means3d, const float* scales, float glob_scale,
                          const float* quats, const float* opacities, const float* sh, int K_stride, int sh_degree,
                          const float* viewmat , const float* twist , const float* times ,
                          float fx, float fy, float cx, float cy, int img_height, int img_width, float clip_thresh,
                          int antialiased, int defer_color, float* records, unsigned* depth_keys,
                          int* num_tiles_hit, int* radii, float rolling_shutter_time ,
                          float* pix_vel ,
                          const float* sh_rest, int param_flags , void* stream);
int gs_project_pixvel_bwd(int N, int P, const float* means3d, const float* scales, float glob_scale,
                          const float* quats, const float* opacities, const float* sh, int K_stride, int sh_degree,
                          const float* viewmat, const float* twist, const float* times, float fx, float fy,
                          float cx, float cy, int img_height, int img_width, float clip_thresh, int antialiased,
                          const float* records, const float* v_records, float* v_means3d, float* v_scales,
                          float* v_quats, float* v_opacities, float* v_sh, float* v_viewmat, float* v_twist,
                          const unsigned char* touched, float* v_xy_sum, int grad_flags, const float* sh_rest,
                          int param_flags, float* v_sh_rest , void* pose_scratch ,
                         long long pose_scratch_bytes,
                         void* stream);

int gs_pack_records(int N, const float* xys, const float* depths, const int* radii, const float* conics,
                    const float* colors , const float* opacity , int img_height, int img_width,
                    float* records , unsigned* depth_keys , int* num_tiles_hit ,
                    void* stream);
int gs_unpack_record_grads(int N, const float* v_records, float* v_xys, float* v_conics, float* v_colors,
                           float* v_opacity, void* stream);

long long gs_scan_workspace_bytes(long long n);
long long gs_radix_sort_workspace_bytes(long long n, int begin_bit, int end_bit);
int gs_exclusive_scan_u32(long long n, const unsigned* in, unsigned* out, unsigned* total_out, void* ws,
                          long long ws_bytes, void* stream);
int gs_radix_sort_pairs_u32(long long n, unsigned* keys0, unsigned* vals0, unsigned* keys1,
                            unsigned* vals1, int vals0_is_iota, int begin_bit, int end_bit, void* ws,
                            long long ws_bytes, int* result_buf , void* stream);
int gs_radix_sort_pairs_gather_u32(long long n, unsigned* keys0, unsigned* vals0, unsigned* keys1, unsigned* vals1,
                                   int vals0_is_iota, int begin_bit, int end_bit, void* ws, long long ws_bytes,
                                   int* result_buf , const unsigned* gather_src, unsigned* gather_out,
                                   const unsigned* n_dev ,
                                   void* stream);
int gs_radix_sort_pairs_carry_u32(long long n, unsigned* keys0, unsigned* vals0, unsigned* keys1, unsigned* vals1,
                                  int vals0_is_iota, int begin_bit, int end_bit, void* ws, long long ws_bytes,
                                  int* result_buf , const unsigned* payload2_in, unsigned* payload2_a,
                                  unsigned* payload2_b, int* result_p2 ,
                                  const unsigned* n_dev , void* stream);
int gs_radix_sort_pairs_u64(long long n, unsigned long long* keys0, unsigned* vals0,
                            unsigned long long* keys1, unsigned* vals1, int vals0_is_iota, int begin_bit,
                            int end_bit, void* ws, long long ws_bytes, int* result_buf ,
                            void* stream);
long long gs_segmented_sort_workspace_bytes(long long n, long long seg_len, int begin_bit, int end_bit);
int gs_segmented_sort_pairs_u32(long long n, long long seg_len, unsigned* keys0, unsigned* vals0,
                                unsigned* keys1, unsigned* vals1, int vals0_is_iota, int begin_bit, int end_bit,
                                void* ws, long long ws_bytes, int* result_buf , void* stream);
long long gs_segmented_sort_compact_workspace_bytes(long long n, long long seg_len, int begin_bit, int end_bit,
                                                    int max_digit_bits);
int gs_segmented_sort_compact_u32(long long n, long long seg_len, unsigned* keys0, unsigned* vals0,
                                  unsigned* keys1, unsigned* vals1, int begin_bit, int end_bit,
                                  int max_digit_bits ,
                                  unsigned skip_key,
                                  unsigned* seg_counts , const unsigned* gather_src,
                                  unsigned* gather_out, void* ws, long long ws_bytes, int* result_buf ,
                                  void* stream);
long long gs_depth_select_workspace_bytes(int segments);
int gs_depth_select(long long n, long long seg_len, const unsigned* keys, const unsigned* weights, long long budget,
                    unsigned* thr_out , unsigned* grand_out, void* ws, long long ws_bytes,
                    void* stream);
int gs_segmented_sort_select_u32(long long n, long long seg_len, const unsigned* keys_src, unsigned* keys0,
                                 unsigned* vals0, unsigned* keys1, unsigned* vals1, int begin_bit, int end_bit,
                                 int max_digit_bits, unsigned skip_key, const unsigned* key_lo, const unsigned* key_hi,
                                 unsigned* seg_counts, const unsigned* gather_src, unsigned* gather_out, void* ws,
                                 long long ws_bytes, int* result_buf ,
                                 long long tail_cap ,
                                 void* stream);
int gs_exclusive_scan_segments_u32(long long n, long long seg_len, const unsigned* seg_counts ,
                                   const unsigned* in, unsigned* out, unsigned* total_out , void* ws,
                                   long long ws_bytes, void* stream);
int gs_make_depth_keys64(long long n, int N, const unsigned* depth_keys, unsigned long long* out,
                         void* stream);
int gs_gather_counts(long long n, const unsigned* sorted_gi, const int* num_tiles_hit,
                     unsigned* counts_out, void* stream);
int gs_emit_intersects(long long n_ranked, int N, int img_height, int img_width, const unsigned* sorted_gi,
                       const unsigned* cum_excl, const float* records, long long n_isect, unsigned* keys,
                       unsigned* vals, unsigned invalid_key, void* stream);
int gs_tile_bin_edges_u32(long long n, const unsigned* sorted_keys, int num_bins, int* bins ,
                          const unsigned* n_dev ,
                          void* stream);
int gs_tile_bin_edges_u64(long long n, const unsigned long long* sorted_isect_ids, int num_bins,
                          int* bins , void* stream);
int gs_tile_bin_edges_ids_u32(long long n, const unsigned* sorted_keys, int num_bins, int* bins ,
                              const unsigned* sorted_vals, const unsigned* gi_of_e, unsigned* ids_out ,
                              void* stream);
int gs_map_gaussian_to_intersects(int N, const float* xys, const float* depths, const int* radii,
                                  const int* cum_tiles_hit, int img_height, int img_width,
                                  long long* isect_ids, int* gaussian_ids, void* stream);

int gs_rasterize_fwd(const float* records, const int* sorted_vals, const int* tile_bins,
                     const int* band_edges , const float* background , int S, int R,
                     int img_height, int img_width, float* out_img , float* out_T ,
                     int* final_idx ,
                     int n_records ,
                     int variant ,
                     void* stream);
int gs_rasterize_bwd(const float* records, const int* sorted_vals, const int* tile_bins,
                     const int* band_edges, const float* background, int S, int R, int img_height,
                     int img_width, const float* out_T, const int* final_idx, const float* v_img,
                     const float* v_alpha, float* v_records,
                     int n_records ,
                     int variant ,
                     void* stream);

int gs_slice_plan(int P, int N, int K, const unsigned* cum_excl ,
                  const unsigned* total , long long base,
                  int* bounds , unsigned* rels ,
                  unsigned* seg_totals ,
                  const unsigned* n_live ,
                  unsigned* tail ,
                  void* stream);
int gs_slice_plan_select(int P, int N, int K, const unsigned* cum_excl, const unsigned* total, int* bounds,
                         unsigned* rels, unsigned* seg_totals, const unsigned* n_live, unsigned* tail,
                         const unsigned* grand, void* stream);
int gs_tile_open_sat(int P, int img_height, int img_width, const unsigned char* tile_done, int* sat,
                     unsigned long long* open_bits ,
                     const int* gate ,
                     void* stream);
int gs_slice_counts(int n_slice, int P, int N, const int* slice_begin , const int* slice_prefix ,
                    const unsigned* sorted_gi, const float* records, const int* sat, int img_height,
                    int img_width, unsigned* slice_gi, unsigned* counts, void* stream);
int gs_slice_counts_exact(int n_slice, int P, int N, const int* slice_begin , const int* slice_prefix ,
                          const unsigned* sorted_gi, const float* records, const int* sat,
                          const unsigned char* tile_done, int img_height, int img_width, unsigned* slice_gi,
                          unsigned* counts, int wave_per_gaussian ,
                          const unsigned* cum_rank ,
                          unsigned long long* hit_masks ,
                          unsigned* mask_off ,
                          const unsigned long long* open_bits ,
                          const int* gate ,
                          void* stream);
int gs_slice_counts_exact_swept(int n_slice, int P, int N, const int* slice_begin, const int* slice_prefix,
                                const unsigned* sorted_gi, const float* records, const int* sat,
                                const unsigned char* tile_done, int img_height, int img_width, unsigned* slice_gi,
                                unsigned* counts, int wave_per_gaussian, const unsigned* cum_rank,
                                unsigned long long* hit_masks, unsigned* mask_off, const unsigned long long* open_bits,
                                const float* pix_vel, float t_min, float t_max, float rolling_shutter_time,
                                void* stream);
int gs_emit_open_intersects(int n_slice, int N, int img_height, int img_width, const unsigned* slice_gi,
                            const unsigned* counts, const unsigned* cum_excl, const float* records,
                            const unsigned char* tile_done , unsigned* keys, unsigned* vals,
                            unsigned invalid_key, int compact ,
                            int wave_per_gaussian,
                            const unsigned long long* hit_masks ,
                            const unsigned* mask_off,
                            unsigned char* tile_hot ,
                            void* stream);
int gs_rasterize_fwd_slice(const float* records, const int* sorted_vals, const int* tile_bins,
                           const int* band_edges, const float* background, int S, int R, int img_height,
                           int img_width, float* out_img, float* out_T, float* live_T, int* final_idx,
                           unsigned char* tile_done, int first, int last,
                           const int* gi_of_e ,
                           const int* sorted_ids ,
                           int n_records ,
                           float* out_depth ,
                           const unsigned char* tile_hot ,
                           int* open_flag ,
                           int variant ,
                           void* stream);
int gs_rasterize_fwd_slice_stats(const float* records, const int* sorted_vals, const int* tile_bins,
                                 const int* band_edges, const float* background, int S, int R, int img_height,
                                 int img_width, float* out_img, float* out_T, float* live_T, int* final_idx,
                                 unsigned char* tile_done, int first, int last, const int* gi_of_e, int* open_flag,
                                 unsigned long long* stats, void* stream);
int gs_rasterize_fwd_rs_slice(const float* records, const int* tile_bins, const int* band_edges, const float* background,
                              int S, int img_height, int img_width, float* out_img, float* out_T, float* live_T,
                              int* final_idx, unsigned char* tile_done, int first, int last, const int* sorted_ids,
                              int n_records, float* out_depth, int* open_flag, const float* pix_vel, int N,
                              float rolling_shutter_time,
                              const float* shared_list_times ,
                              void* stream);
int gs_rasterize_bwd_rs_slice(const float* records, const int* sorted_vals, const int* tile_bins, const int* band_edges,
                              const float* background, int S, int img_height, int img_width, const float* out_T,
                              const int* final_idx, const float* v_img, const float* v_alpha, float* bwd_T, float* bwd_B,
                              float* tuples, unsigned char* flags, const int* sorted_ids, int n_records, int variant,
                              const float* cmb_scale, float cmb_gamma, float cmb_min_level, const float* pix_vel, int N,
                              float rolling_shutter_time,
                              const float* shared_list_times ,
                              void* stream);
int gs_rasterize_bwd_slice(const float* records, const int* sorted_vals, const int* tile_bins,
                           const int* band_edges, const float* background, int S, int R, int img_height,
                           int img_width, const float* out_T, const int* final_idx, const float* v_img,
                           const float* v_alpha, float* bwd_T, float* bwd_B, float* v_records,
                           const int* gi_of_e ,
                           float* tuples , unsigned char* flags ,
                           const int* sorted_ids , int n_records,
                           const unsigned char* tile_hot ,
                           int variant ,
                           const float* cmb_scale ,
                           float cmb_gamma, float cmb_min_level, void* stream);

int gs_reduce_grad_tuples(int n_slice, const unsigned* slice_gi, const unsigned* counts,
                          const unsigned* cum_excl, const float* tuples, const unsigned char* flags,
                          float* v_records, unsigned char* touched ,
                          long long n_isect ,
                          const float* records ,
                          int tuples_per_entry ,
                          void* stream);

int gs_combine_fwd(int S, long long n, const float* samples , float gamma, float min_level,
                   float* out , void* stream);
int gs_combine_bwd(int S, long long n, const float* samples, float gamma, float min_level,
                   const float* out, const float* v_out, float* v_samples , void* stream);
int gs_combine_bwd_scale(int S, long long n, float gamma, const float* out, const float* v_out,
                         float* scale , void* stream);
int gs_combine_fwd_batched(int B, int S, long long n, const float* samples, float gamma, float min_level,
                           float* out, void* stream);
int gs_combine_bwd_batched(int B, int S, long long n, const float* samples, float gamma, float min_level,
                           const float* out, const float* v_out, float* v_samples, void* stream);
int gs_combine_bwd_scale_batched(int B, int S, long long n, float gamma, const float* out, const float* v_out,
                                 float* scale, void* stream);

int gs_dp_row_mask(int N, int n_tensors, float* const* grads, const int* widths,
                   unsigned char* mask , void* stream);
int gs_dp_pack_rows(long long M, const long long* row_idx , int n_tensors,
                    float* const* grads, const int* widths, float* payload , void* stream);
int gs_dp_scatter_add_rows(long long M, const float* payload, int n_tensors, float* const* grads,
                           const int* widths, float scale, void* stream);
int gs_dp_pack_masked_rows(int N, const unsigned char* mask, const int* pos, int cap, int* idx_ws, int n_tensors,
                           float* const* grads, const int* widths, float* payload, void* stream);
int gs_dp_scatter_add_payload(int cap, const float* payload, int n_tensors, float* const* grads, const int* widths,
                              float scale, void* stream);

typedef struct gs_project_inputs {
  const float *means, *scales, *quats, *opacities, *viewmats;
  float glob_scale, fx, fy, cx, cy, clip_thresh;
  int antialiased, defer_color, param_flags;
} gs_project_inputs;
int gs_slice_project_records(int n_slice, int P, int N, const int* slice_begin, const int* slice_prefix,
                             const unsigned* sorted_gi, const gs_project_inputs* in, int img_height, int img_width,
                             float* records, void* stream);
int gs_project_records(int P, int N, const struct gs_project_inputs* in, int img_height, int img_width, float* records,
                       void* stream);

#define GS_FRAME_MAX_SLICES 16
typedef struct gs_frame_desc {
  int N, P, S, R, H, W;
  int slice_base;
  int depth_sort_digit;
  int fwd_variant;
  int reserve_backward;
  float merge_open_fraction;
  float rolling_shutter_time;
  int poll_readback;
  int shared_list;
  float combine_gamma;
  float combine_min_level;
  int band_clipped;
  int depth_select;
  int select_cap;
  float sweep_t_min, sweep_t_max;
  const struct gs_project_inputs* lazy_records;
  int cameras;
} gs_frame_desc;
typedef struct gs_frame_slice {
  long long I;
  int n, wave_per_gaussian, first, last;
  long long svals, bins, fidx, gi_of_e, sorted_ids, slice_gi, counts, cum, tile_hot, n_emitted_dev;
} gs_frame_slice;
typedef struct gs_frame_state {
  int n_slices, P, N, S, R, H, W;
  float rolling_shutter_time;
  int shared_list;
  int depth_select;
  int select_overflow;
  float open_after_first;
  long long n_total;
  long long max_selected;
  long long arena_used;
  long long arena_required;
  gs_frame_slice slice[GS_FRAME_MAX_SLICES];
  int cameras;
} gs_frame_state;
int gs_frame_forward(const gs_frame_desc* desc, float* records, unsigned* depth_keys, const int* num_tiles_hit,
                     const float* background , const int* band_edges , const unsigned char* band_tile_done,
                     const float* color_means, const float* color_sh, const float* color_sh_rest , int color_K_stride, int color_sh_degree,
                     const float* color_viewmats ,
                     const float* pix_vel ,
                     const float* sample_times ,
                     float* out_img , float* out_T , float* out_depth,
                     float* out_combined ,
                     void* arena, long long arena_bytes, void* host_pinned,
                     long long host_pinned_bytes, gs_frame_state* state, void* stream);
long long gs_frame_backward_bytes(const gs_frame_state* state);
int gs_frame_backward(const gs_frame_state* state, const float* records, const float* background, const int* band_edges,
                      const float* out_T, const float* v_img, const float* v_alpha, const float* cmb_scale,
                      float cmb_gamma, float cmb_min_level, int bwd_variant, float* v_records, unsigned char* touched,
                      const float* pix_vel , const float* sample_times ,
                      void* arena, long long arena_bytes, void* stream);
int gs_frame_backward_depth(const gs_frame_state* state, const float* records, const float* background,
                            const int* band_edges, const float* out_T, const float* v_img, const float* v_alpha,
                            const float* cmb_scale, float cmb_gamma, float cmb_min_level, int bwd_variant,
                            float* v_records, unsigned char* touched, const float* pix_vel, const float* sample_times,
                            void* arena, long long arena_bytes, const float* v_depth , void* stream);
int gs_xy_absgrad_sum(int N, int P, int cameras, const float* v_records ,
                      const unsigned char* touched , float* out , void* stream);
int gs_frame_profile_enable(unsigned stage_mask);
int gs_frame_profile_read(int max_events, int* stage_ids, float* ms);

long long gs_image_loss_workspace_bytes(int img_height, int img_width);
int gs_image_loss_fwd_bwd(int img_height, int img_width, const float* pred, const float* gt, float ssim_lambda,
                          float* v_pred, float* loss_out, void* workspace, long long workspace_bytes, void* stream);
int gs_adam_step(int count, float* const* params, const float* const* grads, float* const* exp_avg,
                 float* const* exp_avg_sq, const long long* numel, const float* lr, double beta1, double beta2, double eps,
                 int step, void* stream);
int gs_adam_step_rows(int count, int N, const unsigned char* mask , float* const* params,
                      const float* const* grads, float* const* exp_avg, float* const* exp_avg_sq,
                      const int* widths, const float* lr, double beta1, double beta2, double eps, int step,
                      void* ws, long long ws_bytes, void* stream);
long long gs_adam_step_rows_workspace_bytes(int N);
int gs_visible_rows(int M, int N, const int* radii, unsigned char* mask, void* stream);

int gs_mcmc_inject_noise(int N, float* means, const float* log_scales, const float* quats, const float* opacity_logits,
                         float scaler, long long seed, long long step, const float* noise_in, float* noise_out,
                         void* stream);
int gs_mcmc_relocation(int M, const float* opacities, const float* scales, const int* ratios, float* new_opacities,
                       float* new_scales, void* stream);

int gs_bilagrid_slice_fwd(int B, int H, int W, int G, int GW, int GH, int L, const float* grids, const int* grid_idx,
                          const float* rgb, float* out, void* stream);
long long gs_bilagrid_slice_bwd_workspace_bytes(int B, int H, int W, int G, int GW, int GH, int L);
int gs_bilagrid_slice_bwd(int B, int H, int W, int G, int GW, int GH, int L, const float* grids, const int* grid_idx,
                          const float* rgb, const float* v_out, float* v_rgb, float* v_grids, void* ws,
                          long long ws_bytes, void* stream);
long long gs_bilagrid_tv_workspace_bytes(int G, int GW, int GH, int L);
int gs_bilagrid_tv_fwd_bwd(int G, int GW, int GH, int L, const float* grids, float weight, float* loss_out,
                           float* v_grids, void* ws, long long ws_bytes, void* stream);

#ifdef __cplusplus
}
#endif
#endif
```

Before: 1202.

## Add one-pass depth select with fused compaction, tail sort and device-side slice plan

Adds a one-pass selection path for the depth-select presort. A compaction kernel filters keys below the per-segment threshold into chunked slots using atomics. A finish kernel then sorts each segment in LDS (reusing the factored-out tail sort passes), computes counts and prefix sums, and builds the slice plan on device. This replaces the multi-kernel segmented sort, scan and plan-select sequence, and avoids the separate plan kernel when the selected count fits the tail cap. Overflow falls back to the old multipass path.

```diff
diff --git a/3dgs-deblur_amd/_lib.py b/3dgs-deblur_amd/_lib.py
--- a/3dgs-deblur_amd/_lib.py
+++ b/3dgs-deblur_amd/_lib.py
@@ -41,6 +41,7 @@
     "gs_segmented_sort_select_u32": [_L, _L, _P, _P, _P, _P, _P, _I, _I, _I, ctypes.c_uint, _P, _P, _P, _P, _P, _P, _L,
                                      ctypes.POINTER(_I), _L, _P],
     "gs_depth_select": [_L, _L, _P, _P, _L, _P, _P, _P, _L, _P],
+    "gs_select_onepass_u32": [_L, _L, _P, _P, _P, _L, _P, _P, _P, _P, _P, _P, _P, _P, _I, _P, _P, _P, _P, _L, _P],
     "gs_exclusive_scan_segments_u32": [_L, _L, _P, _P, _P, _P, _P, _L, _P],
     "gs_make_depth_keys64": [_L, _I, _P, _P, _P],
     "gs_gather_counts": [_L, _P, _P, _P, _P],
@@ -101,6 +102,7 @@
     "gs_segmented_sort_workspace_bytes": [_L, _L, _I, _I],
     "gs_segmented_sort_compact_workspace_bytes": [_L, _L, _I, _I, _I],
     "gs_depth_select_workspace_bytes": [_I],
+    "gs_select_onepass_workspace_bytes": [_L, _L],
     "gs_project_pose_scratch_bytes": [_I, _I, _I],
     "gs_image_loss_workspace_bytes": [_I, _I],
     "gs_adam_step_rows_workspace_bytes": [_I],
diff --git a/3dgs-deblur_amd/csrc/binning.hip b/3dgs-deblur_amd/csrc/binning.hip
--- a/3dgs-deblur_amd/csrc/binning.hip
+++ b/3dgs-deblur_amd/csrc/binning.hip
@@ -501,6 +501,116 @@
 constexpr int kTailMaxBits = 9;
 constexpr size_t kTailLds = ((size_t)kTailLocalCap + 16 * (1 << kTailMaxBits) + 64) * sizeof(unsigned);
 
+__device__ __forceinline__ void tail_sort_passes(unsigned (&key)[kTailR], unsigned n, unsigned Re, unsigned wbase, int lane,
+                                                 int wave, int begin_bit, unsigned emask, unsigned kmin, unsigned kmax,
+                                                 unsigned* stage, unsigned* cnt, unsigned* red) {
+  const unsigned long long lt_mask = (1ull << lane) - 1ull;
+  unsigned pos2[kTailR / 2];
+#pragma unroll
+  for (int o = 32; o > 0; o >>= 1) {
+    kmin = min(kmin, (unsigned)__shfl_xor((int)kmin, o));
+    kmax = max(kmax, (unsigned)__shfl_xor((int)kmax, o));
+  }
+  if (lane == 0) { red[wave] = kmin; red[16 + wave] = kmax; }
+  __syncthreads();
+#pragma unroll
+  for (int w = 0; w < 16; ++w) { kmin = min(kmin, red[w]); kmax = max(kmax, red[16 + w]); }
+  const unsigned base = kmin & ~((1u << begin_bit) - 1u);
+  const unsigned span = (kmax - base) >> begin_bit;
+  const int rem = span ? 32 - __clz((int)span) : 0;
+  const int passes = (rem + kTailMaxBits - 1) / kTailMaxBits;
+  const int wbits = passes ? (rem + passes - 1) / passes : 0;
+  const unsigned nb = 1u << wbits, mask = nb - 1u;
+  int shift = begin_bit;
+  for (int p = 0; p < passes; ++p, shift += wbits) {
+    for (unsigned d = threadIdx.x; d < 16u * nb; d += 1024u) cnt[d] = 0u;
+    __syncthreads();
+    unsigned* const wcnt = cnt + (unsigned)wave * nb;
+#pragma unroll
+    for (int r = 0; r < kTailR; ++r) {
+      if ((unsigned)r < Re) {
+        const unsigned e = wbase + (unsigned)r * 64u + lane;
+        const bool valid = e < n;
+        const unsigned digit = (((key[r] & emask) - base) >> shift) & mask;
+        unsigned long long peers = __ballot(valid);
+#pragma unroll
+        for (int b = 0; b < kTailMaxBits; ++b) {
+          if (b < wbits) {
+            const bool bit = (digit >> b) & 1u;
+            const unsigned long long m = __ballot(bit);
+            peers &= bit ? m : ~m;
+          }
+        }
+        const unsigned prefix = __popcll(peers & lt_mask), total = __popcll(peers);
+        unsigned c0 = 0;
+        if (valid) c0 = wcnt[digit];
+        __builtin_amdgcn_wave_barrier();
+        if (valid && prefix == 0) wcnt[digit] = c0 + total;
+        __builtin_amdgcn_wave_barrier();
+        pos2[r >> 1] = (r & 1) ? (pos2[r >> 1] | ((c0 + prefix) << 16)) : (c0 + prefix);
+      }
+    }
+    __syncthreads();
+    {
+      const unsigned d = threadIdx.x;
+      unsigned c = 0;
+      if (d < nb) {
+#pragma unroll
+        for (int w = 0; w < 16; ++w) c += cnt[(unsigned)w * nb + d];
+      }
+      unsigned inc = c;
+#pragma unroll
+      for (int o = 1; o < 64; o <<= 1) {
+        const unsigned t = __shfl_up(inc, o);
+        if (lane >= o) inc += t;
+      }
+      if (lane == 63) red[32 + wave] = inc;
+      __syncthreads();
+      unsigned run = inc - c;
+      for (int w = 0; w < wave; ++w) run += red[32 + w];
+      if (d < nb) {
+#pragma unroll
+        for (int w = 0; w < 16; ++w) {
+          const unsigned cw = cnt[(unsigned)w * nb + d];
+          cnt[(unsigned)w * nb + d] = run;
+          run += cw;
+        }
+      }
+    }
+    __syncthreads();
+    unsigned val[kTailR];
+#pragma unroll
+    for (int r = 0; r < kTailR; ++r) {
+      const unsigned e = wbase + (unsigned)r * 64u + lane;
+      if ((unsigned)r < Re && e < n) {
+        val[r] = stage[e];
+        const unsigned rank = (r & 1) ? pos2[r >> 1] >> 16 : pos2[r >> 1] & 0xffffu;
+        const unsigned slot = wcnt[(((key[r] & emask) - base) >> shift) & mask] + rank;
+        pos2[r >> 1] = (r & 1) ? ((pos2[r >> 1] & 0xffffu) | (slot << 16)) : ((pos2[r >> 1] & 0xffff0000u) | slot);
+      }
+    }
+    __syncthreads();
+#pragma unroll
+    for (int r = 0; r < kTailR; ++r) {
+      const unsigned e = wbase + (unsigned)r * 64u + lane;
+      if ((unsigned)r < Re && e < n) stage[(r & 1) ? pos2[r >> 1] >> 16 : pos2[r >> 1] & 0xffffu] = key[r];
+    }
+    __syncthreads();
+#pragma unroll
+    for (int r = 0; r < kTailR; ++r) {
+      const unsigned e = wbase + (unsigned)r * 64u + lane;
+      if ((unsigned)r < Re && e < n) key[r] = stage[e];
+    }
+    __syncthreads();
+#pragma unroll
+    for (int r = 0; r < kTailR; ++r) {
+      const unsigned e = wbase + (unsigned)r * 64u + lane;
+      if ((unsigned)r < Re && e < n) stage[(r & 1) ? pos2[r >> 1] >> 16 : pos2[r >> 1] & 0xffffu] = val[r];
+    }
+    __syncthreads();
+  }
+}
+
 __global__ __launch_bounds__(1024) void seg_tail_sort_kernel(size_t seg_len, const unsigned* __restrict__ keys_in,
                                                              const unsigned* __restrict__ vals_in,
                                                              unsigned* __restrict__ keys_out,
@@ -519,9 +629,7 @@
   const int lane = lane_id(), wave = threadIdx.x >> 6;
   const unsigned Re = (n + 1023u) >> 10;
   const unsigned wbase = (unsigned)wave * Re * 64u;
-  const unsigned long long lt_mask = (1ull << lane) - 1ull;
   unsigned key[kTailR];
-  unsigned pos2[kTailR / 2];
   unsigned kmin = 0xffffffffu, kmax = 0u;
   const unsigned emask = end_bit >= 32 ? 0xffffffffu : (1u << end_bit) - 1u;
 #pragma unroll
@@ -535,109 +643,7 @@
       kmax = max(kmax, key[r] & emask);
     }
   }
-#pragma unroll
-  for (int o = 32; o > 0; o >>= 1) {
-    kmin = min(kmin, (unsigned)__shfl_xor((int)kmin, o));
-    kmax = max(kmax, (unsigned)__shfl_xor((int)kmax, o));
-  }
-  if (lane == 0) { red[wave] = kmin; red[16 + wave] = kmax; }
-  __syncthreads();
-#pragma unroll
-  for (int w = 0; w < 16; ++w) { kmin = min(kmin, red[w]); kmax = max(kmax, red[16 + w]); }
-  const unsigned base = kmin & ~((1u << begin_bit) - 1u);
-  const unsigned span = (kmax - base) >> begin_bit;
-  const int rem = span ? 32 - __clz((int)span) : 0;
-  const int passes = (rem + kTailMaxBits - 1) / kTailMaxBits;
-  const int wbits = passes ? (rem + passes - 1) / passes : 0;
-  const unsigned nb = 1u << wbits, mask = nb - 1u;
-  int shift = begin_bit;
-  for (int p = 0; p < passes; ++p, shift += wbits) {
-    for (unsigned d = threadIdx.x; d < 16u * nb; d += 1024u) cnt[d] = 0u;
-    __syncthreads();
-    unsigned* const wcnt = cnt + (unsigned)wave * nb;
-#pragma unroll
-    for (int r = 0; r < kTailR; ++r) {
-      if ((unsigned)r < Re) {
-        const unsigned e = wbase + (unsigned)r * 64u + lane;
-        const bool valid = e < n;
-        const unsigned digit = (((key[r] & emask) - base) >> shift) & mask;
-        unsigned long long peers = __ballot(valid);
-#pragma unroll
-        for (int b = 0; b < kTailMaxBits; ++b) {
-          if (b < wbits) {
-            const bool bit = (digit >> b) & 1u;
-            const unsigned long long m = __ballot(bit);
-            peers &= bit ? m : ~m;
-          }
-        }
-        const unsigned prefix = __popcll(peers & lt_mask), total = __popcll(peers);
-        unsigned c0 = 0;
-        if (valid) c0 = wcnt[digit];
-        __builtin_amdgcn_wave_barrier();
-        if (valid && prefix == 0) wcnt[digit] = c0 + total;
-        __builtin_amdgcn_wave_barrier();
-        pos2[r >> 1] = (r & 1) ? (pos2[r >> 1] | ((c0 + prefix) << 16)) : (c0 + prefix);
-      }
-    }
-    __syncthreads();
-    {
-      const unsigned d = threadIdx.x;
-      unsigned c = 0;
-      if (d < nb) {
-#pragma unroll
-        for (int w = 0; w < 16; ++w) c += cnt[(unsigned)w * nb + d];
-      }
-      unsigned inc = c;
-#pragma unroll
-      for (int o = 1; o < 64; o <<= 1) {
-        const unsigned t = __shfl_up(inc, o);
-        if (lane >= o) inc += t;
-      }
-      if (lane == 63) red[32 + wave] = inc;
-      __syncthreads();
-      unsigned run = inc - c;
-      for (int w = 0; w < wave; ++w) run += red[32 + w];
-      if (d < nb) {
-#pragma unroll
-        for (int w = 0; w < 16; ++w) {
-          const unsigned cw = cnt[(unsigned)w * nb + d];
-          cnt[(unsigned)w * nb + d] = run;
-          run += cw;
-        }
-      }
-    }
-    __syncthreads();
-    unsigned val[kTailR];
-#pragma unroll
-    for (int r = 0; r < kTailR; ++r) {
-      const unsigned e = wbase + (unsigned)r * 64u + lane;
-      if ((unsigned)r < Re && e < n) {
-        val[r] = stage[e];
-        const unsigned rank = (r & 1) ? pos2[r >> 1] >> 16 : pos2[r >> 1] & 0xffffu;
-        const unsigned slot = wcnt[(((key[r] & emask) - base) >> shift) & mask] + rank;
-        pos2[r >> 1] = (r & 1) ? ((pos2[r >> 1] & 0xffffu) | (slot << 16)) : ((pos2[r >> 1] & 0xffff0000u) | slot);
-      }
-    }
-    __syncthreads();
-#pragma unroll
-    for (int r = 0; r < kTailR; ++r) {
-      const unsigned e = wbase + (unsigned)r * 64u + lane;
-      if ((unsigned)r < Re && e < n) stage[(r & 1) ? pos2[r >> 1] >> 16 : pos2[r >> 1] & 0xffffu] = key[r];
-    }
-    __syncthreads();
-#pragma unroll
-    for (int r = 0; r < kTailR; ++r) {
-      const unsigned e = wbase + (unsigned)r * 64u + lane;
-      if ((unsigned)r < Re && e < n) key[r] = stage[e];
-    }
-    __syncthreads();
-#pragma unroll
-    for (int r = 0; r < kTailR; ++r) {
-      const unsigned e = wbase + (unsigned)r * 64u + lane;
-      if ((unsigned)r < Re && e < n) stage[(r & 1) ? pos2[r >> 1] >> 16 : pos2[r >> 1] & 0xffffu] = val[r];
-    }
-    __syncthreads();
-  }
+  tail_sort_passes(key, n, Re, wbase, lane, wave, begin_bit, emask, kmin, kmax, stage, cnt, red);
 #pragma unroll
   for (int r = 0; r < kTailR; ++r) {
     const unsigned e = wbase + (unsigned)r * 64u + lane;
@@ -653,6 +659,236 @@
         if (gather_out) gather_out[org + e] = gather_src[v];
       }
     }
+  }
+}
+
+constexpr int kOnepassRounds = 8;
+constexpr int kOnepassChunk = 256 * kOnepassRounds;
+constexpr int kOnepassMaxChunks = 8 * (1 << kTailMaxBits);
+constexpr int kOnepassMaxSegs = 1024;
+
+__global__ __launch_bounds__(256) void select_compact_kernel(size_t seg_len, unsigned nch,
+                                                             const unsigned* __restrict__ keys,
+                                                             const unsigned* __restrict__ weights,
+                                                             const unsigned* __restrict__ key_hi, unsigned cap,
+                                                             int pack_bits, unsigned* __restrict__ ckeys,
+                                                             unsigned* __restrict__ cvals,
+                                                             unsigned* __restrict__ counters ,
+                                                             unsigned* __restrict__ tab ) {
+  __shared__ unsigned s_cnt[kOnepassRounds * 4], s_w[4], s_base;
+  const unsigned seg = blockIdx.y;
+  const int lane = lane_id(), wave = threadIdx.x >> 6;
+  const unsigned long long lt_mask = (1ull << lane) - 1ull;
+  const size_t org = (size_t)seg * seg_len;
+  const unsigned hi = key_hi[seg];
+  const unsigned lim = (unsigned)min((size_t)cap, seg_len);
+  const unsigned cmax = (1u << (32 - pack_bits)) - 1u;
+  for (unsigned c = blockIdx.x; c < nch; c += gridDim.x) {
+    const size_t cbase = (size_t)c * kOnepassChunk;
+    unsigned k[kOnepassRounds], w[kOnepassRounds];
+#pragma unroll
+    for (int r = 0; r < kOnepassRounds; ++r) {
+      const size_t i = cbase + (size_t)r * 256 + threadIdx.x;
+      k[r] = i < seg_len ? keys[org + i] : 0xFFFFFFFFu;
+    }
+    unsigned wsum = 0;
+#pragma unroll
+    for (int r = 0; r < kOnepassRounds; ++r) {
+      const size_t i = cbase + (size_t)r * 256 + threadIdx.x;
+      const bool keep = i < seg_len && k[r] < hi;
+      w[r] = keep ? weights[org + i] : 0u;
+    }
+#pragma unroll
+    for (int r = 0; r < kOnepassRounds; ++r) {
+      const size_t i = cbase + (size_t)r * 256 + threadIdx.x;
+      const unsigned long long m = __ballot(i < seg_len && k[r] < hi);
+      if (lane == 0) s_cnt[r * 4 + wave] = (unsigned)__popcll(m);
+      wsum += w[r];
+    }
+    wsum = (unsigned)wave_sum_i((int)wsum);
+    if (lane == 0) s_w[wave] = wsum;
+    __syncthreads();
+    unsigned off[kOnepassRounds], run = 0;
+#pragma unroll
+    for (int r = 0; r < kOnepassRounds; ++r) {
+#pragma unroll
+      for (int q = 0; q < 4; ++q) {
+        if (q == wave) off[r] = run;
+        run += s_cnt[r * 4 + q];
+      }
+    }
+    if (threadIdx.x == 0) {
+      unsigned slot = 0;
+      if (run) {
+        slot = atomicAdd(&counters[2 * seg], run);
+        atomicAdd(&counters[2 * seg + 1], s_w[0] + s_w[1] + s_w[2] + s_w[3]);
+      }
+      tab[2 * ((size_t)seg * nch + c)] = slot;
+      tab[2 * ((size_t)seg * nch + c) + 1] = run;
+      s_base = slot;
+    }
+    __syncthreads();
+    const unsigned slot0 = s_base;
+#pragma unroll
+    for (int r = 0; r < kOnepassRounds; ++r) {
+      const size_t i = cbase + (size_t)r * 256 + threadIdx.x;
+      const bool keep = i < seg_len && k[r] < hi;
+      const unsigned long long m = __ballot(keep);
+      const unsigned pos = slot0 + off[r] + (unsigned)__popcll(m & lt_mask);
+      if (keep && pos < lim) {
+        ckeys[org + pos] = k[r];
+        cvals[org + pos] = (unsigned)(org + i) | (min(w[r], cmax) << pack_bits);
+      }
+    }
+    __syncthreads();
+  }
+}
+
+__device__ __forceinline__ unsigned wave_incl_scan(unsigned v, int lane) {
+#pragma unroll
+  for (int o = 1; o < 64; o <<= 1) {
+    const unsigned t = __shfl_up(v, o);
+    if (lane >= o) v += t;
+  }
+  return v;
+}
+
+__global__ __launch_bounds__(1024) void select_finish_kernel(size_t seg_len, unsigned segs, unsigned nch, unsigned cap,
+                                                             const unsigned* __restrict__ ckeys,
+                                                             const unsigned* __restrict__ cvals,
+                                                             const unsigned* __restrict__ counters,
+                                                             const unsigned* __restrict__ tab,
+                                                             const unsigned* __restrict__ gather_src, int pack_bits,
+                                                             unsigned* __restrict__ keys_out,
+                                                             unsigned* __restrict__ vals_out,
+                                                             unsigned* __restrict__ counts_out,
+                                                             unsigned* __restrict__ cum_out,
+                                                             unsigned* __restrict__ seg_counts,
+                                                             unsigned* __restrict__ total_out, int plan_K,
+                                                             unsigned* __restrict__ plan ,
+                                                             const unsigned* __restrict__ grand) {
+  extern __shared__ unsigned tail_lds[];
+  unsigned* const stage = tail_lds;
+  unsigned* const cnt = stage + kTailLocalCap;
+  unsigned* const c_first = cnt;
+  unsigned* const c_slot = cnt + kOnepassMaxChunks;
+  unsigned* const red = cnt + 16 * (1 << kTailMaxBits);
+  const unsigned seg = blockIdx.x;
+  const int lane = lane_id(), wave = threadIdx.x >> 6;
+  const size_t org = (size_t)seg * seg_len;
+  unsigned s_n = 0, s_t = 0;
+  if (threadIdx.x < segs) { s_n = counters[2 * threadIdx.x]; s_t = counters[2 * threadIdx.x + 1]; }
+  const int over = __syncthreads_or(s_n > cap);
+  unsigned front = threadIdx.x < seg ? s_t : 0u, all = s_t;
+  front = (unsigned)wave_sum_i((int)front);
+  all = (unsigned)wave_sum_i((int)all);
+  if (lane == 0) { red[wave] = front; red[16 + wave] = all; }
+  __syncthreads();
+  front = 0u; all = 0u;
+#pragma unroll
+  for (int w = 0; w < 16; ++w) { front += red[w]; all += red[16 + w]; }
+  const unsigned n = counters[2 * seg], seg_tiles = counters[2 * seg + 1];
+  const unsigned live = (unsigned)min((size_t)n, seg_len);
+  if (threadIdx.x == 0) {
+    seg_counts[seg] = n;
+    if (seg == 0) *total_out = all;
+  }
+  if (plan) {
+    const size_t PK = (size_t)segs * plan_K;
+    if (threadIdx.x < (unsigned)plan_K) {
+      plan[(size_t)seg * plan_K + threadIdx.x] = live;
+      plan[PK + (size_t)seg * plan_K + threadIdx.x] = seg_tiles;
+    }
+    if (threadIdx.x == 0) {
+      plan[2 * PK + seg] = seg_tiles;
+      plan[2 * PK + segs + seg] = live;
+      if (seg == 0) plan[2 * PK + 2 * (size_t)segs] = *grand;
+    }
+  }
+  if (over) return;
+  if (threadIdx.x == 0) cum_out[org] = front;
+  if (n == 0) return;
+  {
+    unsigned c[4], sl[4], sum = 0;
+#pragma unroll
+    for (int j = 0; j < 4; ++j) {
+      const unsigned ch = threadIdx.x * 4u + j;
+      c[j] = ch < nch ? tab[2 * ((size_t)seg * nch + ch) + 1] : 0u;
+      sl[j] = ch < nch ? tab[2 * ((size_t)seg * nch + ch)] : 0u;
+      sum += c[j];
+    }
+    const unsigned inc = wave_incl_scan(sum, lane);
+    if (lane == 63) red[32 + wave] = inc;
+    __syncthreads();
+    unsigned ex = inc - sum;
+    for (int w = 0; w < wave; ++w) ex += red[32 + w];
+#pragma unroll
+    for (int j = 0; j < 4; ++j) {
+      const unsigned ch = threadIdx.x * 4u + j;
+      if (ch < nch) { c_first[ch] = ex; c_slot[ch] = sl[j]; }
+      ex += c[j];
+    }
+  }
+  __syncthreads();
+  const unsigned Re = (n + 1023u) >> 10;
+  const unsigned wbase = (unsigned)wave * Re * 64u;
+  const unsigned top = 1u << (31 - __clz((int)nch));
+#pragma unroll 1
+  for (unsigned r = 0; r < Re; ++r) {
+    const unsigned e = wbase + r * 64u + lane;
+    if (e < n) {
+      unsigned ch = 0;
+      for (unsigned s = top; s; s >>= 1)
+        if (ch + s < nch && c_first[ch + s] <= e) ch += s;
+      stage[e] = c_slot[ch] + (e - c_first[ch]);
+    }
+  }
+  unsigned key[kTailR];
+  unsigned kmin = 0xffffffffu, kmax = 0u;
+#pragma unroll
+  for (int r = 0; r < kTailR; ++r) {
+    const unsigned e = wbase + (unsigned)r * 64u + lane;
+    const bool ok = (unsigned)r < Re && e < n;
+    const size_t src = org + (ok ? stage[e] : 0u);
+    key[r] = ok ? ckeys[src] : 0u;
+    if (ok) {
+      stage[e] = cvals[src];
+      kmin = min(kmin, key[r]);
+      kmax = max(kmax, key[r]);
+    }
+  }
+  tail_sort_passes(key, n, Re, wbase, lane, wave, 0, 0xffffffffu, kmin, kmax, stage, cnt, red);
+#pragma unroll
+  for (int r = 0; r < kTailR; ++r) {
+    const unsigned e = wbase + (unsigned)r * 64u + lane;
+    if ((unsigned)r < Re && e < n) {
+      const unsigned v = stage[e];
+      const unsigned idx = v & ((1u << pack_bits) - 1u);
+      unsigned c = v >> pack_bits;
+      if (c == (1u << (32 - pack_bits)) - 1u) c = gather_src[idx];
+      keys_out[org + e] = key[r];
+      vals_out[org + e] = idx;
+      counts_out[org + e] = c;
+      stage[e] = c;
+    }
+  }
+  unsigned run = 0;
+#pragma unroll 1
+  for (unsigned r = 0; r < Re; ++r) {
+    const unsigned e = wbase + r * 64u + lane;
+    const unsigned c = e < n ? stage[e] : 0u;
+    const unsigned inc = wave_incl_scan(c, lane);
+    if (e < n) stage[e] = run + inc - c;
+    run += (unsigned)readlane_i((int)inc, 63);
+  }
+  if (lane == 0) red[48 + wave] = run;
+  __syncthreads();
+  unsigned woff = front;
+  for (int w = 0; w < wave; ++w) woff += red[48 + w];
+#pragma unroll 1
+  for (unsigned r = 0; r < Re; ++r) {
+    const unsigned e = wbase + r * 64u + lane;
+    if (e < n) cum_out[org + e] = woff + stage[e];
   }
 }
 
@@ -1838,6 +2074,54 @@
                               tail_cap > 0 ? (unsigned)((tail_cap + sort_block_keys<unsigned>() - 1) / sort_block_keys<unsigned>()) : 0u);
 }
 
+GS_EXPORT long long gs_select_onepass_workspace_bytes(long long n, long long seg_len) {
+  if (n <= 0 || seg_len <= 0 || n % seg_len != 0 || n > (1ll << 28)) return 0;
+  const long long nch = (seg_len + kOnepassChunk - 1) / kOnepassChunk;
+  if (nch > kOnepassMaxChunks || n / seg_len > kOnepassMaxSegs) return 0;
+  return n / seg_len * nch * 2 * (long long)sizeof(unsigned) + 256;
+}
+
+GS_EXPORT int gs_select_onepass_u32(long long n, long long seg_len, const unsigned* keys, const unsigned* weights,
+                                    const unsigned* key_hi, long long cap, unsigned* keys_tmp, unsigned* vals_tmp,
+                                    unsigned* keys_out, unsigned* vals_out, unsigned* counts_out, unsigned* cum_out,
+                                    unsigned* seg_counts, unsigned* total_out, int plan_K, int* plan,
+                                    const unsigned* grand, unsigned* counters, void* ws, long long ws_bytes,
+                                    void* stream) {
+  if (n <= 0 || seg_len <= 0 || n % seg_len != 0 || cap <= 0 || cap > kTailLocalCap || !keys || !weights || !key_hi ||
+      !keys_tmp || !vals_tmp || !keys_out || !vals_out || !counts_out || !cum_out || !seg_counts || !total_out ||
+      !counters || !ws)
+    return GS_ERR_INVALID;
+  static_assert(kTailLocalCap == 24576, "GS_SELECT_ONEPASS_MAX (include/gsdeblur.h) is the one-block sort's capacity");
+  if (plan && (plan_K <= 0 || plan_K > 1024 || !grand)) return GS_ERR_INVALID;
+  const long long need = gs_select_onepass_workspace_bytes(n, seg_len);
+  if (need == 0) return GS_ERR_INVALID;
+  if (ws_bytes < need) return GS_ERR_WORKSPACE;
+  hipStream_t st = (hipStream_t)stream;
+  const long long segs = n / seg_len;
+  const unsigned nch = (unsigned)((seg_len + kOnepassChunk - 1) / kOnepassChunk);
+  int pack_bits = 1;
+  while ((1ll << pack_bits) < n) ++pack_bits;
+  static std::atomic<unsigned long long> lds_set{0ull};
+  int dev = 0;
+  (void)hipGetDevice(&dev);
+  const unsigned long long bit = 1ull << (dev & 63);
+  if ((lds_set.load(std::memory_order_relaxed) & bit) == 0) {
+    hipError_t e = hipFuncSetAttribute(reinterpret_cast<const void*>(select_finish_kernel),
+                                       hipFuncAttributeMaxDynamicSharedMemorySize, (int)kTailLds);
+    if (e != hipSuccess) return 1000 + (int)e;
+    lds_set.fetch_or(bit, std::memory_order_relaxed);
+  }
+  unsigned* tab = reinterpret_cast<unsigned*>(ws);
+  const unsigned gx = (unsigned)std::max(1ll, std::min(((long long)nch + 1) / 2, std::max(1ll, 1024 / segs)));
+  hipLaunchKernelGGL(select_compact_kernel, dim3(gx, (unsigned)segs), dim3(256), 0, st, (size_t)seg_len, nch, keys,
+                     weights, key_hi, (unsigned)cap, pack_bits, keys_tmp, vals_tmp, counters, tab);
+  hipLaunchKernelGGL(select_finish_kernel, dim3((unsigned)segs), dim3(1024), kTailLds, st, (size_t)seg_len,
+                     (unsigned)segs, nch, (unsigned)cap, keys_tmp, vals_tmp, counters, tab, weights, pack_bits, keys_out,
+                     vals_out, counts_out, cum_out, seg_counts, total_out, plan_K, reinterpret_cast<unsigned*>(plan),
+                     grand);
+  return gs_launch_status();
+}
+
 GS_EXPORT int gs_tile_open_sat(int P, int H, int W, const unsigned char* tile_done, int* sat,
                                unsigned long long* open_bits, const int* gate, void* stream) {
   if (P <= 0) return GS_ERR_INVALID;
diff --git a/3dgs-deblur_amd/csrc/frame.hip b/3dgs-deblur_amd/csrc/frame.hip
--- a/3dgs-deblur_amd/csrc/frame.hip
+++ b/3dgs-deblur_amd/csrc/frame.hip
@@ -284,25 +284,46 @@
   const long long w64 = (tx + 63) / 64;
   unsigned long long* open_bits = A.take<unsigned long long>((long long)P * ty * w64);
   const long long sel_b = select ? Arena::up(gs_depth_select_workspace_bytes(P)) + 256 : 0;
+  const long long cnt_b = select ? Arena::up(8ll * P) : 0;
   const long long flag_off = ((1 + kKMax) * P * T + 3) & ~3ll;
-  char* zero_blk = A.take<char>(sel_b + flag_off + 4 * kKMax);
-  unsigned char* zeros_u8 = reinterpret_cast<unsigned char*>(zero_blk) + sel_b;
+  const long long zero_b = Arena::up(sel_b + cnt_b + flag_off + 4 * kKMax);
+  char* zero_blk = A.take<char>(zero_b);
+  unsigned char* zeros_u8 = reinterpret_cast<unsigned char*>(zero_blk) + sel_b + cnt_b;
   unsigned* sel_grand = reinterpret_cast<unsigned*>(zero_blk + sel_b - 256);
+  unsigned* sel_counters = reinterpret_cast<unsigned*>(zero_blk + sel_b);
   unsigned* thr_dev = select ? A.take<unsigned>(P) : nullptr;
+  const long long onepass_ws_b = (select && !d.select_multipass) ? gs_select_onepass_workspace_bytes(n, N) : 0;
+  char* onepass_ws = onepass_ws_b ? A.take<char>(onepass_ws_b) : nullptr;
   int* plan_dev = A.take<int>(plan_ints);
   unsigned char* tile_done_rs = R > 1 ? A.take<unsigned char>(P * T) : nullptr;
   unsigned char* tile_done_samples = shared ? A.take<unsigned char>((long long)S * T) : nullptr;
   if (!A.ok) { state->arena_required = 2 * A.off; return GS_ERR_WORKSPACE; }
   if (shared) CHECK(hip_status(hipMemsetAsync(tile_done_samples, 0, (long long)S * T, st)));
-  CHECK(hip_status(hipMemsetAsync(zero_blk, 0, sel_b + flag_off + 4 * kKMax, st)));
+  CHECK(hip_status(hipMemsetAsync(zero_blk, 0, zero_b, st)));
   int* open_flags = reinterpret_cast<int*>(zeros_u8 + flag_off);
   const long long plan_tiles = (d.band_clipped && R > 1) ? (T + R - 1) / R : T;
   const long long base0 = plan_tiles * (long long)std::max(1, d.slice_base);
 
   const unsigned* sorted_gi = nullptr;
   bool bound_known = false;
+  bool plan_on_device = false;
+  const long long PK = (long long)P * kKMax;
   auto presort = [&](int phase, long long tail_cap) -> int {
     int res = 0;
+    plan_on_device = false;
+    if (select && phase == 0 && !bound_known && onepass_ws && tail_cap > 0 && tail_cap <= GS_SELECT_ONEPASS_MAX) {
+      StageScope sc(ST_DEPTH_SORT, st);
+      CHECK(gs_depth_select(n, N, depth_keys, reinterpret_cast<const unsigned*>(num_tiles_hit), base0, thr_dev,
+                            sel_grand, zero_blk, sel_b - 256, st));
+      bound_known = true;
+      CHECK(gs_select_onepass_u32(n, N, depth_keys, reinterpret_cast<const unsigned*>(num_tiles_hit), thr_dev, tail_cap,
+                                  k0s, v0, k1, v1, counts_r, cum, n_live, total, kKMax, plan_dev, sel_grand, sel_counters,
+                                  onepass_ws, onepass_ws_b, st));
+      sorted_gi = v1;
+      plan_on_device = true;
+      state->select_onepass = 1;
+      return GS_OK;
+    }
     {
       StageScope sc(ST_DEPTH_SORT, st);
       if (!select) {
@@ -332,7 +353,6 @@
   unsigned* hp = reinterpret_cast<unsigned*>(host_pinned) + 1;
   unsigned* hp_seq = reinterpret_cast<unsigned*>(host_pinned);
   const bool poll = d.poll_readback != 0;
-  const long long PK = (long long)P * kKMax;
   std::vector<long long> NV(P), seg_totals(P);
   std::vector<std::vector<long long>> bnd(P), rel(P);
   long long n_total = 0, true_total = 0;
@@ -343,7 +363,9 @@
   auto make_plan = [&](int phase) -> int {
     if (planned) {
       StageScope sc(ST_PLAN, st);
-      if (select && phase == 0)
+      if (plan_on_device)
+        ;
+      else if (select && phase == 0)
         CHECK(gs_slice_plan_select(P, N, kKMax, cum, total, plan_dev, reinterpret_cast<unsigned*>(plan_dev + PK),
                                    reinterpret_cast<unsigned*>(plan_dev + 2 * PK), n_live,
                                    reinterpret_cast<unsigned*>(plan_dev + 2 * PK + P), sel_grand, st));
@@ -408,6 +430,7 @@
     for (int p = 0; p < P; ++p) most = std::max(most, NV[p]);
     if (most > tail_cap) {
       state->select_overflow = 1;
+      state->select_onepass = 0;
       CHECK(presort(0, 0));
       CHECK(make_plan(0));
     }
diff --git a/3dgs-deblur_amd/ops.py b/3dgs-deblur_amd/ops.py
--- a/3dgs-deblur_amd/ops.py
+++ b/3dgs-deblur_amd/ops.py
@@ -180,6 +180,7 @@
 BAND_AWARE = int(os.environ.get("GSD_BAND_AWARE", "1"))
 LAZY_RECORDS = int(os.environ.get("GSD_LAZY_RECORDS", "1"))
 DEPTH_SELECT = int(os.environ.get("GSD_DEPTH_SELECT", "1"))
+SELECT_ONEPASS = True
 NEEDLE_HP = int(os.environ.get("GSD_NEEDLE_HP", "1"))
 
 
@@ -214,6 +215,7 @@
 profiler: Optional[StageProfiler] = None
 last_num_intersects: int = 0
 last_depth_select: int = 0
+last_select_onepass: int = 0
 
 
 def _stage(name: str):
@@ -449,7 +451,8 @@
                                                                                      ("sweep_t_min", ctypes.c_float),
                                                                                      ("sweep_t_max", ctypes.c_float),
                                                                                      ("lazy_records", ctypes.c_void_p),
-                                                                                     ("cameras", ctypes.c_int)]
+                                                                                     ("cameras", ctypes.c_int),
+                                                                                     ("select_multipass", ctypes.c_int)]
 
 
 class _ProjectInputs(ctypes.Structure):
@@ -469,7 +472,7 @@
                 [("rolling_shutter_time", ctypes.c_float), ("shared_list", ctypes.c_int), ("depth_select", ctypes.c_int),
                  ("select_overflow", ctypes.c_int), ("open_after_first", ctypes.c_float)] +
                 [(k, ctypes.c_longlong) for k in ("n_total", "max_selected", "arena_used", "arena_required")] +
-                [("slice", _FrameSlice * 16), ("cameras", ctypes.c_int)])
+                [("slice", _FrameSlice * 16), ("cameras", ctypes.c_int), ("select_onepass", ctypes.c_int)])
 
 
 def _box_share(state) -> Optional[float]:
@@ -589,7 +592,7 @@
                          out_depth: Optional[Tensor] = None, reserve_backward: bool = True, rs=None, combine=None,
                          hints: Optional[FrameHints] = None, band_clipped: bool = False, lazy=None,
                          depth_select: Optional[bool] = None, cameras: int = 1):
-    global last_num_intersects, _slice_totals, last_depth_select
+    global last_num_intersects, _slice_totals, last_depth_select, last_select_onepass
     L = _L()
     dev = records.device
     tx, ty = _tiles(H, W)
@@ -617,7 +620,7 @@
                       int(bool(band_clipped)), int(bool(depth_select and slice_base > 0)),
                       int(min(hints.select_cap, 2 ** 31 - 1)) if depth_select else 0,
                       float(rs[3][0]) if shared and len(rs) > 3 else 0.0, float(rs[3][1]) if shared and len(rs) > 3 else 0.0,
-                      ctypes.addressof(lazy) if lazy is not None else None, int(cameras))
+                      ctypes.addressof(lazy) if lazy is not None else None, int(cameras), int(not SELECT_ONEPASS))
     state = _FrameState()
     out_img = torch.empty(S, H, W, 3, device=dev)
     out_T = torch.empty(S, H, W, device=dev)
@@ -641,6 +644,7 @@
                             int((state.arena_used + L.gs_frame_backward_bytes(ctypes.byref(state))) * 1.15))
     last_num_intersects = int(state.n_total)
     last_depth_select = int(state.depth_select)
+    last_select_onepass = int(state.select_onepass)
     _slice_totals = [arena[sl.n_emitted_dev:sl.n_emitted_dev + 4].view(torch.int32)
                      for sl in (state.slice[i] for i in range(state.n_slices))]
     return out_img, out_T, dict(arena=arena, arena_obj=lease.arena, lease=lease, gen=lease.gen, state=state,
diff --git a/include/gsdeblur.h b/include/gsdeblur.h
--- a/include/gsdeblur.h
+++ b/include/gsdeblur.h
@@ -138,6 +138,18 @@
                                  long long ws_bytes, int* result_buf ,
                                  long long tail_cap ,
                                  void* stream);
+#define GS_SELECT_ONEPASS_MAX 24576
+long long gs_select_onepass_workspace_bytes(long long n, long long seg_len);
+int gs_select_onepass_u32(long long n, long long seg_len, const unsigned* keys ,
+                          const unsigned* weights , const unsigned* key_hi , long long cap,
+                          unsigned* keys_tmp, unsigned* vals_tmp , unsigned* keys_out,
+                          unsigned* vals_out , unsigned* counts_out ,
+                          unsigned* cum_out ,
+                          unsigned* seg_counts ,
+                          unsigned* total_out , int plan_K,
+                          int* plan , const unsigned* grand ,
+                          unsigned* counters , void* ws, long long ws_bytes,
+                          void* stream);
 int gs_exclusive_scan_segments_u32(long long n, long long seg_len, const unsigned* seg_counts ,
                                    const unsigned* in, unsigned* out, unsigned* total_out , void* ws,
                                    long long ws_bytes, void* stream);
@@ -324,6 +336,7 @@
   float sweep_t_min, sweep_t_max;
   const struct gs_project_inputs* lazy_records;
   int cameras;
+  int select_multipass;
 } gs_frame_desc;
 typedef struct gs_frame_slice {
   long long I;
@@ -343,6 +356,7 @@
   long long arena_required;
   gs_frame_slice slice[GS_FRAME_MAX_SLICES];
   int cameras;
+  int select_onepass;
 } gs_frame_state;
 int gs_frame_forward(const gs_frame_desc* desc, float* records, unsigned* depth_keys, const int* num_tiles_hit,
                      const float* background , const int* band_edges , const unsigned char* band_tile_done,
```

Result: slower. 1179 (-1.9%).
